# mcveanlab/Corticall

Hardware: AMD Instinct MI355X
Metric: k-mers traversed/sec (whole node) + contigs/sec, k=47 3-color LdBG (higher is better)
Workload: dtype u64

## Files before the change

### corticall_amd/csrc/capi.cpp

```cpp
#include <string.h>

#include <memory>

#include "build.h"
#include "cursor.h"
#include "engine_host.h"
#include "linkbuild.h"
#include "select.h"
#include "shard.h"
#include "thread.h"
#include "unitigs.h"

using namespace ldbg;

namespace ldbg {
int64_t sort_ctx_file(const std::string& in_path, const std::string& out_path, int device);
int64_t subset_ctx_file(const std::string& in_path, const int64_t* indices, int64_t n, const std::string& out_path);
int64_t join_ctx_files(const std::vector<std::string>& paths, const std::string& out_path, int device);
std::vector<uint8_t> join_ctx_image(const std::vector<std::string>& paths, int device, bool find_view);
void profile_reset_all();
bool profile_get(const char* family, double* ms, int64_t* n);
}

struct ldbg_graph {
    Graph g;
    ldbg_graph(const std::string& p, const void* img, int64_t n, int dev) : g(p, img, n, dev) {}
    ldbg_graph(const std::string& p, const void* hdr, int64_t hdr_bytes, const void* d_recs, int64_t n_recs, int dev) : g(p, hdr, hdr_bytes, d_recs, n_recs, dev) {}
};
struct ldbg_links {
    Links l;
    ldbg_links(const std::string& p, const Graph& g) : l(p, g) {}
    ldbg_links(const BuiltLinks& b, const Graph& g) : l(b, g) {}
};
struct ldbg_engine {
    Engine e;
    std::unique_ptr<CursorHost> cursor;
    std::unique_ptr<CursorBatchHost> cursor_batch;
    explicit ldbg_engine(const ldbg_engine_config& c) : e(c) {}
};
struct ldbg_dfs_result { std::unique_ptr<DfsBatch> b; };
struct ldbg_cursor_result { std::unique_ptr<CursorBatchResult> r; };
struct ldbg_unitigs { Unitigs u; ldbg_unitigs(const Graph& g, const int* c, int n) : u(g, c, n) {} };
struct ldbg_selection {
    Selection s;
    ldbg_selection(const Graph& g, const ldbg_record_filter& f, const Graph* q) : s(g, f, q) {}
    ldbg_selection(const Graph& g, int child_colour, const Graph& dirty) : s(g, child_colour, dirty) {}
};
struct ldbg_threading {
    Threading t;
    ldbg_threading(const Graph* g, const Graph* rois, const char* bases, const int64_t* offsets, int64_t n, int flags, bool dev, rt::stream_t s)
        : t(g, rois, bases, offsets, n, flags, dev, s) {}
};
struct ldbg_image { ShardImage img; ldbg_image(const Graph& shard, int64_t cap, int64_t global) : img(shard, cap, global) {} };

namespace {
thread_local std::string g_err;
template <class F>
ldbg_status guard(F f) {
    try { f(); return LDBG_OK; }
    catch (const StatusError& e) { g_err = e.what(); return (ldbg_status)e.status; }
    catch (const std::bad_alloc&) { g_err = "out of host memory"; return LDBG_ERR_HIP; }
    catch (const std::exception& e) { g_err = e.what(); return LDBG_ERR_ARG; }
}
ldbg_engine_config unwrap(const ldbg_engine_config& c, std::vector<const ldbg_links*>& keep) {
    ldbg_engine_config u = c;
    u.graph = c.graph ? (const ldbg_graph*)&c.graph->g : nullptr;
    u.rois = c.rois ? (const ldbg_graph*)&c.rois->g : nullptr;
    keep.clear();
    for (int i = 0; i < c.nlinks; i++) keep.push_back(c.links[i] ? (const ldbg_links*)&c.links[i]->l : nullptr);
    u.links = keep.data();
    return u;
}
}

extern "C" {

const char* ldbg_last_error(void) { return g_err.c_str(); }
#ifndef LDBG_SRCID
#define LDBG_SRCID "unstamped"
#endif
const char* ldbg_version(void) { return "ldbg 0.2 (gfx950, src " LDBG_SRCID ")"; }
ldbg_status ldbg_device_count(int* count) { *count = rt::device_count(); return LDBG_OK; }

ldbg_status ldbg_kmer_encode(const char* ascii, int k, uint64_t* words_out) {
    return guard([&] {
        if (k <= 0 || k > 128) throw StatusError(LDBG_ERR_ARG, "bad k");
        if (!ascii_to_words_ci(ascii, k, words_out, (k + 31) / 32))
            throw StatusError(LDBG_ERR_ARG, "Nucleotide is not a valid character nucleotide");
    });
}
ldbg_status ldbg_kmer_decode(const uint64_t* words, int k, char* ascii_out) {
    return guard([&] {
        if (k <= 0 || k > 128) throw StatusError(LDBG_ERR_ARG, "bad k");
        words_to_ascii(words, k, (k + 31) / 32, ascii_out);
        ascii_out[k] = 0;
    });
}

ldbg_status ldbg_sort_ctx(const char* in_path, const char* out_path, int device, int64_t* num_records) {
    return guard([&] { const int64_t n = sort_ctx_file(in_path, out_path, device); if (num_records) *num_records = n; });
}

ldbg_status ldbg_ctx_write_records(const char* in_path, const int64_t* indices, int64_t n, const char* out_path) {
    return guard([&] { subset_ctx_file(in_path, indices, n, out_path); });
}

ldbg_status ldbg_join_ctx(const char* const* in_paths, int n_paths, const char* out_path, int device, int64_t* num_records) {
    return guard([&] {
        std::vector<std::string> paths;
        for (int i = 0; i < n_paths; i++) paths.push_back(in_paths[i]);
        const int64_t n = join_ctx_files(paths, out_path, device);
        if (num_records) *num_records = n;
    });
}

ldbg_status ldbg_graph_open(const char* path, int device, ldbg_graph** out) {
    return guard([&] { *out = nullptr; *out = new ldbg_graph(path, nullptr, 0, device); });
}
ldbg_status ldbg_graph_open_memory(const void* image, int64_t nbytes, int device, ldbg_graph** out) {
    return guard([&] { *out = nullptr; *out = new ldbg_graph("<memory>", image, nbytes, device); });
}
ldbg_status ldbg_graph_open_device(const void* header, int64_t header_bytes, const void* d_records, int64_t n_records, int device, ldbg_graph** out) {
    return guard([&] { *out = nullptr; *out = new ldbg_graph("<device>", header, header_bytes, d_records, n_records, device); });
}
ldbg_status ldbg_graph_build(const ldbg_build_sample* samples, int n_samples, int k, int flags, int device, ldbg_graph** out) {
    return guard([&] {
        if (!out) throw StatusError(LDBG_ERR_ARG, "build: null output");
        *out = nullptr;
        const BuiltRecords b = build_records(samples, n_samples, k, flags, device);
        *out = new ldbg_graph("<build>", b.header.data(), (int64_t)b.header.size(), b.d_records.get(), b.N, device);
    });
}
ldbg_status ldbg_graph_build_ctx(const ldbg_build_sample* samples, int n_samples, int k, int flags, int device, const char* out_path, int64_t* num_records) {
    return guard([&] {
        if (!out_path) throw StatusError(LDBG_ERR_ARG, "build: null output path");
        const BuiltRecords b = build_records(samples, n_samples, k, flags, device);
        build_write_ctx(b, out_path);
        if (num_records) *num_records = b.N;
    });
}
ldbg_status ldbg_graph_open_collection(const char* const* paths, int n_paths, int find_view, int device, ldbg_graph** out) {
    return guard([&] {
        *out = nullptr;
        std::vector<std::string> ps;
        for (int i = 0; i < n_paths; i++) ps.push_back(paths[i]);
        const std::vector<uint8_t> img = join_ctx_image(ps, device, find_view != 0);
        *out = new ldbg_graph("<collection>", img.data(), (int64_t)img.size(), device);
    });
}
ldbg_status ldbg_graph_close(ldbg_graph* g) { return guard([&] { delete g; }); }
ldbg_status ldbg_graph_info(const ldbg_graph* g, int* k, int* W, int* C, int64_t* N, int* version) {
    return guard([&] {
        if (k) *k = g->g.hdr.k;
        if (W) *W = g->g.hdr.W;
        if (C) *C = g->g.hdr.C;
        if (N) *N = g->g.hdr.num_records;
        if (version) *version = g->g.hdr.version;
    });
}
ldbg_status ldbg_graph_device(const ldbg_graph* g, int* device) { *device = g->g.device; return LDBG_OK; }
ldbg_status ldbg_graph_set_shard(ldbg_graph* g, int is_shard) {
    return guard([&] { g->g.view.java_tiny = (!is_shard && g->g.view.N <= 2) ? 1 : 0; g->g.is_shard = is_shard != 0; });
}
ldbg_status ldbg_graph_sample_name(const ldbg_graph* g, int color, char* buf, int buflen) {
    return guard([&] {
        if (color < 0 || color >= g->g.hdr.C) throw StatusError(LDBG_ERR_ARG, "colour out of range");
        snprintf(buf, buflen, "%s", g->g.hdr.colors[color].sample_name.c_str());
    });
}
ldbg_status ldbg_graph_color_info(const ldbg_graph* g, int color, ldbg_color_info* out, char* name, int buflen) {
    return guard([&] {
        if (color < 0 || color >= g->g.hdr.C) throw StatusError(LDBG_ERR_ARG, "colour out of range");
        const CtxColor& c = g->g.hdr.colors[color];
        out->mean_read_length = c.mean_read_length;
        out->total_sequence = c.total_sequence;
        out->tip_clipping = c.tip_clipping;
        out->low_covg_supernodes_removed = c.low_covg_supernodes_removed;
        out->low_covg_kmers_removed = c.low_covg_kmers_removed;
        out->cleaned_against_graph = c.cleaned_against_graph;
        out->low_cov_supernodes_threshold = c.low_cov_supernodes_threshold;
        out->low_cov_kmer_threshold = c.low_cov_kmer_threshold;
        if (name) snprintf(name, buflen, "%s", c.cleaned_against_graph_name.c_str());
    });
}
ldbg_status ldbg_graph_color_for_sample_name(const ldbg_graph* g, const char* name, int* color) {
    return guard([&] { *color = g->g.color_for_sample_name(name); });
}

ldbg_status ldbg_graph_records_dev(const ldbg_graph* g, int64_t first, int64_t n, uint64_t* d_words, uint32_t* d_cov, uint8_t* d_edges, void* stream) {
    return guard([&] {
        if (first < 0 || n < 0 || first + n > g->g.hdr.num_records) throw StatusError(LDBG_ERR_ARG, "record range outside 0.." + std::to_string(g->g.hdr.num_records));
        rt::set_device(g->g.device);
        g->g.records_dev(first, n, d_words, d_cov, d_edges, stream ? (rt::stream_t)stream : g->g.stream);
    });
}
ldbg_status ldbg_graph_records(const ldbg_graph* g, int64_t first, int64_t n, uint64_t* words, uint32_t* cov, uint8_t* edges) {
    return guard([&] {
        if (first < 0 || n < 0 || first + n > g->g.hdr.num_records) throw StatusError(LDBG_ERR_ARG, "record range outside 0.." + std::to_string(g->g.hdr.num_records));
        if (n == 0) return;
        rt::set_device(g->g.device);
        const int W = g->g.hdr.W, C = g->g.hdr.C;
        rt::stream_t s = g->g.stream;
        uint64_t* dw = (uint64_t*)rt::dmalloc((size_t)n * W * 8);
        uint32_t* dc = cov ? (uint32_t*)rt::dmalloc((size_t)n * C * 4) : nullptr;
        uint8_t* de = edges ? (uint8_t*)rt::dmalloc((size_t)n * C) : nullptr;
        g->g.records_dev(first, n, dw, dc, de, s);
        if (words) rt::d2h(words, dw, (size_t)n * W * 8, s);
        if (cov) rt::d2h(cov, dc, (size_t)n * C * 4, s);
        if (edges) rt::d2h(edges, de, (size_t)n * C, s);
        rt::stream_sync(s);
        rt::dfree(dw); rt::dfree(dc); rt::dfree(de);
    });
}

ldbg_status ldbg_graph_find_dev(const ldbg_graph* g, const uint64_t* d_packed, int64_t n, int64_t* d_idx, uint32_t* d_cov, uint8_t* d_edges, void* stream) {
    return guard([&] {
        rt::set_device(g->g.device);
        g->g.find_dev(d_packed, n, d_idx, d_cov, d_edges, stream ? (rt::stream_t)stream : g->g.stream);
    });
}
ldbg_status ldbg_shard_owner_dev(int k, const uint64_t* d_packed, int64_t n, int world, uint64_t* d_canon, int32_t* d_owner, void* stream) {
    return guard([&] {
        shard_owner_dev(k, d_packed, n, world, d_canon, d_owner, (rt::stream_t)stream);
        rt::stream_sync((rt::stream_t)stream);
    });
}
ldbg_status ldbg_shard_owner(int k, const uint64_t* packed, int64_t n, int world, int device, int32_t* owner) {
    return guard([&] {
        if (n <= 0) return;
        if (rt::device_count() <= device) throw StatusError(LDBG_ERR_HIP, "no HIP device " + std::to_string(device) + " available (libldbg has no CPU fallback)");
        rt::set_device(device);
        const int W = (k + 31) / 32;
        rt::stream_t s = rt::stream_create();
        uint64_t* dq = (uint64_t*)rt::dmalloc((size_t)n * W * 8);
        int32_t* d_o = (int32_t*)rt::dmalloc((size_t)n * 4);
        rt::h2d(dq, packed, (size_t)n * W * 8, s);
        shard_owner_dev(k, dq, n, world, nullptr, d_o, s);
        rt::d2h(owner, d_o, (size_t)n * 4, s);
        rt::stream_sync(s);
        rt::dfree(dq); rt::dfree(d_o);
        rt::stream_destroy(s);
    });
}
ldbg_status ldbg_shard_nbr_queries(const ldbg_graph* g, int64_t first, int64_t n, uint64_t* d_words, uint8_t* d_flips, uint8_t* d_have) {
    return guard([&] { rt::set_device(g->g.device); shard_nbr_queries(g->g, first, n, d_words, d_flips, d_have); });
}
ldbg_status ldbg_shard_set_nbr(ldbg_graph* g, int64_t first, int64_t n, const int32_t* d_owner, const int64_t* d_lidx, const uint8_t* d_flips) {
    return guard([&] { rt::set_device(g->g.device); shard_set_nbr(g->g, first, n, d_owner, d_lidx, d_flips); });
}
ldbg_status ldbg_image_create(const ldbg_graph* shard, int64_t cap, int64_t global_records, ldbg_image** out) {
    return guard([&] {
        *out = nullptr;
        if (cap < 1 || cap > ldbg::max_records_per_device()) throw StatusError(LDBG_ERR_ARG, "image capacity out of range");
        *out = new ldbg_image(shard->g, cap, global_records);
    });
}
ldbg_status ldbg_image_destroy(ldbg_image* im) { return guard([&] { delete im; }); }
ldbg_status ldbg_image_graph(ldbg_image* im, ldbg_graph** g) { return guard([&] { *g = reinterpret_cast<ldbg_graph*>(&im->img.graph()); }); }
ldbg_status ldbg_image_row_bytes(const ldbg_image* im, int* bytes) { return guard([&] { *bytes = im->img.row_bytes(); }); }
ldbg_status ldbg_image_clear(ldbg_image* im) { return guard([&] { rt::set_device(im->img.graph().device); im->img.clear(); }); }
static rt::stream_t image_stream(const ldbg_image* im, void* stream) { return stream ? (rt::stream_t)stream : im->img.graph().stream; }
ldbg_status ldbg_image_serve(const ldbg_image* im, int my_rank, const uint64_t* d_keys, int64_t n, uint8_t* d_out, void* stream) {
    return guard([&] { rt::set_device(im->img.graph().device); im->img.serve(my_rank, (const unsigned long long*)d_keys, n, 1, d_out, image_stream(im, stream)); });
}
ldbg_status ldbg_image_serve_chain(const ldbg_image* im, int my_rank, const uint64_t* d_keys, int64_t n, int depth, uint8_t* d_out, void* stream) {
    return guard([&] { rt::set_device(im->img.graph().device); im->img.serve(my_rank, (const unsigned long long*)d_keys, n, depth, d_out, image_stream(im, stream)); });
}
ldbg_status ldbg_image_insert(ldbg_image* im, const ldbg_engine* e, const uint8_t* d_rows, int64_t n, void* stream) {
    return guard([&] { rt::set_device(im->img.graph().device); im->img.insert(e ? &e->e : nullptr, d_rows, n, image_stream(im, stream)); });
}
ldbg_status ldbg_image_lookup(const ldbg_image* im, const uint64_t* d_keys, int64_t n, int32_t* d_slots, void* stream) {
    return guard([&] { rt::set_device(im->img.graph().device); im->img.lookup((const unsigned long long*)d_keys, n, d_slots, image_stream(im, stream)); });
}
ldbg_status ldbg_image_bucket(ldbg_image* im, int world, uint32_t cap_per_owner, uint64_t* d_send, void* stream) {
    return guard([&] { rt::set_device(im->img.graph().device); im->img.bucket(world, cap_per_owner, (unsigned long long*)d_send, image_stream(im, stream)); });
}
ldbg_status ldbg_image_request(ldbg_image* im, const uint64_t* d_keys, int64_t n, void* stream) {
    return guard([&] { rt::set_device(im->img.graph().device); im->img.request((const unsigned long long*)d_keys, n, image_stream(im, stream)); });
}
ldbg_status ldbg_image_reset_requests(ldbg_image* im, void* stream) {
    return guard([&] { rt::set_device(im->img.graph().device); im->img.reset_requests(image_stream(im, stream)); });
}
ldbg_status ldbg_image_counters(const ldbg_image* im, int64_t* n_rows, int64_t* n_req, int* overflow) {
    return guard([&] { rt::set_device(im->img.graph().device); im->img.counters(n_rows, n_req, overflow); });
}
ldbg_status ldbg_engine_sharded_walk_begin(ldbg_engine* e, ldbg_image* im, const char* seeds, int64_t n, const int32_t* d_seed_slot, void* stream) {
    return guard([&] { e->e.sharded_walk_begin(im->img, seeds, n, d_seed_slot, (rt::stream_t)stream); });
}
ldbg_status ldbg_engine_sharded_walk_round(ldbg_engine* e, int64_t* d_stats) { return guard([&] { e->e.sharded_walk_round(d_stats); }); }
ldbg_status ldbg_engine_sharded_walk_finish(ldbg_engine* e, int64_t* total_bytes, int64_t* traversed) {
    return guard([&] {
        try { e->e.sharded_walk_finish(total_bytes, traversed); }
        catch (const StatusError& se) {
            if (se.status == LDBG_ERR_CAPACITY && std::string(se.what()) == "LINKSTORE_FULL") e->e.link_store_capacity *= 4;
            throw;
        }
    });
}

ldbg_status ldbg_graph_find(const ldbg_graph* g, const uint64_t* packed, int64_t n, int64_t* idx_out, uint32_t* cov_out, uint8_t* edges_out) {
    return guard([&] {
        if (n <= 0) return;
        rt::set_device(g->g.device);
        const int W = g->g.hdr.W, C = g->g.hdr.C;
        rt::stream_t s = g->g.stream;
        uint64_t* dq = (uint64_t*)rt::dmalloc((size_t)n * W * 8);
        int64_t* di = (int64_t*)rt::dmalloc((size_t)n * 8);
        uint32_t* dc = cov_out ? (uint32_t*)rt::dmalloc((size_t)n * C * 4) : nullptr;
        uint8_t* de = edges_out ? (uint8_t*)rt::dmalloc((size_t)n * C) : nullptr;
        rt::h2d(dq, packed, (size_t)n * W * 8, s);
        g->g.find_dev(dq, n, di, dc, de, s);
        rt::d2h(idx_out, di, (size_t)n * 8, s);
        if (cov_out) rt::d2h(cov_out, dc, (size_t)n * C * 4, s);
        if (edges_out) rt::d2h(edges_out, de, (size_t)n * C, s);
        rt::stream_sync(s);
        rt::dfree(dq); rt::dfree(di); rt::dfree(dc); rt::dfree(de);
    });
}
ldbg_status ldbg_graph_find_ascii(const ldbg_graph* g, const char* kmers, int64_t n, int64_t* idx_out, uint32_t* cov_out, uint8_t* edges_out) {
    return guard([&] {
        rt::set_device(g->g.device);
        const int W = g->g.hdr.W, k = g->g.hdr.k, C = g->g.hdr.C;
        if (n <= 0) return;
        std::vector<uint64_t> packed((size_t)n * W);
        std::vector<uint8_t> valid((size_t)n);
        ascii_batch_to_words(kmers, n, k, W, packed.data(), valid.data());
        rt::stream_t s = g->g.stream;
        DevBlocks tmp;
        uint64_t* dq = tmp.get<uint64_t>((size_t)n * W);
        uint8_t* dv = tmp.get<uint8_t>((size_t)n);
        int64_t* di = tmp.get<int64_t>((size_t)n);
        uint32_t* dc = cov_out ? tmp.get<uint32_t>((size_t)n * C) : nullptr;
        uint8_t* de = edges_out ? tmp.get<uint8_t>((size_t)n * C) : nullptr;
        rt::h2d(dq, packed.data(), (size_t)n * W * 8, s);
        rt::h2d(dv, valid.data(), (size_t)n, s);
        g->g.find_dev(dq, n, di, dc, de, s, dv);
        rt::d2h(idx_out, di, (size_t)n * 8, s);
        if (cov_out) rt::d2h(cov_out, dc, (size_t)n * C * 4, s);
        if (edges_out) rt::d2h(edges_out, de, (size_t)n * C, s);
        rt::stream_sync(s);
    });
}

ldbg_status ldbg_graph_unitigs(const ldbg_graph* g, const int* colors, int n_colors, ldbg_unitigs** out) {
    return guard([&] {
        *out = nullptr;
        if (!colors && n_colors > 0) throw StatusError(LDBG_ERR_ARG, "unitigs: null colours");
        *out = new ldbg_unitigs(g->g, colors, n_colors);
    });
}
ldbg_status ldbg_unitigs_info(const ldbg_unitigs* u, int64_t* count, int64_t* total_bases, int64_t* longest, double* build_ms) {
    return guard([&] {
        if (count) *count = u->u.count;
        if (total_bases) *total_bases = u->u.total_bases;
        if (longest) *longest = u->u.longest;
        if (build_ms) *build_ms = u->u.build_ms;
    });
}
ldbg_status ldbg_unitigs_get(const ldbg_unitigs* u, int64_t first, int64_t n, int64_t* offsets, char* bases, int64_t capacity) {
    return guard([&] { u->u.get(first, n, offsets, bases, capacity, false, u->u.graph.stream); });
}
ldbg_status ldbg_unitigs_get_dev(const ldbg_unitigs* u, int64_t first, int64_t n, int64_t* d_offsets, char* d_bases, int64_t capacity, void* stream) {
    return guard([&] { u->u.get(first, n, d_offsets, d_bases, capacity, true, stream ? (rt::stream_t)stream : u->u.graph.stream); });
}
ldbg_status ldbg_unitigs_coverage(const ldbg_unitigs* u, int64_t first, int64_t n, uint32_t* cov) { return guard([&] { u->u.coverage(first, n, cov); }); }
ldbg_status ldbg_unitigs_of_records(const ldbg_unitigs* u, const int64_t* records, int64_t n, int64_t* unitig, int64_t* position, int8_t* orientation) {
    return guard([&] { u->u.of_records(records, n, unitig, position, orientation); });
}
ldbg_status ldbg_unitigs_write_fasta(const ldbg_unitigs* u, const char* path) { return guard([&] { u->u.write_fasta(path); }); }
ldbg_status ldbg_unitigs_write_gfa1(const ldbg_unitigs* u, const char* path, int sample_color, int flags) {
    return guard([&] { u->u.write_gfa1(path, sample_color, flags); });
}
ldbg_status ldbg_unitigs_free(ldbg_unitigs* u) { return guard([&] { delete u; }); }

ldbg_status ldbg_graph_select(const ldbg_graph* g, const ldbg_record_filter* filter, ldbg_selection** out) {
    return guard([&] {
        *out = nullptr;
        if (!filter) throw StatusError(LDBG_ERR_ARG, "select: null filter");
        *out = new ldbg_selection(g->g, *filter, nullptr);
    });
}
ldbg_status ldbg_graph_select_lookup(const ldbg_graph* g, const ldbg_record_filter* filter, const ldbg_graph* q, ldbg_selection** out) {
    return guard([&] {
        *out = nullptr;
        if (!filter || !q) throw StatusError(LDBG_ERR_ARG, "select: null filter or query graph");
        *out = new ldbg_selection(g->g, *filter, &q->g);
    });
}
ldbg_status ldbg_selection_count(const ldbg_selection* sel, int64_t* n) { return guard([&] { *n = sel->s.count; }); }
ldbg_status ldbg_selection_indices(const ldbg_selection* sel, int64_t first, int64_t n, int64_t* idx) {
    return guard([&] { sel->s.indices(first, n, idx, false, sel->s.graph.stream); });
}
ldbg_status ldbg_selection_indices_dev(const ldbg_selection* sel, int64_t first, int64_t n, int64_t* d_idx, void* stream) {
    return guard([&] { sel->s.indices(first, n, d_idx, true, stream ? (rt::stream_t)stream : sel->s.graph.stream); });
}
ldbg_status ldbg_selection_write_ctx(const ldbg_selection* sel, const int* colours, int n_colours, const char* header_path, const char* out_path) {
    return guard([&] { sel->s.write_ctx(colours, n_colours, header_path, out_path); });
}
ldbg_status ldbg_selection_open_graph(const ldbg_selection* sel, const int* colours, int n_colours, const char* header_path, ldbg_graph** out) {
    return guard([&] {
        *out = nullptr;
        const std::vector<uint8_t> hdr = sel->s.header(colours, n_colours, header_path);
        const DevRecords d = sel->s.pack(colours, n_colours);
        *out = new ldbg_graph("<selection>", hdr.data(), (int64_t)hdr.size(), d.get(), sel->s.count, sel->s.graph.device);
    });
}
ldbg_status ldbg_selection_free(ldbg_selection* sel) { return guard([&] { delete sel; }); }

ldbg_status ldbg_graph_recover(const ldbg_graph* g, int child_colour, const ldbg_graph* dirty, ldbg_selection** out, int64_t* n_recovered) {
    return guard([&] {
        if (!out) throw StatusError(LDBG_ERR_ARG, "recover: null output");
        *out = nullptr;
        if (!g || !dirty) throw StatusError(LDBG_ERR_ARG, "recover: null graph");
        *out = new ldbg_selection(g->g, child_colour, dirty->g);
        if (n_recovered) *n_recovered = (*out)->s.n_recovered;
    });
}
ldbg_status ldbg_selection_recovered_coverage(const ldbg_selection* sel, int64_t first, int64_t n, int32_t* cov) {
    return guard([&] { sel->s.recovered_coverage(first, n, cov); });
}
ldbg_status ldbg_selection_write_recovered(const ldbg_selection* sel, const char* out_path) {
    return guard([&] {
        if (!out_path) throw StatusError(LDBG_ERR_ARG, "recover: null output path");
        sel->s.write_recovered(out_path);
    });
}
ldbg_status ldbg_selection_open_recovered(const ldbg_selection* sel, ldbg_graph** out) {
    return guard([&] {
        *out = nullptr;
        const std::vector<uint8_t> hdr = sel->s.recovered_header();
        const DevRecords d = sel->s.pack_recovered();
        *out = new ldbg_graph("<recovered>", hdr.data(), (int64_t)hdr.size(), d.get(), sel->s.count, sel->s.graph.device);
    });
}

ldbg_status ldbg_links_open(const char* path, const ldbg_graph* g, ldbg_links** out) {
    return guard([&] { *out = nullptr; *out = new ldbg_links(path, g->g); });
}
ldbg_status ldbg_links_build_ctp(const ldbg_graph* g, const char* sample_name, const char* bases, const int64_t* offsets, int64_t n_reads, int flags,
                                 const char* out_path, int64_t* num_kmers_with_links, int64_t* num_links) {
    return guard([&] {
        if (!g) throw StatusError(LDBG_ERR_ARG, "links build: null graph");
        if (!out_path) throw StatusError(LDBG_ERR_ARG, "links build: null output path");
        const BuiltLinks b = build_links(g->g, sample_name, bases, offsets, n_reads, flags);
        built_links_write(b, out_path);
        if (num_kmers_with_links) *num_kmers_with_links = (int64_t)b.records.size();
        if (num_links) *num_links = b.num_links;
    });
}
ldbg_status ldbg_links_build(const ldbg_graph* g, const char* sample_name, const char* bases, const int64_t* offsets, int64_t n_reads, int flags, ldbg_links** out) {
    return guard([&] {
        if (!out) throw StatusError(LDBG_ERR_ARG, "links build: null output");
        *out = nullptr;
        if (!g) throw StatusError(LDBG_ERR_ARG, "links build: null graph");
        const BuiltLinks b = build_links(g->g, sample_name, bases, offsets, n_reads, flags);
        *out = new ldbg_links(b, g->g);
    });
}
ldbg_status ldbg_graph_thread(const ldbg_graph* g, const ldbg_graph* rois, const char* bases, const int64_t* offsets, int64_t n_seqs, int flags, ldbg_threading** out) {
    return guard([&] {
        if (!out) throw StatusError(LDBG_ERR_ARG, "thread: null output");
        *out = nullptr;
        *out = new ldbg_threading(g ? &g->g : nullptr, rois ? &rois->g : nullptr, bases, offsets, n_seqs, flags, false, nullptr);
    });
}
ldbg_status ldbg_graph_thread_dev(const ldbg_graph* g, const ldbg_graph* rois, const void* d_bases, const void* d_offsets, int64_t n_seqs, int flags, void* stream,
                                  ldbg_threading** out) {
    return guard([&] {
        if (!out) throw StatusError(LDBG_ERR_ARG, "thread: null output");
        *out = nullptr;
        *out = new ldbg_threading(g ? &g->g : nullptr, rois ? &rois->g : nullptr, (const char*)d_bases, (const int64_t*)d_offsets, n_seqs, flags, true, (rt::stream_t)stream);
    });
}
ldbg_status ldbg_threading_info(const ldbg_threading* t, int64_t* n_seqs, int64_t* n_windows, int64_t* n_regions, double* device_ms) {
    return guard([&] {
        if (!t) throw StatusError(LDBG_ERR_ARG, "thread: null threading");
        if (n_seqs) *n_seqs = t->t.n_seqs;
        if (n_windows) *n_windows = t->t.n_windows;
        if (n_regions) *n_regions = t->t.n_regions;
        if (device_ms) *device_ms = t->t.device_ms;
    });
}
ldbg_status ldbg_threading_windows(const ldbg_threading* t, int64_t first, int64_t n, int64_t* rec, uint8_t* info, int32_t* copy_index) {
    return guard([&] {
        if (!t) throw StatusError(LDBG_ERR_ARG, "thread: null threading");
        t->t.windows(first, n, rec, info, copy_index, false, nullptr);
    });
}
ldbg_status ldbg_threading_windows_dev(const ldbg_threading* t, int64_t first, int64_t n, void* d_rec, void* d_info, void* d_copy_index, void* stream) {
    return guard([&] {
        if (!t) throw StatusError(LDBG_ERR_ARG, "thread: null threading");
        t->t.windows(first, n, (int64_t*)d_rec, (uint8_t*)d_info, (int32_t*)d_copy_index, true, (rt::stream_t)stream);
    });
}
ldbg_status ldbg_threading_coverage(const ldbg_threading* t, int colour, int64_t first, int64_t n, int32_t* cov) {
    return guard([&] {
        if (!t) throw StatusError(LDBG_ERR_ARG, "thread: null threading");
        t->t.coverage(colour, first, n, cov);
    });
}
ldbg_status ldbg_threading_summary(const ldbg_threading* t, int64_t first_seq, int64_t n, int64_t* win_start, int32_t* first_hit, int32_t* last_hit, int32_t* n_hits,
                                   int32_t* n_distinct, uint8_t* ends) {
    return guard([&] {
        if (!t) throw StatusError(LDBG_ERR_ARG, "thread: null threading");
        t->t.summary(first_seq, n, win_start, first_hit, last_hit, n_hits, n_distinct, ends);
    });
}
ldbg_status ldbg_threading_regions(const ldbg_threading* t, int64_t* region_offsets, int32_t* start, int32_t* stop, int64_t capacity) {
    return guard([&] {
        if (!t) throw StatusError(LDBG_ERR_ARG, "thread: null threading");
        t->t.regions(region_offsets, start, stop, capacity);
    });
}
ldbg_status ldbg_threading_free(ldbg_threading* t) { return guard([&] { delete t; }); }

ldbg_status ldbg_links_close(ldbg_links* l) { return guard([&] { delete l; }); }
ldbg_status ldbg_links_index(const char* in_path, const char* out_path, const char* source, int64_t* num_records) {
    return guard([&] { const int64_t n = links_index_file(in_path, out_path, source ? source : ""); if (num_records) *num_records = n; });
}
ldbg_status ldbg_links_source(const ldbg_links* l, char* buf, int buflen) { return guard([&] { snprintf(buf, buflen, "%s", l->l.source().c_str()); }); }
ldbg_status ldbg_links_info(const ldbg_links* l, int* version, int* num_colors, int* k, int64_t* nkg, int64_t* nkl, int64_t* nl) {
    return guard([&] {
        if (version) *version = l->l.version;
        if (num_colors) *num_colors = l->l.num_colors;
        if (k) *k = l->l.k;
        if (nkg) *nkg = l->l.num_kmers_in_graph;
        if (nkl) *nkl = l->l.num_kmers_with_links;
        if (nl) *nl = l->l.num_links;
    });
}
ldbg_status ldbg_links_sample_name(const ldbg_links* l, int color, char* buf, int buflen) {
    return guard([&] {
        if (color < 0 || color >= (int)l->l.sample_names.size()) throw StatusError(LDBG_ERR_ARG, "colour out of range");
        snprintf(buf, buflen, "%s", l->l.sample_names[color].c_str());
    });
}
ldbg_status ldbg_links_get(const ldbg_links* l, const char* kmer, int* found, char* buf, int64_t buflen) {
    return guard([&] {
        const HostLinksRecord* r = l->l.get(std::string(kmer, l->l.k));
        *found = r ? 1 : 0;
        std::string s;
        if (r) {
            s = r->kmer + " " + std::to_string(r->juncs.size()) + "\n";
            for (auto& j : r->juncs) {
                s += j.is_fw ? "F " : "R ";
                s += std::to_string(j.num_junctions) + " ";
                for (size_t c = 0; c < j.cov.size(); c++) { if (c) s += ","; s += std::to_string(j.cov[c]); }
                s += " " + j.junctions + "\n";
            }
        }
        if ((int64_t)s.size() + 1 > buflen) throw StatusError(LDBG_ERR_CAPACITY, "buffer too small: need " + std::to_string(s.size() + 1));
        memcpy(buf, s.c_str(), s.size() + 1);
    });
}

void ldbg_engine_config_default(ldbg_engine_config* c) {
    memset(c, 0, sizeof(*c));
    c->direction = LDBG_DIR_BOTH;
    c->combination_operator = LDBG_OP_OR;
    c->stopping_rule = LDBG_STOP_CONTIG;
    c->max_branch_length = 75000;
    c->connect_all_neighbors = 0;
    c->strict_java_flip = 1;
}
ldbg_status ldbg_engine_create(const ldbg_engine_config* cfg, ldbg_engine** out) {
    return guard([&] {
        *out = nullptr;
        if (cfg->n_traversal > LDBG_MAX_COLORS || cfg->n_joining > LDBG_MAX_COLORS || cfg->n_recruitment > LDBG_MAX_COLORS || cfg->n_secondary > LDBG_MAX_COLORS)
            throw StatusError(LDBG_ERR_ARG, "too many colours");
        std::vector<const ldbg_links*> keep;
        ldbg_engine_config u = unwrap(*cfg, keep);
        *out = new ldbg_engine(u);
    });
}
ldbg_status ldbg_engine_destroy(ldbg_engine* e) { return guard([&] { delete e; }); }

static ldbg_status walk_batch_run_any(ldbg_engine* e, const char* seeds, int64_t n, int64_t* total_bytes, int64_t* traversed, bool on_device) {
    return guard([&] {
        for (int attempt = 0;; attempt++) {
            try { e->e.walk_batch_run(seeds, n, total_bytes, traversed, on_device); return; }
            catch (const StatusError& se) {
                if (se.status == LDBG_ERR_CAPACITY && std::string(se.what()) == "LINKSTORE_FULL" && attempt < 8) { e->e.link_store_capacity *= 4; continue; }
                throw;
            }
        }
    });
}
ldbg_status ldbg_engine_walk_batch_run(ldbg_engine* e, const char* seeds, int64_t n, int64_t* total_bytes, int64_t* traversed) {
    return walk_batch_run_any(e, seeds, n, total_bytes, traversed, false);
}
ldbg_status ldbg_engine_walk_batch_run_device(ldbg_engine* e, const void* d_seeds, int64_t n, int64_t* total_bytes, int64_t* traversed) {
    if (n > 0 && !d_seeds) return guard([&] { throw StatusError(LDBG_ERR_ARG, "ldbg_engine_walk_batch_run_device: null seeds"); });
    return walk_batch_run_any(e, (const char*)d_seeds, n, total_bytes, traversed, true);
}
ldbg_status ldbg_host_alloc(int64_t bytes, void** out) {
    return guard([&] { *out = nullptr; if (bytes < 0) throw StatusError(LDBG_ERR_ARG, "ldbg_host_alloc: negative size"); *out = rt::hmalloc_pinned((size_t)bytes); });
}
ldbg_status ldbg_host_free(void* p) { return guard([&] { rt::hfree_pinned(p); }); }
ldbg_status ldbg_engine_walk_batch_fetch(ldbg_engine* e, char* arena, int64_t cap, int64_t* offsets, int64_t* walk_len) {
    return guard([&] { e->e.walk_batch_fetch(arena, cap, offsets, walk_len); });
}
ldbg_status ldbg_engine_walk_batch(ldbg_engine* e, const char* seeds, int64_t n, char* arena, int64_t cap, int64_t* offsets, int64_t* walk_len, int64_t* traversed) {
    int64_t total = 0;
    ldbg_status st = ldbg_engine_walk_batch_run(e, seeds, n, &total, traversed);
    if (st != LDBG_OK) return st;
    return ldbg_engine_walk_batch_fetch(e, arena, cap, offsets, walk_len);
}
ldbg_status ldbg_engine_walk_vertices(ldbg_engine* e, int64_t walk, int64_t capacity, int64_t* len, uint64_t* words, int64_t* rec, int32_t* copy, int32_t* index) {
    return guard([&] { e->e.walk_vertices(walk, capacity, len, words, rec, copy, index); });
}

ldbg_status ldbg_engine_walk_roi_hits(ldbg_engine* e, int64_t* offsets, uint32_t* hits, int64_t capacity, uint8_t* has_null) {
    return guard([&] { e->e.walk_roi_hits(offsets, hits, capacity, has_null); });
}

ldbg_status ldbg_engine_dfs_batch(ldbg_engine* e, const char* sources, int64_t n, const char* sinks, const int64_t* sink_offsets, ldbg_dfs_result** out) {
    return guard([&] {
        *out = nullptr;
        for (int attempt = 0;; attempt++) {
            try {
                std::unique_ptr<DfsBatch> b(e->e.dfs_batch(sources, n, sinks, sink_offsets));
                *out = new ldbg_dfs_result{std::move(b)};
                return;
            } catch (const StatusError& se) {
                const std::string what = se.what();
                if (se.status == LDBG_ERR_CAPACITY && what == "LINKSTORE_FULL" && attempt < 8) { e->e.link_store_capacity *= 4; continue; }
                if (se.status == LDBG_ERR_CAPACITY && what == "LOG_FULL" && e->e.dfs_log_blocks < (1 << 20)) { e->e.dfs_log_blocks *= 8; continue; }
                if (se.status == LDBG_ERR_CAPACITY && what == "DEPTH_OVERFLOW" && e->e.dfs_max_depth < 4096) { e->e.dfs_max_depth *= 4; continue; }
                if (se.status == LDBG_ERR_CAPACITY && what == "DEPTH_OVERFLOW")
                    throw StatusError(LDBG_ERR_UNSUPPORTED, "dfs recursion deeper than 4096 branches (the reference overflows its thread stack here)");
                throw;
            }
        }
    });
}
ldbg_status ldbg_engine_sharded_dfs_batch(ldbg_engine* e, ldbg_image* im, const char* sources, int64_t n, const char* sinks, const int64_t* sink_offsets,
                                          const int32_t* d_seed_slot, const int32_t* d_sink_slot, int (*round_done)(void*), void* user,
                                          int64_t* d_stats, void* stream, ldbg_dfs_result** out) {
    return guard([&] {
        *out = nullptr;
        if (&im->img.graph() != e->e.graph) throw StatusError(LDBG_ERR_ARG, "the engine was not created on this image's graph");
        ShardedRun sr{&im->img, d_seed_slot, d_sink_slot, round_done, user, d_stats, (rt::stream_t)stream};
        try {
            std::unique_ptr<DfsBatch> b(e->e.dfs_batch(sources, n, sinks, sink_offsets, &sr));
            b->materialize();
            *out = new ldbg_dfs_result{std::move(b)};
        } catch (const StatusError& se) {
            const std::string what = se.what();
            if (se.status == LDBG_ERR_CAPACITY && what == "LINKSTORE_FULL") e->e.link_store_capacity *= 4;
            if (se.status == LDBG_ERR_CAPACITY && what == "LOG_FULL" && e->e.dfs_log_blocks < (1 << 20)) e->e.dfs_log_blocks *= 8;
            if (se.status == LDBG_ERR_CAPACITY && what == "DEPTH_OVERFLOW" && e->e.dfs_max_depth < 4096) e->e.dfs_max_depth *= 4;
            throw;
        }
    });
}
static const DfsGraphHost& dfs_at(const ldbg_dfs_result* r, int64_t i) {
    if (!r || !r->b) throw StatusError(LDBG_ERR_ARG, "no dfs result");
    if (i < 0 || i >= (int64_t)r->b->results.size()) throw StatusError(LDBG_ERR_ARG, "dfs result index out of range");
    return r->b->results[(size_t)i];
}
ldbg_status ldbg_dfs_result_sizes(const ldbg_dfs_result* r, int64_t i, int* is_null, int64_t* n_vertices, int64_t* n_edges) {
    return guard([&] {
        const DfsGraphHost& g = dfs_at(r, i);
        if (is_null) *is_null = g.is_null ? 1 : 0;
        if (n_vertices) *n_vertices = g.n_vertices();
        if (n_edges) *n_edges = g.n_edges();
    });
}
ldbg_status ldbg_dfs_result_get(const ldbg_dfs_result* r, int64_t i, uint64_t* kmer_words, int64_t* rec, int32_t* copy_index, int32_t* index,
                                int32_t* edge_src, int32_t* edge_dst, int32_t* edge_color) {
    return guard([&] {
        dfs_at(r, i);
        if (kmer_words) r->b->materialize();
        const DfsGraphHost& g = dfs_at(r, i);
        if (g.packed) { r->b->read_packed(i, rec, copy_index, index, edge_src, edge_dst, edge_color); return; }
        if (kmer_words && !g.words.empty()) memcpy(kmer_words, g.words.data(), g.words.size() * 8);
        for (size_t v = 0; v < g.verts.size(); v++) {
            if (rec) rec[v] = g.verts[v].rec;
            if (copy_index) copy_index[v] = g.verts[v].copy;
            if (index) index[v] = g.verts[v].index;
        }
        for (size_t x = 0; x < g.edges.size(); x++) {
            if (edge_src) edge_src[x] = g.edges[x].src;
            if (edge_dst) edge_dst[x] = g.edges[x].dst;
            if (edge_color) edge_color[x] = g.edges[x].color;
        }
    });
}
ldbg_status ldbg_dfs_result_walk(const ldbg_dfs_result* r, int64_t i, const char* seed, int color, char* contig, int64_t capacity, int64_t* len) {
    return guard([&] {
        dfs_at(r, i);
        const std::string c = r->b->walk_contig(i, seed, color);
        if (len) *len = (int64_t)c.size();
        if ((int64_t)c.size() + 1 > capacity) throw StatusError(LDBG_ERR_CAPACITY, "contig buffer too small: need " + std::to_string(c.size() + 1));
        memcpy(contig, c.c_str(), c.size() + 1);
    });
}
ldbg_status ldbg_dfs_result_merge(ldbg_dfs_result* r, const int64_t* which, int64_t m, ldbg_dfs_result** out) {
    return guard([&] {
        *out = nullptr;
        std::unique_ptr<DfsBatch> b(dfs_merge(*r->b, which, m));
        *out = new ldbg_dfs_result{std::move(b)};
    });
}
ldbg_status ldbg_dfs_result_free(ldbg_dfs_result* r) { delete r; return LDBG_OK; }
ldbg_status ldbg_engine_neighbours_batch(ldbg_engine* e, const char* kmers, int64_t n, int forward, int64_t* offsets, uint64_t* kmer_words, int64_t* rec, int64_t capacity) {
    return guard([&] { e->e.neighbours_batch(kmers, n, forward != 0, offsets, kmer_words, rec, capacity); });
}
ldbg_status ldbg_engine_dfs_kmers_traversed(const ldbg_engine* e, int64_t* n) { return guard([&] { *n = e->e.dfs_traversed(); }); }

static CursorHost& cursor_of(ldbg_engine* e) {
    if (!e->cursor) e->cursor.reset(new CursorHost(e->e));
    return *e->cursor;
}
ldbg_status ldbg_engine_assemble(ldbg_engine* e, const char* seed, int64_t capacity, int64_t* len, uint64_t* kmer_words, int64_t* rec) {
    return guard([&] { cursor_of(e).assemble(seed, capacity, len, kmer_words, rec); });
}
ldbg_status ldbg_engine_seek(ldbg_engine* e, const char* kmer) { return guard([&] { cursor_of(e).seek(kmer); }); }
ldbg_status ldbg_engine_has_next(ldbg_engine* e, int* yes) { return guard([&] { *yes = cursor_of(e).has(true) ? 1 : 0; }); }
ldbg_status ldbg_engine_has_previous(ldbg_engine* e, int* yes) { return guard([&] { *yes = cursor_of(e).has(false) ? 1 : 0; }); }
ldbg_status ldbg_engine_next(ldbg_engine* e, char* kmer_out, int64_t* rec_out) { return guard([&] { cursor_of(e).step(true, kmer_out, rec_out); }); }
ldbg_status ldbg_engine_previous(ldbg_engine* e, char* kmer_out, int64_t* rec_out) { return guard([&] { cursor_of(e).step(false, kmer_out, rec_out); }); }

static ldbg_status cursor_batch_any(ldbg_engine* e, const char* seeds, int64_t n, bool on_device, int direction, int64_t max_steps, const ldbg_cursor_stop* stop,
                                    ldbg_cursor_result** out) {
    return guard([&] {
        if (!e || !out) throw StatusError(LDBG_ERR_ARG, "cursor batch: null engine or result pointer");
        *out = nullptr;
        if (!e->cursor_batch) e->cursor_batch.reset(new CursorBatchHost(e->e));
        std::unique_ptr<CursorBatchResult> r(e->cursor_batch->run(seeds, n, on_device, direction, max_steps, stop));
        *out = new ldbg_cursor_result{std::move(r)};
    });
}
ldbg_status ldbg_engine_cursor_batch(ldbg_engine* e, const char* seeds, int64_t n, int direction, int64_t max_steps, const ldbg_cursor_stop* stop,
                                     ldbg_cursor_result** out) {
    return cursor_batch_any(e, seeds, n, false, direction, max_steps, stop, out);
}
ldbg_status ldbg_engine_cursor_batch_device(ldbg_engine* e, const void* d_seeds, int64_t n, int direction, int64_t max_steps, const ldbg_cursor_stop* stop,
                                            ldbg_cursor_result** out) {
    return cursor_batch_any(e, (const char*)d_seeds, n, true, direction, max_steps, stop, out);
}
static const CursorBatchResult& cursor_result_of(const ldbg_cursor_result* r) {
    if (!r || !r->r) throw StatusError(LDBG_ERR_ARG, "no cursor result");
    return *r->r;
}
ldbg_status ldbg_cursor_result_sizes(const ldbg_cursor_result* r, int64_t* n_seeds, int64_t* n_vertices, int* kmer_words) {
    return guard([&] {
        const CursorBatchResult& c = cursor_result_of(r);
        if (n_seeds) *n_seeds = c.n;
        if (n_vertices) *n_vertices = c.total;
        if (kmer_words) *kmer_words = c.W;
    });
}
ldbg_status ldbg_cursor_result_get(const ldbg_cursor_result* r, int64_t* offsets, uint64_t* kmer_words, int64_t* rec, int32_t* n_reverse, int32_t* n_forward,
                                   int64_t* seed_rec, uint8_t* end_reverse, uint8_t* end_forward, uint8_t* status) {
    return guard([&] { cursor_result_of(r).get(offsets, kmer_words, rec, n_reverse, n_forward, seed_rec, end_reverse, end_forward, status, false, nullptr); });
}
ldbg_status ldbg_cursor_result_get_dev(const ldbg_cursor_result* r, void* d_offsets, void* d_kmer_words, void* d_rec, void* d_n_reverse, void* d_n_forward,
                                       void* d_seed_rec, void* d_end_reverse, void* d_end_forward, void* d_status, void* stream) {
    return guard([&] {
        cursor_result_of(r).get(d_offsets, d_kmer_words, d_rec, d_n_reverse, d_n_forward, d_seed_rec, d_end_reverse, d_end_forward, d_status, true, (rt::stream_t)stream);
    });
}
ldbg_status ldbg_cursor_result_free(ldbg_cursor_result* r) { delete r; return LDBG_OK; }

#ifdef LDBG_HOSTSIM
void ldbg_debug_ls(uint64_t* out) {
    auto& d = ldbg::ls_debug();
    out[0] = d.adds; out[1] = d.newkeys; out[2] = d.choices; out[3] = d.scan; out[4] = d.maxn; out[5] = d.steps; out[6] = d.sum_n;
    out[7] = d.runs_a; out[8] = d.runs_b; out[9] = d.run_vertices; out[10] = d.retries; out[11] = d.repeats;
    d = ldbg::LsDebug();
}
#endif
#ifdef LDBG_HOSTSIM
extern "C" void ldbg_hostsim_set_lanes(int n) { int v = 1; while (v * 2 <= n && v < 64) v *= 2; ::ldbg::sim::lanes_setting() = v; }
#endif
ldbg_status ldbg_profile_reset(void) { profile_reset_all(); return LDBG_OK; }
ldbg_status ldbg_profile_get(const char* family, double* total_ms, int64_t* launches) {
    profile_get(family, total_ms, launches);
    return LDBG_OK;
}

}
```

### corticall_amd/csrc/engine_host.h

```cpp
#pragma once
#include <memory>
#include <string>
#include <vector>

#include "engine.h"

namespace ldbg {

struct WalkChunk {
    int64_t first = 0, n = 0;
    void* d_path = nullptr;
    size_t path_cap = 0, contigs_cap = 0;
    void* d_contigs = nullptr;
    void* d_seed_words = nullptr;
    void* d_term = nullptr;
    void* d_contig_off = nullptr;
    void* d_walk_len = nullptr;
    int64_t total_bytes = 0;
    int64_t total_entries = 0;
    bool host_ready = false;
    std::vector<int64_t> strand_off;
    std::vector<int64_t> contig_off;
    std::vector<int64_t> walk_len;
    std::vector<uint32_t> status;
    void* d_strand_c = nullptr;
    void* d_strand_off = nullptr;
    int max_blocks = 0;
    RunIndexView runs{};
    bool dense_pending = false;
};

struct DfsVertex { int64_t rec; int64_t slot; int32_t copy, index; uint8_t flip; };
struct DfsEdge { int src, dst, color; };
struct DfsGraphHost {
    bool is_null = true;
    bool packed = false;
    uint32_t n_rev = 0, n_fwd = 0, p_seg = 0;
    uint64_t p_off = 0;
    int64_t n_vertices() const { return packed ? (int64_t)n_rev + n_fwd - ((n_rev && n_fwd) ? 1 : 0) : (int64_t)verts.size(); }
    int64_t n_edges() const { return packed ? (int64_t)(n_rev ? n_rev - 1 : 0) + (n_fwd ? n_fwd - 1 : 0) : (int64_t)edges.size(); }
    int64_t slot_base = 0;
    std::vector<DfsVertex> verts;
    std::vector<DfsEdge> edges;
    std::vector<uint64_t> words;
    std::vector<uint32_t> cov;
    std::vector<std::vector<uint64_t>> null_kmers;
};
struct DfsBatch {
    int k = 0, W = 0, C = 0;
    int64_t traversed = 0;
    std::vector<DfsGraphHost> results;
    const Graph* graph = nullptr;
    std::vector<std::vector<uint64_t>> packed_store;
    int color = 0;
    void read_packed(int64_t i, int64_t* rec, int32_t* copy_index, int32_t* index, int32_t* edge_src, int32_t* edge_dst, int32_t* edge_color) const;
    std::vector<std::vector<uint64_t>> key_segments;
    int64_t n_gather = 0;
    bool materialized = false;
    void materialize();
    std::string walk_contig(int64_t i, const char* seed, int color);
};

DfsBatch* dfs_merge(DfsBatch& b, const int64_t* which, int64_t m);

struct WalkArgs;
struct WalkRun;
struct DfsRun;
struct DfsKeys;
class ShardImage;
struct ShardedRun {
    ShardImage* img;
    const int32_t* d_seed_slot;
    const int32_t* d_sink_slot;
    int (*round_done)(void* user);
    void* user;
    int64_t* d_stats;
    rt::stream_t stream;
};
uint64_t vt_series(uint64_t init, uint64_t vmax);
uint32_t vt_initial_entries();

class Engine {
public:
    explicit Engine(const ldbg_engine_config& cfg);
    ~Engine();
    const Graph* graph = nullptr;
    const Graph* rois = nullptr;
    std::vector<const Links*> my_links;
    ldbg_engine_config cfg{};
    EngineView view{};

    void walk_batch_run(const char* seeds, int64_t n, int64_t* total_contig_bytes, int64_t* kmers_traversed, bool seeds_on_device = false);
    void walk_batch_fetch(char* arena, int64_t cap, int64_t* offsets, int64_t* walk_len);
    void walk_vertices(int64_t walk, int64_t capacity, int64_t* len, uint64_t* words, int64_t* rec, int32_t* copy, int32_t* index);
    void clear_batch();
    void enter();
    rt::stream_t estream() const { return stream_; }
    void quiesce() noexcept;
    void walk_roi_hits(int64_t* offsets, uint32_t* hits, int64_t capacity, uint8_t* has_null);
    void sharded_walk_begin(ShardImage& img, const char* seeds, int64_t n, const int32_t* d_seed_slot, rt::stream_t round_stream);
    void sharded_walk_round(int64_t* d_stats);
    void sharded_walk_finish(int64_t* total_contig_bytes, int64_t* kmers_traversed);
    void sharded_abort();
    DfsBatch* dfs_batch(const char* sources, int64_t n, const char* sinks, const int64_t* sink_offsets, const ShardedRun* sharded = nullptr);
    void neighbours_batch(const char* kmers, int64_t n, bool forward, int64_t* offsets, uint64_t* kmer_words, int64_t* rec, int64_t capacity);
    int dfs_max_depth = 64;
    int dfs_log_blocks = 64;
    int64_t dfs_traversed() const { return dfs_traversed_; }
    int64_t dfs_retried_ = 0;
    int64_t retried_strands() const { return retried_strands_; }

    int64_t batch_n = 0, batch_bytes = 0, batch_traversed = 0;
    std::vector<WalkChunk> chunks;
    uint32_t link_store_capacity = 64;

private:
    rt::stream_t stream_ = nullptr, own_stream_ = nullptr;
    void* d_vpool_ = nullptr; void* d_ls_ = nullptr; void* d_snap_ = nullptr;
    void* d_pool_ = nullptr; void* d_block_table_ = nullptr;
    int64_t n_slots_ = 0, bt_strands_ = 0;
    uint64_t n_blocks_ = 0, vpool_entries_ = 0, vpool_dirty_ = 0;
    uint32_t ecap_ = 0;
    int max_blocks_ = 0;
    void* d_frames_ = nullptr; size_t d_frames_bytes_ = 0;
    void* d_roi_bits_ = nullptr;
    void* d_roi_of_ = nullptr;
    int64_t dfs_traversed_ = 0;
    std::unique_ptr<MergedLinks> merged_;
    std::unique_ptr<class RunIndex> runs_;
    int64_t retried_strands_ = 0;
    std::vector<uint8_t> sink_valid_;
    std::vector<uint8_t> seed_valid_;
    void* d_batch_words_ = nullptr; void* d_batch_valid_ = nullptr; void* d_batch_ascii_ = nullptr;
    void seeds_to_device(const char* seeds, int64_t n, bool seeds_on_device);
    void drop_batch_seeds();
    unsigned long long* h_small_ = nullptr;
    void ensure_host(WalkChunk& c);
    void build_roi_bits();
    void dfs_prepare(DfsRun& r, const std::vector<uint64_t>& seed_words, const std::vector<uint64_t>& sink_words, const int64_t* sink_offsets,
                     int64_t first, int64_t n, const ShardedRun* sharded);
    void dfs_launch_resident(DfsRun& r);
    void dfs_launch_sharded(DfsRun& r);
    bool dfs_check_status(DfsRun& r, DfsBatch& out);
    void dfs_fetch_logs(DfsRun& r);
    DfsKeys dfs_assemble(DfsRun& r, DfsBatch& out);
    void dfs_secondary_colours(DfsRun& r, DfsBatch& out, DfsKeys& keys);
    void launch_compact_paths(const int64_t* d_strand_off, int64_t n_strands, uint64_t* d_dense, int max_blocks);
    void launch_path_lengths(const uint32_t* d_strand_c, int64_t n_strands, int max_blocks, uint32_t* d_len);
    void launch_expand_paths(const uint32_t* d_strand_c, const int64_t* d_strand_off, int64_t n_strands, uint64_t* d_dense, int max_blocks, const RunIndexView& runs,
                             unsigned* d_overflow);
    void ensure_run_index();
    void ensure_scratch(int64_t n_strands, uint32_t ecap, int max_blocks, uint64_t table_floor = 0, bool small = false);
    uint64_t scratch_scale_ = 1, scratch_scale_built_ = 1; bool scratch_full_ = true; int64_t pool_growths_ = 0;
    uint64_t table_floor_ = 0;
    void* h_stage_[2] = {nullptr, nullptr};
    void download(char* dst, const void* d_src, size_t bytes);
    uint64_t* h_log_ = nullptr; size_t h_log_cap_ = 0;
    void release_scratch();
    struct Spare { void* p; size_t bytes; };
    std::vector<Spare> spares_;
    void* result_alloc(size_t bytes, size_t* cap);
    void result_free(void* p, size_t cap);
    void drop_spares();
    void zero_dirty_tables(rt::stream_t s);
    bool run_chunk(int64_t first, int64_t n, WalkChunk& out, int64_t* traversed);
    void ensure_dense(WalkChunk& c);
    void materialize_pending();
    static constexpr int64_t kFetchStride = 7919;
    static constexpr uint32_t kWalkImgYield = 32u, kDfsImgYield = 128u;
    void fill_strand_args(WalkArgs& a, int64_t ns, int max_blocks, uint32_t vcap_max, unsigned long long* d_ctr, ShardImage* img, const int32_t* d_seed_slot,
                          int64_t stride, uint32_t img_yield);
    void walk_prepare(int64_t first, int64_t n, WalkRun& r, ShardImage* img, const int32_t* d_seed_slot);
    void walk_launch(WalkRun& r);
    bool walk_finish(WalkRun& r, int64_t* traversed);
    WalkRun* sharded_run_ = nullptr;
    ShardImage* sharded_img_ = nullptr;
    rt::stream_t sharded_stream_ = nullptr;
    int64_t sharded_rounds_ = 0;
};

}
```

### corticall_amd/csrc/rt.h

```cpp
#pragma once
#include <stdint.h>
#include <stdlib.h>
#include <string.h>

#include <algorithm>
#include <map>
#include <mutex>
#include <string>
#include <type_traits>
#include <unordered_map>
#include <utility>
#include <vector>

#include "../../include/ldbg.h"
#include "ctx_host.h"

#ifndef LDBG_HOSTSIM
#include <hip/hip_runtime.h>
#define LDBG_KERNEL __global__
#define LDBG_WAVE_KERNEL __global__ __launch_bounds__(64)
#define LDBG_WAVE_KERNEL_N(n) __global__ __launch_bounds__(n)
#define LDBG_DEV __device__ __forceinline__
#define LDBG_HOSTDEV __host__ __device__ __forceinline__
#if defined(__HIP_DEVICE_COMPILE__)
#define LDBG_GLOBAL(T, p) ((__attribute__((address_space(1))) T*)(p))
#define LDBG_LDS(T, p) ((__attribute__((address_space(3))) T*)(p))
#else
#define LDBG_GLOBAL(T, p) ((T*)(p))
#define LDBG_LDS(T, p) ((T*)(p))
#endif

namespace ldbg {
namespace rt {

inline void check(hipError_t e, const char* what) {
    if (e != hipSuccess) throw StatusError(LDBG_ERR_HIP, std::string(what) + ": " + hipGetErrorString(e));
}
inline int device_count() {
    int n = 0;
    hipError_t e = hipGetDeviceCount(&n);
    if (e != hipSuccess) { (void)hipGetLastError(); return 0; }
    return n;
}
inline void set_device(int d) { check(hipSetDevice(d), "hipSetDevice"); }
inline int cu_count(int d) {
    int n = 0;
    check(hipDeviceGetAttribute(&n, hipDeviceAttributeMultiprocessorCount, d), "hipDeviceGetAttribute");
    return n > 0 ? n : 256;
}
struct BlockCache {
    std::mutex m;
    std::unordered_map<void*, std::pair<int, size_t>> live;
    std::map<std::pair<int, size_t>, std::vector<void*>> free_;
    size_t held = 0;
    static size_t size_class(size_t n) {
        size_t c = 4096;
        while (c < n) { if (c + c / 2 >= n) return c + c / 2; c *= 2; }
        return c;
    }
    void release_all() {
        std::lock_guard<std::mutex> g(m);
        for (auto& kv : free_) for (void* p : kv.second) (void)hipFree(p);
        free_.clear(); held = 0;
    }
};
inline BlockCache& block_cache() { static BlockCache c; return c; }
inline void* dmalloc(size_t n) {
    void* p = nullptr;
    hipError_t e = hipMalloc(&p, n ? n : 1);
    if (e != hipSuccess) { (void)hipGetLastError(); block_cache().release_all(); e = hipMalloc(&p, n ? n : 1); }
    check(e, "hipMalloc");
    return p;
}
inline void dfree(void* p) {
    if (!p) return;
    { BlockCache& c = block_cache(); std::lock_guard<std::mutex> g(c.m); c.live.erase(p); }
    (void)hipFree(p);
}
inline void* tmalloc(size_t n) {
    BlockCache& c = block_cache();
    const size_t cls = BlockCache::size_class(n);
    if (cls > ((size_t)64 << 20)) return dmalloc(n);
    int dev = 0;
    check(hipGetDevice(&dev), "hipGetDevice");
    {
        std::lock_guard<std::mutex> g(c.m);
        auto it = c.free_.find({dev, cls});
        if (it != c.free_.end() && !it->second.empty()) {
            void* p = it->second.back();
            it->second.pop_back();
            c.held -= cls;
            c.live[p] = {dev, cls};
            return p;
        }
    }
    void* p = dmalloc(cls);
    std::lock_guard<std::mutex> g(c.m);
    c.live[p] = {dev, cls};
    return p;
}
inline void tfree(void* p) {
    if (!p) return;
    BlockCache& c = block_cache();
    {
        std::lock_guard<std::mutex> g(c.m);
        auto it = c.live.find(p);
        if (it != c.live.end() && c.held + it->second.second <= ((size_t)1 << 30)) {
            c.free_[it->second].push_back(p);
            c.held += it->second.second;
            c.live.erase(it);
            return;
        }
        if (it != c.live.end()) c.live.erase(it);
    }
    (void)hipFree(p);
}
inline void* hmalloc_pinned(size_t n) { void* p = nullptr; check(hipHostMalloc(&p, n ? n : 1, hipHostMallocDefault), "hipHostMalloc"); return p; }
inline void hfree_pinned(void* p) { if (p) (void)hipHostFree(p); }
inline bool host_is_pinned(const void* p) {
    hipPointerAttribute_t a;
    if (hipPointerGetAttributes(&a, p) != hipSuccess) { (void)hipGetLastError(); return false; }
    return a.type == hipMemoryTypeHost;
}
typedef hipStream_t stream_t;
inline stream_t stream_create() { hipStream_t s; check(hipStreamCreateWithFlags(&s, hipStreamNonBlocking), "hipStreamCreate"); return s; }
inline void stream_destroy(stream_t s) { if (s) (void)hipStreamDestroy(s); }
inline void stream_sync(stream_t s) { check(hipStreamSynchronize(s), "hipStreamSynchronize"); }
inline void h2d(void* d, const void* h, size_t n, stream_t s) { if (n) check(hipMemcpyAsync(d, h, n, hipMemcpyHostToDevice, s), "hipMemcpyAsync H2D"); }
inline void d2h(void* h, const void* d, size_t n, stream_t s) { if (n) check(hipMemcpyAsync(h, d, n, hipMemcpyDeviceToHost, s), "hipMemcpyAsync D2H"); }
inline void d2d(void* d, const void* s_, size_t n, stream_t s) { if (n) check(hipMemcpyAsync(d, s_, n, hipMemcpyDeviceToDevice, s), "hipMemcpyAsync D2D"); }
inline void dmemset(void* d, int v, size_t n, stream_t s) { if (n) check(hipMemsetAsync(d, v, n, s), "hipMemsetAsync"); }
inline void mem_info(size_t* free_b, size_t* total_b) { check(hipMemGetInfo(free_b, total_b), "hipMemGetInfo"); }
inline void launch_check(const char* name) { check(hipGetLastError(), name); }
template <class K>
inline int blocks_per_cu(K kernel, int block) {
    static std::mutex m;
    static std::map<std::pair<const void*, std::pair<int, int>>, int> known;
    int dev = 0;
    check(hipGetDevice(&dev), "hipGetDevice");
    const std::pair<const void*, std::pair<int, int>> key{(const void*)kernel, {block, dev}};
    std::lock_guard<std::mutex> g(m);
    auto it = known.find(key);
    if (it != known.end()) return it->second;
    int n = 0;
    check(hipOccupancyMaxActiveBlocksPerMultiprocessor(&n, kernel, block, 0), "hipOccupancyMaxActiveBlocksPerMultiprocessor");
    if (n < 1) throw StatusError(LDBG_ERR_HIP, "hipOccupancyMaxActiveBlocksPerMultiprocessor: the kernel does not fit a compute unit");
    known[key] = n;
    return n;
}

struct Event {
    hipEvent_t e = nullptr;
    Event() { check(hipEventCreate(&e), "hipEventCreate"); }
    ~Event() { if (e) (void)hipEventDestroy(e); }
    Event(Event&& o) noexcept : e(o.e) { o.e = nullptr; }
    Event& operator=(Event&& o) noexcept { if (this != &o) { if (e) (void)hipEventDestroy(e); e = o.e; o.e = nullptr; } return *this; }
    Event(const Event&) = delete;
    Event& operator=(const Event&) = delete;
    void record(stream_t s) { check(hipEventRecord(e, s), "hipEventRecord"); }
    void wait() { check(hipEventSynchronize(e), "hipEventSynchronize"); }
    static float elapsed_ms(Event& a, Event& b) {
        check(hipEventSynchronize(b.e), "hipEventSynchronize");
        float ms = 0;
        check(hipEventElapsedTime(&ms, a.e, b.e), "hipEventElapsedTime");
        return ms;
    }
};

}
}

#define LDBG_LAUNCH(kernel, grid, block, stream, ...)                               \
    do {                                                                            \
        hipLaunchKernelGGL(kernel, dim3((unsigned)(grid)), dim3((unsigned)(block)), 0, stream, __VA_ARGS__); \
        ::ldbg::rt::launch_check(#kernel);                                          \
    } while (0)

namespace ldbg {
LDBG_DEV int64_t global_tid() { return (int64_t)blockIdx.x * blockDim.x + threadIdx.x; }
LDBG_DEV int64_t global_nthreads() { return (int64_t)gridDim.x * blockDim.x; }
LDBG_DEV unsigned long long atomic_add_u64(unsigned long long* p, unsigned long long v) { return atomicAdd(p, v); }
LDBG_DEV unsigned atomic_add_u32(unsigned* p, unsigned v) { return atomicAdd(p, v); }
LDBG_DEV unsigned atomic_min_u32(unsigned* p, unsigned v) { return atomicMin(p, v); }
LDBG_DEV unsigned atomic_max_u32(unsigned* p, unsigned v) { return atomicMax(p, v); }
LDBG_DEV unsigned atomic_or_u32(unsigned* p, unsigned v) { return atomicOr(p, v); }
LDBG_DEV unsigned long long atomic_min_u64(unsigned long long* p, unsigned long long v) { return atomicMin(p, v); }
LDBG_DEV unsigned long long atomic_cas_u64(unsigned long long* p, unsigned long long cmp, unsigned long long v) { return atomicCAS(p, cmp, v); }
LDBG_DEV unsigned long long atomic_exch_u64(unsigned long long* p, unsigned long long v) { return atomicExch(p, v); }
LDBG_DEV int wave_size() { return blockDim.x < 64u ? (int)blockDim.x : 64; }
LDBG_DEV int wave_lane() { return (int)(threadIdx.x & 63u); }
LDBG_DEV unsigned long long wave_ballot(bool p) { return __ballot(p ? 1 : 0); }
LDBG_DEV uint32_t wave_bcast_u32(uint32_t v, int src) { return (uint32_t)__builtin_amdgcn_readlane((int)v, __builtin_amdgcn_readfirstlane(src)); }
LDBG_DEV uint64_t wave_bcast_u64(uint64_t v, int src) {
    uint32_t lo = wave_bcast_u32((uint32_t)v, src), hi = wave_bcast_u32((uint32_t)(v >> 32), src);
    return ((uint64_t)hi << 32) | lo;
}
LDBG_DEV uint32_t wave_shfl_u32(uint32_t v, int src) { return (uint32_t)__shfl((int)v, src & 63, 64); }
LDBG_DEV uint64_t wave_shfl_u64(uint64_t v, int src) { return ((uint64_t)wave_shfl_u32((uint32_t)(v >> 32), src) << 32) | wave_shfl_u32((uint32_t)v, src); }
LDBG_DEV void wave_fence() { __threadfence_block(); }
LDBG_DEV void device_fence() { __threadfence(); }
LDBG_DEV uint64_t wave_shfl_xor_u64(uint64_t v, int m) {
    uint32_t lo = (uint32_t)__shfl_xor((int)(uint32_t)v, m, 64), hi = (uint32_t)__shfl_xor((int)(uint32_t)(v >> 32), m, 64);
    return ((uint64_t)hi << 32) | lo;
}
LDBG_DEV uint64_t wave_min_u64(uint64_t v) { for (int m = wave_size() >> 1; m > 0; m >>= 1) { uint64_t o = wave_shfl_xor_u64(v, m); v = o < v ? o : v; } return v; }
LDBG_DEV uint64_t wave_max_u64(uint64_t v) { for (int m = wave_size() >> 1; m > 0; m >>= 1) { uint64_t o = wave_shfl_xor_u64(v, m); v = o > v ? o : v; } return v; }
LDBG_DEV int wave_count_below(unsigned long long ballot) { return __builtin_popcountll(ballot & ((1ull << wave_lane()) - 1ull)); }
LDBG_DEV uint32_t wave_incl_scan_u32(uint32_t v) {
    const int lane = wave_lane();
    for (int d = 1; d < wave_size(); d <<= 1) { const uint32_t o = (uint32_t)__shfl_up((int)v, d, 64); if (lane >= d) v += o; }
    return v;
}
}

#else
#define LDBG_KERNEL static
#define LDBG_WAVE_KERNEL static
#define LDBG_WAVE_KERNEL_N(n) static
#define LDBG_DEV inline
#define LDBG_HOSTDEV inline
#define LDBG_GLOBAL(T, p) ((T*)(p))
#define LDBG_LDS(T, p) ((T*)(p))
#ifndef __forceinline__
#define __forceinline__
#endif

namespace ldbg {
namespace rt {
inline int device_count() { return 1; }
inline void set_device(int) {}
inline int cu_count(int) { return 256; }
inline bool poison() { static const bool on = getenv("LDBG_HOSTSIM_POISON") != nullptr; return on; }
inline void* dmalloc(size_t n) {
    if (!poison()) return calloc(n ? n : 1, 1);
    void* p = malloc(n ? n : 1);
    if (p) memset(p, 0xAB, n ? n : 1);
    return p;
}
inline void dfree(void* p) { free(p); }
inline void* tmalloc(size_t n) { return dmalloc(n); }
inline void tfree(void* p) { free(p); }
inline void* hmalloc_pinned(size_t n) { return malloc(n ? n : 1); }
inline void hfree_pinned(void* p) { free(p); }
inline bool host_is_pinned(const void*) { return getenv("LDBG_HOSTSIM_PAGEABLE") == nullptr; }
typedef void* stream_t;
inline stream_t stream_create() { return nullptr; }
inline void stream_destroy(stream_t) {}
inline void stream_sync(stream_t) {}
inline void h2d(void* d, const void* h, size_t n, stream_t) { if (n) memcpy(d, h, n); }
inline void d2h(void* h, const void* d, size_t n, stream_t) { if (n) memcpy(h, d, n); }
inline void d2d(void* d, const void* s, size_t n, stream_t) { if (n) memmove(d, s, n); }
inline void dmemset(void* d, int v, size_t n, stream_t) { if (n) memset(d, v, n); }
template <class K> inline int blocks_per_cu(K, int) { return 8; }
inline void mem_info(size_t* free_b, size_t* total_b) {
    size_t mb = 2048;
    if (const char* ev = getenv("LDBG_HOSTSIM_MEM_MB")) mb = (size_t)atoll(ev);
    *free_b = mb << 20; *total_b = mb << 20;
}
struct Event {
    void record(stream_t) {}
    void wait() {}
    static float elapsed_ms(Event&, Event&) { return 0.0f; }
};
}
}
#include <execinfo.h>
#include <ucontext.h>
#include <stdio.h>
#include <functional>
#include <vector>
namespace ldbg {
namespace sim {
struct Wave {
    int lanes = 1, cur = 0, live = 0, arrived = 0;
    unsigned long long gen = 0;
    bool active = false;
    ucontext_t sched;
    ucontext_t ctx[64];
    std::vector<char> stacks[64];
    uint8_t done[64];
    int kind[64];
    void* site[64];
    uint64_t x[2][64];
    uint64_t y[2][64];
    int64_t tid0 = 0, nthreads = 1;
    std::function<void()>* body = nullptr;
};
inline Wave& wave() { static thread_local Wave w; return w; }
inline int& lanes_setting() { static int n = [] { const char* e = getenv("LDBG_HOSTSIM_LANES"); int v = e ? atoi(e) : 1; return v < 1 ? 1 : (v > 64 ? 64 : v); }(); return n; }
inline int lanes_env() { return lanes_setting(); }
inline void yield() { Wave& w = wave(); swapcontext(&w.ctx[w.cur], &w.sched); }
inline int collective(int kind, uint64_t a, uint64_t b = 0) {
    Wave& w = wave();
    const int buf = (int)(w.gen & 1ull);
    const unsigned long long my_gen = w.gen;
    w.x[buf][w.cur] = a; w.y[buf][w.cur] = b; w.kind[w.cur] = kind; w.site[w.cur] = __builtin_return_address(0);
    w.arrived++;
    if (w.arrived == w.live) {
        for (int l = 0; l < w.lanes; l++)
            if (!w.done[l] && w.kind[l] != kind) {
                fprintf(stderr, "[hostsim] wavefront divergence: lane %d is at primitive %d (%p), lane %d at %d (%p); the arriving lane's stack:\n", w.cur, kind, w.site[w.cur], l, w.kind[l], w.site[l]);
                void* bt[32];
                backtrace_symbols_fd(bt, backtrace(bt, 32), 2);
                abort();
            }
        w.arrived = 0; w.gen++;
    } else {
        while (w.gen == my_gen) yield();
    }
    return buf;
}
inline void trampoline() {
    Wave& w = wave();
    (*w.body)();
    w.done[w.cur] = 1;
    w.live--;
    if (w.live > 0 && w.arrived == w.live) {
        const int kd = [&] { for (int l = 0; l < w.lanes; l++) if (!w.done[l]) return w.kind[l]; return 0; }();
        for (int l = 0; l < w.lanes; l++)
            if (!w.done[l] && w.kind[l] != kd) { fprintf(stderr, "[hostsim] wavefront divergence at a lane's exit\n"); abort(); }
        w.arrived = 0; w.gen++;
    }
    swapcontext(&w.ctx[w.cur], &w.sched);
}
void run_wave(int lanes, int64_t tid0, int64_t nthreads, std::function<void()>& body);
}
struct SimIdx { int64_t tid, nthreads; };
inline SimIdx& sim_idx() { static thread_local SimIdx s{0, 1}; return s; }
inline int64_t global_tid() { return sim_idx().tid; }
inline int64_t global_nthreads() { return sim_idx().nthreads; }
inline void sim::run_wave(int lanes, int64_t tid0, int64_t nthreads, std::function<void()>& body) {
    Wave& w = wave();
    w.lanes = lanes; w.live = lanes; w.arrived = 0; w.gen = 0; w.active = true; w.body = &body; w.tid0 = tid0; w.nthreads = nthreads;
    for (int l = 0; l < lanes; l++) {
        if (w.stacks[l].empty()) w.stacks[l].resize((size_t)1 << 20);
        w.done[l] = 0; w.kind[l] = 0;
        getcontext(&w.ctx[l]);
        w.ctx[l].uc_stack.ss_sp = w.stacks[l].data();
        w.ctx[l].uc_stack.ss_size = w.stacks[l].size();
        w.ctx[l].uc_link = &w.sched;
        makecontext(&w.ctx[l], (void (*)())sim::trampoline, 0);
    }
    while (w.live > 0) {
        for (int l = 0; l < lanes; l++) {
            if (w.done[l]) continue;
            w.cur = l;
            sim_idx().tid = tid0 + l; sim_idx().nthreads = nthreads;
            swapcontext(&w.sched, &w.ctx[l]);
        }
    }
    w.active = false; w.lanes = 1; w.cur = 0;
}
inline unsigned long long atomic_add_u64(unsigned long long* p, unsigned long long v) { unsigned long long o = *p; *p += v; return o; }
inline unsigned atomic_add_u32(unsigned* p, unsigned v) { unsigned o = *p; *p += v; return o; }
inline unsigned atomic_min_u32(unsigned* p, unsigned v) { unsigned o = *p; if (v < o) *p = v; return o; }
inline unsigned atomic_max_u32(unsigned* p, unsigned v) { unsigned o = *p; if (v > o) *p = v; return o; }
inline unsigned atomic_or_u32(unsigned* p, unsigned v) { unsigned o = *p; *p |= v; return o; }
inline unsigned long long atomic_min_u64(unsigned long long* p, unsigned long long v) { unsigned long long o = *p; if (v < o) *p = v; return o; }
inline unsigned long long atomic_cas_u64(unsigned long long* p, unsigned long long cmp, unsigned long long v) { unsigned long long o = *p; if (o == cmp) *p = v; return o; }
inline unsigned long long atomic_exch_u64(unsigned long long* p, unsigned long long v) { unsigned long long o = *p; *p = v; return o; }
inline int wave_size() { return sim::wave().active ? sim::wave().lanes : 1; }
inline int wave_lane() { return sim::wave().active ? sim::wave().cur : 0; }
inline unsigned long long wave_ballot(bool p) {
    sim::Wave& w = sim::wave();
    if (!w.active) return p ? 1ull : 0ull;
    const int b = sim::collective(1, p ? 1ull : 0ull);
    unsigned long long m = 0;
    for (int l = 0; l < w.lanes; l++) if (!w.done[l] && w.x[b][l]) m |= 1ull << l;
    return m;
}
inline uint64_t wave_shfl_u64(uint64_t v, int src) {
    sim::Wave& w = sim::wave();
    if (!w.active) return v;
    const int b = sim::collective(2, v);
    return w.x[b][src & (w.lanes - 1)];
}
inline uint32_t wave_shfl_u32(uint32_t v, int src) { return (uint32_t)wave_shfl_u64(v, src); }
inline uint32_t wave_bcast_u32(uint32_t v, int src) { return (uint32_t)wave_shfl_u64(v, src); }
inline uint64_t wave_bcast_u64(uint64_t v, int src) { return wave_shfl_u64(v, src); }
inline uint64_t wave_shfl_xor_u64(uint64_t v, int m) { return wave_shfl_u64(v, wave_lane() ^ m); }
inline void wave_fence() { if (sim::wave().active) (void)sim::collective(3, 0ull); }
inline void device_fence() {}
inline uint64_t wave_min_u64(uint64_t v) { for (int m = wave_size() >> 1; m > 0; m >>= 1) { uint64_t o = wave_shfl_xor_u64(v, m); v = o < v ? o : v; } return v; }
inline uint64_t wave_max_u64(uint64_t v) { for (int m = wave_size() >> 1; m > 0; m >>= 1) { uint64_t o = wave_shfl_xor_u64(v, m); v = o > v ? o : v; } return v; }
inline int wave_count_below(unsigned long long ballot) { return __builtin_popcountll(ballot & ((1ull << wave_lane()) - 1ull)); }
inline uint32_t wave_incl_scan_u32(uint32_t v) {
    sim::Wave& w = sim::wave();
    if (!w.active) return v;
    const int b = sim::collective(4, v);
    uint32_t s = 0;
    for (int l = 0; l <= w.cur; l++) if (!w.done[l]) s += (uint32_t)w.x[b][l];
    return s;
}
}

#define LDBG_LAUNCH(kernel, grid, block, stream, ...)                      \
    do {                                                                   \
        int64_t nt__ = (int64_t)(grid) * (int64_t)(block);                 \
        if (nt__ > 4096) nt__ = 4096;                                      \
        const int lanes__ = ::ldbg::sim::lanes_env() > 1 && (int64_t)(block) <= 64 ? (int)std::min<int64_t>((int64_t)(block), (int64_t)::ldbg::sim::lanes_env()) : 1; \
        if (lanes__ > 1) {                                                 \
            nt__ = (nt__ / lanes__) * lanes__; if (nt__ < lanes__) nt__ = lanes__; \
            std::function<void()> body__ = [&]() { kernel(__VA_ARGS__); }; \
            for (int64_t t__ = 0; t__ < nt__; t__ += lanes__) ::ldbg::sim::run_wave(lanes__, t__, nt__, body__); \
            ::ldbg::sim_idx().tid = 0; ::ldbg::sim_idx().nthreads = 1;     \
            break;                                                         \
        }                                                                  \
        ::ldbg::sim_idx().nthreads = nt__;                                 \
        for (int64_t t__ = 0; t__ < nt__; t__++) {                         \
            ::ldbg::sim_idx().tid = t__;                                   \
            kernel(__VA_ARGS__);                                           \
        }                                                                  \
    } while (0)
#endif

#define LDBG_LAUNCH_W(W, KER, grid, block, stream, ...)                               \
    do {                                                                              \
        switch ((int)(W)) {                                                           \
            case 1: LDBG_LAUNCH(KER<1>, grid, block, stream, __VA_ARGS__); break;     \
            case 2: LDBG_LAUNCH(KER<2>, grid, block, stream, __VA_ARGS__); break;     \
            case 3: LDBG_LAUNCH(KER<3>, grid, block, stream, __VA_ARGS__); break;     \
            default: LDBG_LAUNCH(KER<4>, grid, block, stream, __VA_ARGS__); break;    \
        }                                                                             \
    } while (0)

namespace ldbg {
template <class F>
inline decltype(auto) with_words(int W, F&& f) {
    switch (W) {
        case 1: return f(std::integral_constant<int, 1>{});
        case 2: return f(std::integral_constant<int, 2>{});
        case 3: return f(std::integral_constant<int, 3>{});
        default: return f(std::integral_constant<int, 4>{});
    }
}
inline int grid_for(int64_t n, int block = 256, int max_blocks = 4096) {
    return (int)std::max<int64_t>(1, std::min<int64_t>((n + block - 1) / block, max_blocks));
}
inline uint32_t next_pow2(uint64_t v, uint64_t cap = ~0ull) { uint64_t p = 1; while (p < v) p <<= 1; return (uint32_t)std::min<uint64_t>(p, cap); }
}
```

### corticall_amd/csrc/walk.cpp

```cpp
#include <algorithm>
#include <chrono>
#include <numeric>
#include <thread>

#include "lscoop.h"
#include "runs.h"
#include "runstep.h"
#include "shard.h"
#include "strand.h"

namespace ldbg {

#define LDBG_STREAM_BLOCK 64
#define LDBG_STREAM_GRID 65536

LDBG_DEV void walk_finish(const WalkArgs& a, StrandState& st) {
    strand_finish(a, st);
    const bool good = !st.branch_null && st.status == ST_OK;
    a.strand_n[st.s] = good ? st.gV : 0u;
    a.strand_c[st.s] = good ? st.pw.n : 0u;
}

template <int W>
LDBG_DEV bool strand_step(const WalkArgs& a, StrandState& st, LinkStoreDev& ls, const StepPre& pre, RunState& rs) {
    const EngineView& e = a.e;
    const bool fwd = st.fwd;
    if (st.status != ST_OK) return true;
    st.iters++;
    Node& cv = st.cv;
    const uint32_t m = fwd ? cv.next_mask : cv.prev_mask;
    int adj = 0;
    Node av = cv;
    if (e.cursor_on && st.cu.has) {
        av = cursor_step<W, true>(e, st.cu, ls, st.vt, fwd, &pre, &rs.seen_marks);
        if (st.cu.status != ST_OK) { st.status = st.cu.status; return true; }
        if (st.cu.has) { node_sync(cv, st.cu.nxt); node_sync(av, st.cu.nxt); }
        const int cnt = node_count(av);
        av.copy = fwd ? cnt : -cnt;
        adj = 1;
    } else {
        for (unsigned b = 0; b < 4; b++) {
            if (!((m >> b) & 1u)) continue;
            Node x;
            node_child_located(e, st.vt, cv, fwd, b, x);
            if (node_count(x) > 0) continue;
            adj++;
            av = x;
        }
    }
    const int acopy = cv.copy < 0 ? -cv.copy : cv.copy;
    const uint64_t ecv = cv.idx >= 0 ? cv.vent : 0ull;
    const bool previously = acopy < vt_count_e(ecv);
    if (!previously && cv.idx >= 0) {
        if (acopy + 1 > 32767) { st.status = ST_COPY_OVERFLOW; return true; }
        node_store(st.vt, cv, vt_with_count(ecv, acopy + 1));
        node_sync(av, cv);
        if (e.cursor_on) { node_sync(st.cu.cur, cv); if (st.cu.has) node_sync(st.cu.nxt, cv); }
    }
    const bool reached = st.gV > (uint32_t)e.max_len;
    if (previously) { st.branch_null = true; return true; }
    if (adj != 1 || reached) return true;
    if (st.gV == 0) {
        if (!path_append(a, st.s, st.pw, pack_vertex(cv))) { st.status = ST_POOL_FULL; return true; }
        st.gV = 1;
    }
    if (!path_append(a, st.s, st.pw, pack_vertex(av))) { st.status = ST_POOL_FULL; return true; }
    st.gV++;
    st.quirk |= (cv.flip && !cv.fj) || (av.flip && !av.fj);
    if (av.idx < 0) {
        const Kmer<W> tk = child_kmer<W>(e, cv, fwd, av.base);
        uint64_t* out = a.term + st.s * W;
#pragma unroll
        for (int i = 0; i < W; i++) out[i] = tk.w[i];
    }
    cv = av;
    if (cv.npe) { st.status = ST_NULLPTR; return true; }
    return false;
}

LDBG_DEV bool lean_ok(const WalkArgs& a, const StrandState& st) {
    return lean_cursor_ok(a.e, st) && st.gV >= 2 && st.gV <= (uint32_t)a.e.max_len
        && (st.pw.n & (LDBG_PATH_BLOCK - 1)) != 0u;
}
LDBG_DEV bool lean_again(const WalkArgs& a, const StrandState& st, const RunState& rs) {
    return lean_cursor_again(a.e, st) && st.gV <= (uint32_t)a.e.max_len && (st.pw.n & (LDBG_PATH_BLOCK - 1)) != 0u
        && !(a.e.runs.uinfo && run_entry_a(a.e, st, rs));
}
template <int W>
LDBG_DEV void lean_step(const WalkArgs& a, StrandState& st, LinkStoreDev& ls, RunState& rs) {
#ifdef LDBG_LEAN_PROFILE
    const unsigned long long t0 = __builtin_readcyclecounter();
#endif
    const Node av = lean_cursor_advance<W>(a.e, st, ls, &rs.seen_marks);
#ifdef LDBG_LEAN_PROFILE
    if (a.st_gen && a.e.lean_rows) {
        const unsigned long long t3 = __builtin_readcyclecounter();
        a.st_prof[4 * st.s] += st.cu.nxt.p1 - t0; a.st_prof[4 * st.s + 1] += st.cu.nxt.p2 - st.cu.nxt.p1;
        a.st_prof[4 * st.s + 2] += t3 - st.cu.nxt.p2; a.st_prof[4 * st.s + 3] += 1;
    }
#endif
    LDBG_GLOBAL(uint64_t, st.pw.cur)[st.pw.n & (LDBG_PATH_BLOCK - 1)] = pack_vertex(av);
    st.pw.n++;
    st.gV++;
    st.cv = av;
}

template <int W, int BS, bool IMG>
LDBG_WAVE_KERNEL_N(BS) void k_walk(WalkArgs a) {
    const int64_t slot = global_tid();
    if (slot >= a.n_slots) return;
#ifdef LDBG_WALK_DIAG
    if (a.wg_times && threadIdx.x == 0) a.wg_times[2 * blockIdx.x] = __builtin_amdgcn_s_memrealtime();
#endif
    uint32_t kc_run = 0, kc_runv = 0, kc_lean = 0, kc_gen = 0, kc_add = 0, kc_choice = 0, wave_general = 0;
    LinkStoreDev ls;
    LsWave lw;
    lane_link_store<BS>(a, slot, ls, lw);
    WalkLane wl;
    StrandState& st = wl.st;
    st.vt.tab = nullptr; st.vt.mask = 0; st.vt.used = 0; st.status = ST_OK;
    RunState& rs = wl.rs;
    rs.seed_pos = LDBG_RUN_NONE; rs.seen_marks = 0; rs.choices = 0; rs.anchor_at = 0; rs.anchor_gv = 0; rs.anchor_marks = 0; rs.anchor_n = 0; rs.anchor_cap = 0;
    rs.period = 0; rs.anchor_sig = 0; rs.anchor_cv = 0; rs.anchor_t = 0;
    const bool runs_on = a.e.runs.uinfo != nullptr;
    bool active = false, exhausted = false;
    bool suspended = false, begun = true;
    StrandSave* save = (StrandSave*)a.save;
    if constexpr (IMG) active = lane_restore(save[slot], wl, ls, begun);
    uint32_t wave_iterations = 0;
    while (wave_ballot((active && !suspended) || (!active && !exhausted)) != 0ull) {
        if (IMG && a.yield_iters != 0u && wave_iterations >= a.yield_iters) break;
        wave_iterations++;
        if (!active && !exhausted) {
            int64_t skipped = -1;
            const int64_t s = strand_fetch(a, exhausted, &skipped);
            if (skipped >= 0) a.strand_c[skipped] = 0;
            if (s >= 0 && IMG) {
                st.s = s; st.fwd = (s & 1) != 0; active = true; begun = false;
            } else if (s >= 0) {
                active = strand_begin<W>(a, st, ls, s);
                rs.seed_pos = st.cv.idx >= 0 && ui_valid(st.cv.ui) ? ui_pos(st.cv.ui) : LDBG_RUN_NONE;
                rs.seen_marks = 0; rs.choices = 0; rs.anchor_at = 0; rs.period = 0;
                if (!active) walk_finish(a, st);
            }
        }
        if (IMG && active && !suspended) {
            if (!begun) {
                if (!seed_rows_ready<W>(a, st.s, st.fwd)) suspended = true;
                else {
                    begun = true;
                    active = strand_begin<W>(a, st, ls, st.s);
                    rs.seed_pos = LDBG_RUN_NONE; rs.seen_marks = 0; rs.choices = 0; rs.anchor_at = 0; rs.period = 0;
                    if (!active) walk_finish(a, st);
                }
            }
            if (active && begun && !suspended && st.status == ST_OK) {
                const bool ready = (a.e.cursor_on && st.cu.has) ? rows_ready(a.img, st.cu.nxt, st.fwd) : rows_ready(a.img, st.cv, st.fwd);
                if (!ready) suspended = true;
            }
        }
        const bool running = active && begun && !suspended;
#ifdef LDBG_WALK_DIAG
        unsigned long long tc0 = 0;
        if (a.wave_cat) tc0 = __builtin_amdgcn_s_memrealtime();
#endif
        wave_grow_tables(a, st, running);
#ifdef LDBG_WALK_DIAG
        unsigned long long tc1 = 0;
        if (a.wave_cat) tc1 = __builtin_amdgcn_s_memrealtime();
#endif
        bool stepped = false;
        auto run_phase = [&](bool on) {
            if (!(runs_on && on)) return;
            const bool ma = run_mode_a(a, st, rs);
            const bool mb = !ma && run_mode_b(a, st, rs);
            if (ma || mb) {
                stepped = true;
                const uint32_t it0 = st.iters;
                const bool ended = run_step<W>(a, st, ls, rs, ma);
                kc_run++; kc_runv += st.iters - it0;
                if (ended) { walk_finish(a, st); active = false; }
            }
        };
        run_phase(running);
#ifdef LDBG_WALK_DIAG
        unsigned long long tc2 = 0;
        if (a.wave_cat) tc2 = __builtin_amdgcn_s_memrealtime();
#endif
        const bool lean = running && active && (!IMG || !stepped) && lean_ok(a, st) && !(runs_on && run_entry_a(a.e, st, rs));
        if (lean) {
            int r = 0;
            const uint32_t used0 = st.vt.used;
#pragma unroll 1
            do { lean_step<W>(a, st, ls, rs); } while (++r < a.lean_run && lean_again(a, st, rs));
            kc_lean += (uint32_t)r;
            rs.seen_marks += st.vt.used - used0;
            st.cu.cur = st.cv;
        }
#ifdef LDBG_WALK_DIAG
        if (a.wave_cat && threadIdx.x == 0) {
            const unsigned long long tc3 = __builtin_amdgcn_s_memrealtime();
            unsigned long long* wc = a.wave_cat + 16 * blockIdx.x;
            wc[0] += 1; wc[1] += tc1 - tc0; wc[2] += tc2 - tc1; wc[3] += tc3 - tc2;
        }
#endif
        bool general = running && active;
        if (general && (lean || stepped)) {
            if constexpr (IMG) general = false;
            else general = !(runs_on && (run_mode_a(a, st, rs) || run_mode_b(a, st, rs))) && !(lean_ok(a, st) && !(runs_on && run_entry_a(a.e, st, rs)));
        }
        const unsigned long long general_lanes = wave_ballot(general);
        if (general_lanes == 0ull) continue;
        wave_general++;
#ifdef LDBG_WALK_DIAG
        unsigned long long tc4 = 0, tprep[4] = {0, 0, 0, 0};
        if (a.wave_cat) tc4 = __builtin_amdgcn_s_memrealtime();
        const unsigned long long t_general = a.st_gen ? __builtin_amdgcn_s_memrealtime() : 0ull;
#endif
        const bool cur_mode = general && st.status == ST_OK && a.e.cursor_on && st.cu.has;
        StepPre pre;
        const uint32_t used1 = st.vt.used;
#ifdef LDBG_WALK_DIAG
        coop_step_prepare<W>(a.e, st, ls, lw, cur_mode, pre, a.wave_cat ? tprep : nullptr);
        if (a.st_gen && general) {
            a.st_gen[2 * st.s] += __builtin_amdgcn_s_memrealtime() - t_general;
            a.st_gen[2 * st.s + 1] += 1;
        }
        unsigned long long tc5 = 0;
        if (a.wave_cat) tc5 = __builtin_amdgcn_s_memrealtime();
#else
        coop_step_prepare<W>(a.e, st, ls, lw, cur_mode, pre);
#endif
        kc_add += pre.n_added; kc_choice += pre.choice_done ? 1u : 0u;
        if (general) {
            kc_gen++;
            bool ended = strand_step<W>(a, st, ls, pre, rs);
            rs.seen_marks += st.vt.used - used1;
            if (!ended && a.snap && pre.choice_done && st.status == ST_OK) ended = periodic_check(a, st, ls, rs, a.snap + (size_t)slot * LDBG_SNAP_CAP);
            if (ended) { walk_finish(a, st); active = false; }
        }
#ifdef LDBG_WALK_DIAG
        if (a.wave_cat && threadIdx.x == 0) {
            unsigned long long* wc = a.wave_cat + 16 * blockIdx.x;
            const unsigned long long tc6 = __builtin_amdgcn_s_memrealtime();
            wc[4] += 1; wc[5] += tc6 - tc4; wc[6] += tprep[0] - tc4; wc[7] += tprep[1] - tprep[0]; wc[8] += tc5 - tprep[1]; wc[9] += tc6 - tc5;
            wc[10] += (unsigned long long)__builtin_popcountll(general_lanes); wc[11] += tprep[2] & 0xFFFFFFFFull; wc[12] += tprep[2] >> 32;
            wc[13] += tprep[3] & 0xFFFFull; wc[14] += (tprep[3] >> 16) & 0xFFFFull; wc[15] += tprep[3] >> 32;
        }
#endif
    }
    if constexpr (IMG) lane_save(a, save[slot], active, wl, ls, begun);
#ifdef LDBG_WALK_DIAG
    if (a.wg_times && threadIdx.x == 0) a.wg_times[2 * blockIdx.x + 1] = __builtin_amdgcn_s_memrealtime();
#endif
    if (a.kinds) {
        const uint32_t kc[6] = {kc_run, kc_runv, kc_lean, kc_gen, kc_add, kc_choice};
#pragma unroll
        for (int q = 0; q < 6; q++) {
            const uint32_t tot = wave_incl_scan_u32(kc[q]);
            if (wave_lane() == wave_size() - 1 && tot) atomic_add_u64(a.kinds + q, (unsigned long long)tot);
        }
        if (wave_lane() == 0) {
            atomic_add_u64(a.kinds + 6, (unsigned long long)wave_iterations);
            atomic_add_u64(a.kinds + 7, (unsigned long long)wave_general);
            unsigned long long* mx = a.kinds + 8;
            const unsigned long long mine = ((unsigned long long)wave_general << 32) | (unsigned long long)wave_iterations;
#ifndef LDBG_HOSTSIM
            atomicMax(mx, mine);
#else
            if (mine > *mx) *mx = mine;
#endif
        }
    }
}

LDBG_KERNEL void k_seed_words(const unsigned char* ascii, int64_t n, int k, int W, uint64_t* words, uint8_t* valid) {
    const int nw = (k + 31) / 32, lead = W - nw;
    for (int64_t q = global_tid(); q < n; q += global_nthreads()) {
        const unsigned char* c = ascii + q * k;
        uint64_t w[4] = {0ull, 0ull, 0ull, 0ull};
        bool bad = false;
        int i = 0;
        for (int wi = lead; wi < W; wi++) {
            const int cnt = wi == lead ? k - 32 * (nw - 1) : 32;
            uint64_t acc = 0;
            for (int j = 0; j < cnt; j++) {
                unsigned v = 0;
                switch (c[i++]) {
                    case 'A': v = 0; break;
                    case 'C': v = 1; break;
                    case 'G': v = 2; break;
                    case 'T': v = 3; break;
                    default: bad = true; break;
                }
                acc = (acc << 2) | (uint64_t)v;
            }
            w[wi] = acc;
        }
        for (int wi = 0; wi < W; wi++) words[q * W + wi] = bad ? 0ull : w[wi];
        valid[q] = bad ? 0 : 1;
    }
}
LDBG_KERNEL void k_retry_list(const uint32_t* status, int64_t ns, uint32_t* list, unsigned long long* count) {
    for (int64_t s = global_tid(); s < ns; s += global_nthreads())
        if (status[s] == ST_RETRY_PLAIN) list[atomic_add_u64(count, 1ull)] = (uint32_t)s;
}
struct AsmArgs {
    EngineView e;
    int64_t n;
    int op_and, k;
    const uint64_t* seeds;
    const uint64_t* pool; const uint32_t* block_table; int max_blocks;
    const uint32_t* strand_n; const uint32_t* status; const uint32_t* iters; const uint8_t* quirk;
    int64_t* walk_len;
    uint8_t* seed_ok;
    uint32_t* contig_len;
    unsigned long long* flags;
};
LDBG_DEV unsigned long long wave_sum_u64(unsigned long long v) { for (int m = wave_size() >> 1; m > 0; m >>= 1) v += wave_shfl_xor_u64(v, m); return v; }
LDBG_KERNEL void k_walk_lengths(AsmArgs a) {
    const int64_t WS = wave_size(), lane = wave_lane();
    const int64_t wave = global_tid() / WS, nwaves = (global_nthreads() + WS - 1) / WS;
    unsigned long long n_full = 0, n_err = 0, n_quirk = 0, n_iters = 0;
    for (int64_t base = wave * WS; base < a.n; base += nwaves * WS) {
        const int64_t i = base + lane;
        if (i >= a.n) continue;
        const uint32_t sr = a.status[2 * i], sf = a.status[2 * i + 1];
        uint32_t nr = a.strand_n[2 * i], nf = a.strand_n[2 * i + 1];
        bool null_r = sr == ST_BRANCH_NULL, null_f = sf == ST_BRANCH_NULL;
        bool err = (sr != ST_OK && !null_r) || (sf != ST_OK && !null_f);
        bool is_null = a.op_and ? (null_r || null_f) : (null_r && null_f);
        int64_t len = 0;
        uint8_t ok = 0;
        if (!err && !is_null && nr + nf > 0) {
            const int64_t ss = nr > 0 ? 2 * i : 2 * i + 1;
            uint64_t seed_entry = a.pool[(uint64_t)a.block_table[ss * a.max_blocks] * LDBG_PATH_BLOCK];
            int64_t idx = path_idx(seed_entry);
            if (idx >= 0 && (int32_t)graph_cov(a.e.g, idx, a.e.first_trav) > 0) {
                ok = 1;
                len = (int64_t)(nr > 0 ? nr - 1 : 0) + (int64_t)(nf > 0 ? nf - 1 : 0) + 1;
            }
        }
        a.walk_len[i] = len;
        a.seed_ok[i] = ok;
        a.contig_len[i] = len > 0 ? (uint32_t)(len + a.k - 1) : 0u;
        n_full += (sr == ST_POOL_FULL) + (sf == ST_POOL_FULL);
        n_err += (sr != ST_OK && !null_r && sr != ST_POOL_FULL) + (sf != ST_OK && !null_f && sf != ST_POOL_FULL);
        n_quirk += (a.quirk[2 * i] != 0) + (a.quirk[2 * i + 1] != 0);
        n_iters += (unsigned long long)a.iters[2 * i] + a.iters[2 * i + 1];
    }
    n_full = wave_sum_u64(n_full); n_err = wave_sum_u64(n_err); n_quirk = wave_sum_u64(n_quirk); n_iters = wave_sum_u64(n_iters);
    if (lane == 0) {
        if (n_full) atomic_add_u64(a.flags + 0, n_full);
        if (n_err) atomic_add_u64(a.flags + 1, n_err);
        if (n_quirk) atomic_add_u64(a.flags + 2, n_quirk);
        if (n_iters) atomic_add_u64(a.flags + 3, n_iters);
    }
}
#define OFF_SCAN_OWNERS 4096
LDBG_KERNEL void k_off_sums(int64_t n, int64_t chunk, const uint32_t* cnt, unsigned long long* sums) {
    for (int64_t t = global_tid(); t < OFF_SCAN_OWNERS; t += global_nthreads()) {
        const int64_t lo = std::min<int64_t>(t * chunk, n), hi = std::min<int64_t>(lo + chunk, n);
        unsigned long long s = 0;
        for (int64_t i = lo; i < hi; i++) s += cnt[i];
        sums[t] = s;
    }
}
LDBG_KERNEL void k_off_top(unsigned long long* sums, int64_t* total) {
    if (global_tid() / wave_size() != 0) return;
    const int WS = wave_size(), lane = wave_lane(), per = OFF_SCAN_OWNERS / WS;
    unsigned long long mine = 0;
    for (int j = 0; j < per; j++) mine += sums[lane * per + j];
    unsigned long long base = 0, all = 0;
    for (int l = 0; l < WS; l++) { const unsigned long long t = wave_bcast_u64(mine, l); if (l < lane) base += t; all += t; }
    for (int j = 0; j < per; j++) { const unsigned long long v = sums[lane * per + j]; sums[lane * per + j] = base; base += v; }
    if (lane == 0) *total = (int64_t)all;
}
LDBG_KERNEL void k_off_apply(int64_t n, int64_t chunk, const uint32_t* cnt, const unsigned long long* sums, const int64_t* total, int64_t* off) {
    for (int64_t t = global_tid(); t < OFF_SCAN_OWNERS; t += global_nthreads()) {
        const int64_t lo = std::min<int64_t>(t * chunk, n), hi = std::min<int64_t>(lo + chunk, n);
        unsigned long long run = sums[t];
        for (int64_t i = lo; i < hi; i++) { off[i] = (int64_t)run; run += cnt[i]; }
        if (t == 0) off[n] = *total;
    }
}
static void launch_offsets(const uint32_t* d_cnt, int64_t n, int64_t* d_off, unsigned long long* d_tmp, int64_t* d_total, rt::stream_t s) {
    const int64_t chunk = (n + OFF_SCAN_OWNERS - 1) / OFF_SCAN_OWNERS;
    LDBG_LAUNCH(k_off_sums, OFF_SCAN_OWNERS / 256, 256, s, n, chunk, d_cnt, d_tmp);
    LDBG_LAUNCH(k_off_top, 1, 64, s, d_tmp, d_total);
    LDBG_LAUNCH(k_off_apply, OFF_SCAN_OWNERS / 256, 256, s, n, chunk, d_cnt, (const unsigned long long*)d_tmp, (const int64_t*)d_total, d_off);
}


LDBG_KERNEL void k_compact_paths(const uint64_t* pool, const uint32_t* block_table, int max_blocks, const int64_t* strand_off,
                                 int64_t n_strands, uint64_t* dense) {
    const int64_t wave = global_tid() >> 6, lane = global_tid() & 63, nwaves = (global_nthreads() + 63) >> 6;
    for (int64_t s = wave; s < n_strands; s += nwaves) {
        const int64_t o = strand_off[s], n = strand_off[s + 1] - o;
        for (int64_t j = lane; j < n; j += 64)
            dense[o + j] = pool[(uint64_t)block_table[s * max_blocks + j / LDBG_PATH_BLOCK] * LDBG_PATH_BLOCK + (j & (LDBG_PATH_BLOCK - 1))];
    }
}

struct ExpandArgs {
    const uint64_t* pool; const uint32_t* block_table; int max_blocks;
    const uint32_t* strand_c;
    const int64_t* strand_off;
    int64_t n_strands;
    RunIndexView runs;
    uint64_t* dense;
    unsigned* overflow;
};
LDBG_DEV uint64_t expand_stored(const ExpandArgs& a, int64_t s, uint32_t j) {
    return a.pool[(uint64_t)a.block_table[s * a.max_blocks + j / LDBG_PATH_BLOCK] * LDBG_PATH_BLOCK + (j & (LDBG_PATH_BLOCK - 1))];
}
LDBG_KERNEL void k_expand_paths(ExpandArgs a) {
    const int64_t wave = global_tid() / wave_size(), nwaves = (global_nthreads() + wave_size() - 1) / wave_size();
    const uint32_t lane = (uint32_t)wave_lane(), WS = (uint32_t)wave_size();
    for (int64_t s = wave; s < a.n_strands; s += nwaves) {
        const uint32_t nc = a.strand_c[s];
        uint64_t* out = a.dense + a.strand_off[s];
        const bool fwd = (s & 1) != 0;
        uint32_t base_v = 0;
        for (uint32_t j0 = 0; j0 < nc; j0 += WS) {
            const uint32_t j = j0 + lane;
            uint64_t e = 0, prev = 0;
            if (j < nc) {
                e = expand_stored(a, s, j);
                if (j & (LDBG_PATH_BLOCK - 1)) prev = expand_stored(a, s, j - 1);
            }
            const uint32_t cnt = j < nc ? pd_expanded(prev, e) : 0u;
            const uint32_t incl = wave_incl_scan_u32(cnt);
            const uint32_t at = base_v + incl - cnt;
            const bool head = cnt > 0u && pd_is_head(e);
            if (cnt == 1u && !head) out[at] = e;
            unsigned long long hb = wave_ballot(head);
            while (hb) {
                const int L = __builtin_ctzll(hb);
                hb &= hb - 1;
                const uint64_t he = wave_bcast_u64(e, L);
                const uint32_t hat = wave_bcast_u32(at, L);
                const uint32_t hj = j0 + (uint32_t)L;
                const uint64_t payload = expand_stored(a, s, hj + 1);
                const uint32_t len = wave_bcast_u32(cnt, L);
                if (LDBG_PD_KIND(he) == LDBG_PD_RUN) {
                    const uint32_t acopy = (uint32_t)(he >> 20) & 0xFFFFu;
                    const bool asc = (he >> 36) & 1ull, inv = (he >> 37) & 1ull;
                    const uint32_t first = (uint32_t)payload;
                    const int copy = fwd ? (int)acopy : -(int)acopy;
                    for (uint32_t i = lane; i < len; i += WS) {
                        const uint32_t pos = asc ? first + i : first - i;
                        const uint32_t u = a.runs.uo[pos];
                        const unsigned bb = a.runs.ubase[pos];
                        const unsigned b0 = !inv ? (bb & 3u) : 3u - ((bb >> 2) & 3u), b1 = !inv ? ((bb >> 2) & 3u) : 3u - (bb & 3u);
                        out[hat + i] = path_pack((int64_t)(u & 0x7FFFFFFFu), ((u >> 31) != 0u) != inv, fwd ? b1 : b0, copy);
                    }
                } else {
                    wave_fence();
                    const uint32_t first = (uint32_t)payload, period = (uint32_t)(payload >> 32);
                    for (uint32_t i = lane; i < len; i += WS) {
                        const uint32_t o = i % period;
                        const uint64_t s1 = LDBG_GLOBAL(const uint64_t, out)[first + o], s2 = LDBG_GLOBAL(const uint64_t, out)[first + period + o];
                        const int c = path_copy(s2) + (int)(i / period + 1u) * (path_copy(s2) - path_copy(s1));
                        if (c > 32767 || c < -32767) *a.overflow = 1u;
                        out[hat + i] = (s2 & ~(0xFFFFFFull << 36)) | (((uint64_t)(uint32_t)c & 0xFFFFFFull) << 36);
                    }
                }
            }
            base_v += wave_bcast_u32(incl, (int)WS - 1);
        }
    }
}

struct ContigArgs {
    GraphView g;
    int64_t n;
    const uint64_t* seeds;
    const uint64_t* dense;
    const int64_t* strand_off;
    const int64_t* walk_len;
    const int64_t* contig_off;
    const uint8_t* quirk;
    const uint64_t* term;
    char* out;
};
template <int W>
LDBG_DEV Kmer<W> walk_vertex_kmer(const ContigArgs& a, int64_t i, int64_t v, int64_t ro, int64_t nr, int64_t fo) {
    const int64_t nrev = nr > 0 ? nr - 1 : 0;
    uint64_t e;
    const uint64_t* term;
    if (v < nrev) { e = a.dense[ro + (nr - 1 - v)]; term = a.term + (2 * i) * W; }
    else if (v == nrev) { e = nr > 0 ? a.dense[ro] : a.dense[fo]; term = a.seeds + i * W; }
    else { e = a.dense[fo + (v - nrev)]; term = a.term + (2 * i + 1) * W; }
    Kmer<W> km;
    const int64_t ri = path_idx(e);
    if (ri >= 0) { km = graph_key<W>(a.g, ri); if (path_flip(e)) km = kmer_revcomp<W>(km, a.g.k); }
    else { for (int w = 0; w < W; w++) km.w[w] = term[w]; }
    return km;
}
template <int W>
LDBG_KERNEL void k_contigs(ContigArgs a) {
    const int k = a.g.k;
    const int64_t wave = global_tid() >> 6, lane = global_tid() & 63, nwaves = (global_nthreads() + 63) >> 6;
    for (int64_t i = wave; i < a.n; i += nwaves) {
        if (a.walk_len[i] == 0) continue;
        const int64_t L = a.contig_off[i + 1] - a.contig_off[i];
        const int64_t ro = a.strand_off[2 * i], nr = a.strand_off[2 * i + 1] - ro;
        const int64_t fo = a.strand_off[2 * i + 1];
        const int64_t nrev = nr > 0 ? nr - 1 : 0;
        char* o = a.out + a.contig_off[i];
        if (a.quirk[2 * i] | a.quirk[2 * i + 1]) {
            for (int64_t p = lane; p < L; p += 64) {
                const int64_t v = p < k ? 0 : p - k + 1;
                const Kmer<W> km = walk_vertex_kmer<W>(a, i, v, ro, nr, fo);
                o[p] = "ACGT"[kmer_base<W>(km, k, p < k ? (int)p : k - 1)];
            }
            continue;
        }
        Kmer<W> sk;
#pragma unroll
        for (int w = 0; w < W; w++) sk.w[w] = a.seeds[i * W + w];
        for (int64_t p = lane; p < L; p += 64) {
            unsigned b;
            if (p < nrev) b = path_base(a.dense[ro + (nr - 1 - p)]);
            else if (p < nrev + k) b = kmer_base<W>(sk, k, (int)(p - nrev));
            else b = path_base(a.dense[fo + (p - nrev - k + 1)]);
            o[p] = "ACGT"[b];
        }
    }
}

struct ContigRleArgs {
    GraphView g;
    RunIndexView runs;
    int64_t n;
    const uint64_t* seeds;
    const uint64_t* pool; const uint32_t* block_table; int max_blocks;
    const uint32_t* strand_c; const uint32_t* strand_n;
    const int64_t* walk_len; const int64_t* contig_off;
    char* out;
};
LDBG_DEV uint64_t rle_stored(const ContigRleArgs& a, int64_t s, uint32_t j) {
    return a.pool[(uint64_t)a.block_table[s * a.max_blocks + j / LDBG_PATH_BLOCK] * LDBG_PATH_BLOCK + (j & (LDBG_PATH_BLOCK - 1))];
}
template <int W>
LDBG_KERNEL void k_contigs_rle(ContigRleArgs a) {
    const int k = a.g.k;
    const int64_t wave = global_tid() / wave_size(), nwaves = (global_nthreads() + wave_size() - 1) / wave_size();
    const uint32_t lane = (uint32_t)wave_lane(), WS = (uint32_t)wave_size();
    for (int64_t i = wave; i < a.n; i += nwaves) {
        if (a.walk_len[i] == 0) continue;
        char* o = a.out + a.contig_off[i];
        const int64_t nr = a.strand_n[2 * i], nrev = nr > 0 ? nr - 1 : 0;
        Kmer<W> sk;
#pragma unroll
        for (int w = 0; w < W; w++) sk.w[w] = a.seeds[i * W + w];
        for (uint32_t p = lane; p < (uint32_t)k; p += WS) o[nrev + p] = "ACGT"[kmer_base<W>(sk, k, (int)p)];
        for (int dir = 0; dir < 2; dir++) {
            const int64_t s = 2 * i + dir;
            const bool fwd = dir == 1;
            const uint32_t nc = a.strand_c[s];
            auto place = [&](uint32_t v) -> int64_t { return fwd ? nrev + k - 1 + (int64_t)v : nrev - (int64_t)v; };
            uint32_t base_v = 0;
            uint64_t carry = 0;
            for (uint32_t j0 = 0; j0 < nc; j0 += WS) {
                const uint32_t j = j0 + lane;
                const uint64_t* blk = a.pool + (uint64_t)a.block_table[s * a.max_blocks + j0 / LDBG_PATH_BLOCK] * LDBG_PATH_BLOCK;
                const uint64_t e = j < nc ? LDBG_GLOBAL(const uint64_t, blk)[j & (LDBG_PATH_BLOCK - 1)] : 0ull;
                const uint64_t up = wave_shfl_u64(e, (int)lane - 1);
                const uint64_t prev = (j & (LDBG_PATH_BLOCK - 1)) == 0u ? 0ull : (lane == 0u ? carry : up);
                carry = wave_shfl_u64(e, (int)WS - 1);
                const uint32_t cnt = j < nc ? pd_expanded(prev, e) : 0u;
                const uint32_t incl = wave_incl_scan_u32(cnt);
                const uint32_t at = base_v + incl - cnt;
                const bool head = cnt > 0u && pd_is_head(e);
                if (cnt == 1u && !head && at >= 1u) o[place(at)] = "ACGT"[path_base(e)];
                const bool is_run = head && LDBG_PD_KIND(e) == LDBG_PD_RUN;
                unsigned long long hb = wave_ballot(is_run);
                const uint32_t GS = WS == 64u ? 16u : WS, g = lane / GS, sub = lane % GS;
                const uint8_t* ub = LDBG_GLOBAL(const uint8_t, a.runs.ubase);
                while (hb) {
                    uint32_t myL = 0;
                    bool gv = false;
                    for (uint32_t q = 0; q < WS / GS; q++) {
                        if (!hb) break;
                        const int L = __builtin_ctzll(hb);
                        hb &= hb - 1;
                        if (g == q) { myL = (uint32_t)L; gv = true; }
                    }
                    const uint64_t he = wave_shfl_u64(e, (int)myL);
                    const uint32_t hat = wave_shfl_u32(at, (int)myL), len_of = wave_shfl_u32(cnt, (int)myL);
                    const uint32_t len = gv ? len_of : 0u;
                    const uint64_t next_e = wave_shfl_u64(e, (int)myL + 1);
                    const uint64_t payload = !gv ? 0ull : (myL + 1u < WS ? next_e : rle_stored(a, s, j0 + myL + 1u));
                    const bool asc = (he >> 36) & 1ull, inv = (he >> 37) & 1ull;
                    const uint32_t first = (uint32_t)payload;
                    const unsigned shift = (fwd != inv) ? 2u : 0u, comp = inv ? 3u : 0u;
                    auto ascii = [&](unsigned bb) -> unsigned { return (0x54474341u >> (8u * (((bb >> shift) & 3u) ^ comp))) & 0xFFu; };
                    auto ascii4 = [&](uint32_t bb4) -> uint32_t {
                        const uint32_t f = ((bb4 >> shift) & 0x03030303u) ^ (comp * 0x01010101u);
#ifndef LDBG_HOSTSIM
                        return __builtin_amdgcn_perm(0u, 0x54474341u, f);
#else
                        uint32_t v = 0;
                        for (int bI = 0; bI < 4; bI++) v |= ((0x54474341u >> (8u * ((f >> (8 * bI)) & 3u))) & 0xFFu) << (8 * bI);
                        return v;
#endif
                    };
                    const uint8_t* in_lo = asc ? ub + first : ub + first - (len ? len - 1u : 0u);
                    char* out_lo = LDBG_GLOBAL(char, o) + (fwd ? place(hat) : place(hat + (len ? len - 1u : 0u)));
                    const bool same = asc == fwd;
                    const uint32_t nd = len / 8u;
                    uint32_t max_nd = wave_bcast_u32(nd, 0);
                    for (uint32_t q = 1; q < WS / GS; q++) { const uint32_t o2 = wave_bcast_u32(nd, (int)(q * GS)); max_nd = o2 > max_nd ? o2 : max_nd; }
                    for (uint32_t base = 0; base < max_nd; base += 4u * GS) {
                        uint64_t w[4];
#pragma unroll
                        for (int q = 0; q < 4; q++) {
                            const uint32_t ci = base + (uint32_t)q * GS + sub;
                            w[q] = 0;
                            if (ci < nd) __builtin_memcpy(&w[q], in_lo + (same ? 8u * ci : len - 8u - 8u * ci), 8);
                        }
#pragma unroll
                        for (int q = 0; q < 4; q++) {
                            const uint32_t ci = base + (uint32_t)q * GS + sub;
                            uint64_t v = (uint64_t)ascii4((uint32_t)w[q]) | ((uint64_t)ascii4((uint32_t)(w[q] >> 32)) << 32);
                            if (!same) v = __builtin_bswap64(v);
                            if (ci < nd) __builtin_memcpy(out_lo + 8u * ci, &v, 8);
                        }
                    }
                    for (uint32_t t = 8u * nd + sub; t < len; t += GS) {
                        const unsigned bb = in_lo[same ? t : len - 1u - t];
                        out_lo[t] = (char)ascii(bb);
                    }
                }
                hb = wave_ballot(head && !is_run);
                while (hb) {
                    const int L = __builtin_ctzll(hb);
                    hb &= hb - 1;
                    const uint32_t hat = wave_bcast_u32(at, L), len = wave_bcast_u32(cnt, L);
                    const uint64_t payload = (uint32_t)L + 1u < WS ? wave_bcast_u64(e, L + 1) : rle_stored(a, s, j0 + (uint32_t)L + 1);
                    wave_fence();
                    const uint32_t first = (uint32_t)payload, period = (uint32_t)(payload >> 32);
                    const uint32_t nch = (len + 7u) / 8u;
                    for (uint32_t c = lane; c < nch; c += WS) {
                        const uint32_t t0 = 8u * c, m = len - t0 < 8u ? len - t0 : 8u;
                        uint32_t r = t0 % period;
                        uint64_t v = 0;
#pragma unroll
                        for (uint32_t b = 0; b < 8u; b++) {
                            if (b < m) {
                                const uint64_t ch = (uint8_t)LDBG_GLOBAL(const char, o)[place(first + period + r)];
                                v |= ch << (8u * (fwd ? b : m - 1u - b));
                            }
                            r++;
                            if (r == period) r = 0;
                        }
                        char* lo = LDBG_GLOBAL(char, o) + (fwd ? place(hat + t0) : place(hat + t0 + m - 1u));
                        if (m == 8u) __builtin_memcpy(lo, &v, 8);
                        else for (uint32_t b = 0; b < m; b++) lo[b] = (char)(v >> (8u * b));
                    }
                }
                base_v += wave_bcast_u32(incl, (int)WS - 1);
            }
        }
    }
}

template <int W>
LDBG_KERNEL void k_walk_vertices(GraphView g, const uint64_t* dense, int64_t ro, int64_t nr, int64_t fo, int64_t nf,
                                 const uint64_t* term_r, const uint64_t* term_f, int64_t len, uint64_t* words, int64_t* rec,
                                 int32_t* copy, int32_t* index) {
    const int64_t nrev = nr > 0 ? nr - 1 : 0;
    for (int64_t p = global_tid(); p < len; p += global_nthreads()) {
        uint64_t e;
        int idx_label;
        const uint64_t* term;
        if (p < nrev) { e = dense[ro + (nr - 1 - p)]; idx_label = -1; term = term_r; }
        else if (p == nrev) { e = nr > 0 ? dense[ro] : dense[fo]; idx_label = 0; term = nullptr; }
        else { e = dense[fo + (p - nrev)]; idx_label = 1; term = term_f; }
        int64_t ri = path_idx(e);
        Kmer<W> km;
        if (ri >= 0) {
            km = graph_key<W>(g, ri);
            if (path_flip(e)) km = kmer_revcomp<W>(km, g.k);
        } else {
            for (int w = 0; w < W; w++) km.w[w] = term ? term[w] : 0;
        }
        for (int w = 0; w < W; w++) words[p * W + w] = km.w[w];
        rec[p] = ri;
        copy[p] = path_copy(e);
        index[p] = idx_label;
    }
}

struct RoiHitArgs {
    const uint32_t* roi_of;
    int64_t n;
    const uint64_t* dense; const int64_t* strand_off; const int64_t* walk_len;
    unsigned long long* count;
    const int64_t* out_off;
    uint32_t* out;
    uint8_t* has_null;
    int fill;
};
LDBG_KERNEL void k_roi_hits(RoiHitArgs a) {
    const int64_t wave = global_tid() >> 6, lane = global_tid() & 63, nwaves = (global_nthreads() + 63) >> 6;
    for (int64_t i = wave; i < a.n; i += nwaves) {
        const int64_t ro = a.strand_off[2 * i], nr = a.strand_off[2 * i + 1] - ro;
        const int64_t fo = a.strand_off[2 * i + 1], nf = a.strand_off[2 * i + 2] - fo;
        const bool in_walk = a.walk_len[i] > 0;
        bool null_seen = false;
        for (int64_t p = lane; p < nr + nf; p += 64) {
            const bool fwd_part = p >= nr;
            const uint64_t e = a.dense[fwd_part ? fo + (p - nr) : ro + p];
            const int64_t idx = path_idx(e);
            if (idx < 0) { null_seen = true; continue; }
            if (fwd_part && p == nr && nr > 0) continue;
            if (!in_walk) continue;
            const uint32_t r = a.roi_of[idx];
            if (r == 0xFFFFFFFFu) continue;
            const unsigned long long slot = atomic_add_u64(&a.count[i], 1ull);
            if (a.fill) a.out[a.out_off[i] + (int64_t)slot] = r;
        }
        if (!a.fill && null_seen) a.has_null[i] = 1;
    }
}
template <int W>
LDBG_KERNEL void k_roi_of(GraphView g, GraphView rois, uint32_t* roi_of) {
    for (int64_t i = global_tid(); i < rois.N; i += global_nthreads()) {
        GraphView exact = g;
        exact.java_tiny = 0;
        const int64_t idx = graph_find_canonical<W>(exact, graph_key<W>(rois, i));
        if (idx >= 0) roi_of[idx] = (uint32_t)i;
    }
}

Engine::Engine(const ldbg_engine_config& c) : cfg(c) {
    if (c.n_traversal <= 0) throw StatusError(LDBG_ERR_CORTEXJDK, "Traversal color(s) must be specified.");
    if (!c.graph) throw StatusError(LDBG_ERR_CORTEXJDK, "Must provide graph to traverse.");
    graph = (const Graph*)c.graph;
    rois = (const Graph*)c.rois;
    stream_ = graph->stream;
    const int nc = graph->hdr.C;
    auto fail = [&](const char* what, int col) {
        throw StatusError(LDBG_ERR_CORTEXJDK, std::string(what) + " colors must be between 0 and " + std::to_string(nc) + " (provided " + std::to_string(col) + ")");
    };
    for (int i = 0; i < c.n_traversal; i++) if (c.traversal_colors[i] >= nc || c.traversal_colors[i] < 0) fail("Traversal", c.traversal_colors[i]);
    for (int i = 0; i < c.n_joining; i++) if (c.joining_colors[i] < 0 || c.joining_colors[i] >= nc) fail("Joining", c.joining_colors[i]);
    for (int i = 0; i < c.n_recruitment; i++) if (c.recruitment_colors[i] < 0 || c.recruitment_colors[i] >= nc) fail("Recruitment", c.recruitment_colors[i]);
    for (int i = 0; i < c.n_secondary; i++) if (c.secondary_colors[i] < 0 || c.secondary_colors[i] >= nc) fail("Secondary", c.secondary_colors[i]);
    if (c.stopping_rule < 0 || c.stopping_rule >= LDBG_STOP_COUNT) throw StatusError(LDBG_ERR_CORTEXJDK, "Must provide stopping rule for graph traversal");

    rt::set_device(graph->device);
    view.g = graph->view;
    view.trav_mask = view.recruit_mask = view.join_mask = 0;
    for (int i = 0; i < c.n_traversal; i++) view.trav_mask |= 1u << c.traversal_colors[i];
    for (int i = 0; i < c.n_recruitment; i++) view.recruit_mask |= 1u << c.recruitment_colors[i];
    for (int i = 0; i < c.n_joining; i++) view.join_mask |= 1u << c.joining_colors[i];
    view.trav_sel4 = view.recruit_sel4 = 0;
    for (int col = 0; col < 4; col++) {
        if ((view.trav_mask >> col) & 1u) view.trav_sel4 |= 0xFFu << (8 * col);
        if ((view.recruit_mask >> col) & 1u) view.recruit_sel4 |= 0xFFu << (8 * col);
    }
    view.first_trav = c.traversal_colors[0];
    view.stopper = c.stopping_rule;
    view.max_len = c.max_branch_length;
    view.connect_all = c.connect_all_neighbors;
    view.strict_flip = c.strict_java_flip;
    view.lean_rows = (view.g.k & 1) && row_is_packed(view.g) ? 1 : 0;
    for (int i = 0; i < c.nlinks; i++) {
        const Links* l = (const Links*)c.links[i];
        if (!l) continue;
        bool mine = false;
        for (int t = 0; t < c.n_traversal; t++)
            if (!l->sample_names.empty() && l->sample_names[0] == graph->hdr.colors[c.traversal_colors[t]].sample_name) mine = true;
        if (mine) my_links.push_back(l);
    }
    merged_.reset(new MergedLinks(my_links, *graph));
    view.links = merged_->view;
    view.link_flag_mask = merged_->flag_mask;
    view.cursor_on = c.nlinks > 0 ? 1 : 0;
    if (!graph->is_image) {
        rt::set_device(graph->device);
        rt::stream_sync(graph->stream);
        own_stream_ = rt::stream_create();
        if (own_stream_) stream_ = own_stream_;
    }
}
void Engine::enter() {
    rt::set_device(graph->device);
    if (stream_ != graph->stream) rt::stream_sync(graph->stream);
}

Engine::~Engine() { if (own_stream_) { try { rt::set_device(graph->device); } catch (...) {} }
                    sharded_abort(); clear_batch(); drop_batch_seeds(); drop_spares(); rt::hfree_pinned(h_small_); rt::hfree_pinned(h_log_); rt::hfree_pinned(h_stage_[0]); rt::hfree_pinned(h_stage_[1]); release_scratch(); rt::dfree(d_frames_); rt::dfree(d_roi_bits_); rt::dfree(d_roi_of_);
                    if (own_stream_) { quiesce(); rt::stream_destroy(own_stream_); } }

void Engine::walk_roi_hits(int64_t* offsets, uint32_t* hits, int64_t capacity, uint8_t* has_null) {
    if (!rois) throw StatusError(LDBG_ERR_ARG, "walk_roi_hits: the engine has no ROI graph");
    enter();
    rt::stream_t s = stream_;
    const int W = graph->hdr.W;
    if (!d_roi_of_) {
        if (rois->hdr.k != graph->hdr.k) throw StatusError(LDBG_ERR_ARG, "the ROI graph must have the k-mer size of the traversed graph");
        const size_t nrec = (size_t)std::max<int64_t>(1, graph->view.N);
        d_roi_of_ = rt::dmalloc(nrec * 4);
        rt::dmemset(d_roi_of_, 0xFF, nrec * 4, s);
        if (rois->view.N > 0) {
            LDBG_LAUNCH_W(W, k_roi_of, grid_for(rois->view.N), 256, s, graph->view, rois->view, (uint32_t*)d_roi_of_);
        }
    }
    std::vector<std::vector<unsigned long long>> counts(chunks.size());
    int64_t total = 0;
    offsets[0] = 0;
    for (size_t ci = 0; ci < chunks.size(); ci++) {
        WalkChunk& c = chunks[ci];
        RoiHitArgs a;
        ensure_dense(c);
        a.roi_of = (const uint32_t*)d_roi_of_; a.n = c.n; a.dense = (const uint64_t*)c.d_path;
        const int64_t* d_soff = (const int64_t*)c.d_strand_off;
        const int64_t* d_wl = (const int64_t*)c.d_walk_len;
        unsigned long long* d_cnt = (unsigned long long*)rt::dmalloc((size_t)std::max<int64_t>(1, c.n) * 8);
        uint8_t* d_null = (uint8_t*)rt::dmalloc((size_t)std::max<int64_t>(1, c.n));
        rt::dmemset(d_cnt, 0, (size_t)std::max<int64_t>(1, c.n) * 8, s);
        rt::dmemset(d_null, 0, (size_t)std::max<int64_t>(1, c.n), s);
        a.strand_off = d_soff; a.walk_len = d_wl; a.count = d_cnt; a.out_off = nullptr; a.out = nullptr; a.has_null = d_null; a.fill = 0;
        const int grid = grid_for(c.n * 64);
        LDBG_LAUNCH(k_roi_hits, grid, 256, s, a);
        counts[ci].resize((size_t)c.n);
        rt::d2h(counts[ci].data(), d_cnt, (size_t)c.n * 8, s);
        rt::d2h(has_null + c.first, d_null, (size_t)c.n, s);
        rt::stream_sync(s);
        std::vector<int64_t> off((size_t)c.n + 1, 0);
        for (int64_t i = 0; i < c.n; i++) { off[i + 1] = off[i] + (int64_t)counts[ci][i]; offsets[c.first + i + 1] = total + off[i + 1]; }
        const int64_t chunk_total = off[c.n];
        if (total + chunk_total <= capacity && chunk_total > 0) {
            int64_t* d_off = (int64_t*)rt::dmalloc((size_t)(c.n + 1) * 8);
            uint32_t* d_out = (uint32_t*)rt::dmalloc((size_t)chunk_total * 4);
            rt::h2d(d_off, off.data(), (size_t)(c.n + 1) * 8, s);
            rt::dmemset(d_cnt, 0, (size_t)c.n * 8, s);
            a.out_off = d_off; a.out = d_out; a.fill = 1;
            LDBG_LAUNCH(k_roi_hits, grid, 256, s, a);
            rt::d2h(hits + total, d_out, (size_t)chunk_total * 4, s);
            rt::stream_sync(s);
            rt::dfree(d_off); rt::dfree(d_out);
        }
        total += chunk_total;
        rt::dfree(d_cnt); rt::dfree(d_null);
    }
    if (total > capacity) throw StatusError(LDBG_ERR_CAPACITY, "hit buffer too small: need " + std::to_string(total));
}

void Engine::ensure_run_index() {
    if (runs_ || getenv("LDBG_NO_RUNS") || !(view.g.k & 1) || graph->is_image) return;
    runs_.reset(new RunIndex(view, graph->device, stream_));
    profile_add("run_index", runs_->build_ms);
    if (getenv("LDBG_HOST_TIMES"))
        fprintf(stderr, "[ldbg] run index: %lld chains hold %lld of %lld records, built in %.1f ms\n", (long long)runs_->n_chains,
                (long long)runs_->n_in_chains, (long long)view.g.N, runs_->build_ms);
}

void Engine::ensure_dense(WalkChunk& c) {
    if (!c.dense_pending) return;
    enter();
    rt::stream_t s = stream_;
    const int64_t ns = 2 * c.n;
    c.d_path = result_alloc((size_t)std::max<int64_t>(1, c.total_entries) * 8, &c.path_cap);
    unsigned* d_ovf = (unsigned*)rt::dmalloc(4);
    rt::dmemset(d_ovf, 0, 4, s);
    ExpandArgs xa;
    xa.pool = (const uint64_t*)d_pool_; xa.block_table = (const uint32_t*)d_block_table_; xa.max_blocks = c.max_blocks;
    xa.strand_c = (const uint32_t*)c.d_strand_c; xa.strand_off = (const int64_t*)c.d_strand_off; xa.n_strands = ns;
    xa.runs = c.runs; xa.dense = (uint64_t*)c.d_path; xa.overflow = d_ovf;
    LDBG_LAUNCH(k_expand_paths, grid_for(ns * 64, LDBG_STREAM_BLOCK, LDBG_STREAM_GRID), LDBG_STREAM_BLOCK, s, xa);
    unsigned ovf = 0;
    rt::d2h(&ovf, d_ovf, 4, s);
    rt::stream_sync(s);
    rt::dfree(d_ovf);
    c.dense_pending = false;
    if (ovf) throw StatusError(LDBG_ERR_UNSUPPORTED, "a vertex was visited more than 32767 times in one walk");
}
void Engine::materialize_pending() { for (auto& c : chunks) ensure_dense(c); }

LDBG_KERNEL void k_path_lengths(const uint64_t* pool, const uint32_t* block_table, int max_blocks, const uint32_t* strand_c, int64_t n_strands, uint32_t* len) {
    const int64_t wave = global_tid() / wave_size(), nwaves = (global_nthreads() + wave_size() - 1) / wave_size();
    const uint32_t lane = (uint32_t)wave_lane(), WS = (uint32_t)wave_size();
    for (int64_t s = wave; s < n_strands; s += nwaves) {
        const uint32_t nc = strand_c[s];
        uint32_t total = 0;
        for (uint32_t j0 = 0; j0 < nc; j0 += WS) {
            const uint32_t j = j0 + lane;
            uint32_t cnt = 0;
            if (j < nc) {
                const uint64_t* blk = pool + (uint64_t)block_table[s * max_blocks + j / LDBG_PATH_BLOCK] * LDBG_PATH_BLOCK;
                const uint32_t o = j & (LDBG_PATH_BLOCK - 1);
                cnt = pd_expanded(o ? blk[o - 1] : 0ull, blk[o]);
            }
            total += wave_bcast_u32(wave_incl_scan_u32(cnt), (int)WS - 1);
        }
        if (lane == 0) len[s] = total;
    }
}
void Engine::launch_path_lengths(const uint32_t* d_strand_c, int64_t n_strands, int max_blocks, uint32_t* d_len) {
    LDBG_LAUNCH(k_path_lengths, grid_for(n_strands * 64, LDBG_STREAM_BLOCK, LDBG_STREAM_GRID), LDBG_STREAM_BLOCK, stream_, (const uint64_t*)d_pool_, (const uint32_t*)d_block_table_, max_blocks,
                d_strand_c, n_strands, d_len);
}
void Engine::launch_expand_paths(const uint32_t* d_strand_c, const int64_t* d_strand_off, int64_t n_strands, uint64_t* d_dense, int max_blocks, const RunIndexView& runs,
                                 unsigned* d_overflow) {
    ExpandArgs xa;
    xa.pool = (const uint64_t*)d_pool_; xa.block_table = (const uint32_t*)d_block_table_; xa.max_blocks = max_blocks;
    xa.strand_c = d_strand_c; xa.strand_off = d_strand_off; xa.n_strands = n_strands;
    xa.runs = runs; xa.dense = d_dense; xa.overflow = d_overflow;
    LDBG_LAUNCH(k_expand_paths, grid_for(n_strands * 64, LDBG_STREAM_BLOCK, LDBG_STREAM_GRID), LDBG_STREAM_BLOCK, stream_, xa);
}

void Engine::launch_compact_paths(const int64_t* d_strand_off, int64_t n_strands, uint64_t* d_dense, int max_blocks) {
    LDBG_LAUNCH(k_compact_paths, grid_for(n_strands * 64), 256, stream_, (const uint64_t*)d_pool_, (const uint32_t*)d_block_table_, max_blocks,
                d_strand_off, n_strands, d_dense);
}

void Engine::release_scratch() {
    drop_spares();
    rt::dfree(d_vpool_); rt::dfree(d_ls_); rt::dfree(d_snap_); rt::dfree(d_pool_); rt::dfree(d_block_table_);
    d_vpool_ = d_ls_ = d_snap_ = d_pool_ = d_block_table_ = nullptr;
    n_slots_ = 0; n_blocks_ = 0; bt_strands_ = 0; vpool_entries_ = 0; vpool_dirty_ = 0;
}

LDBG_KERNEL void k_zero16(uint64_t* p, uint64_t n_pairs) {
    for (uint64_t i = (uint64_t)global_tid(); i < n_pairs; i += (uint64_t)global_nthreads()) {
#ifndef LDBG_HOSTSIM
        struct alignas(16) U2 { uint64_t a, b; };
        ((U2*)p)[i] = U2{0ull, 0ull};
#else
        p[2 * i] = 0; p[2 * i + 1] = 0;
#endif
    }
}
void Engine::zero_dirty_tables(rt::stream_t s) {
    if (vpool_dirty_ == 0) { vpool_dirty_ = vpool_entries_; return; }
    const uint64_t n = std::min<uint64_t>((vpool_dirty_ + 1) & ~1ull, vpool_entries_ & ~1ull);
    if (n > 0) LDBG_LAUNCH(k_zero16, 256 * 16, 256, s, (uint64_t*)d_vpool_, n / 2);
    if (n < std::min<uint64_t>(vpool_dirty_, vpool_entries_)) rt::dmemset((uint64_t*)d_vpool_ + n, 0, (size_t)(std::min<uint64_t>(vpool_dirty_, vpool_entries_) - n) * 8, s);
    vpool_dirty_ = vpool_entries_;
}

void* Engine::result_alloc(size_t bytes, size_t* cap) {
    int best = -1;
    for (int i = 0; i < (int)spares_.size(); i++)
        if (spares_[i].bytes >= bytes && (best < 0 || spares_[i].bytes < spares_[best].bytes)) best = i;
    if (best >= 0) {
        Spare sp = spares_[best];
        spares_.erase(spares_.begin() + best);
        *cap = sp.bytes;
        return sp.p;
    }
    void* p = nullptr;
    try { p = rt::dmalloc(bytes); }
    catch (const StatusError&) { drop_spares(); p = rt::dmalloc(bytes); }
    *cap = bytes;
    return p;
}
void Engine::result_free(void* p, size_t cap) {
    if (!p) return;
    if (spares_.size() >= 8 || cap == 0) { rt::dfree(p); return; }
    spares_.push_back({p, cap});
}
void Engine::drop_spares() {
    for (auto& sp : spares_) rt::dfree(sp.p);
    spares_.clear();
}

void Engine::quiesce() noexcept {
    try {
        rt::stream_sync(stream_);
        if (sharded_run_ && sharded_stream_ && sharded_stream_ != stream_) rt::stream_sync(sharded_stream_);
    } catch (...) {}
}
void Engine::clear_batch() {
    if (!chunks.empty()) quiesce();
    for (auto& c : chunks) {
        result_free(c.d_path, c.path_cap); result_free(c.d_contigs, c.contigs_cap); rt::tfree(c.d_seed_words); rt::tfree(c.d_term);
        rt::tfree(c.d_strand_c); rt::tfree(c.d_strand_off); rt::tfree(c.d_contig_off); rt::tfree(c.d_walk_len);
    }
    chunks.clear();
    batch_n = batch_bytes = batch_traversed = 0;
}

uint64_t vt_series(uint64_t init, uint64_t vmax) {
    uint64_t c = std::min(init, vmax), sum = 0;
    while (true) { sum += c; if (c >= vmax) break; c = std::min(c * 4, vmax); }
    return sum;
}
uint32_t vt_initial_entries() {
    uint32_t v = LDBG_VT_INITIAL;
    if (const char* ev = getenv("LDBG_VT_INITIAL")) v = std::max<uint32_t>(64u, next_pow2((uint64_t)atoll(ev)));
    return v;
}

void Engine::ensure_scratch(int64_t ns, uint32_t ecap, int max_blocks, uint64_t table_floor, bool small) {
    rt::stream_t s = stream_;
    const uint64_t small_v = (uint64_t)ns * 1024ull * scratch_scale_, small_b = (uint64_t)ns * 2ull * scratch_scale_;
    const bool reusable = d_vpool_ && ecap_ == ecap && max_blocks_ == max_blocks && bt_strands_ >= ns && table_floor_ >= table_floor;
    if (reusable && (scratch_full_ || (small && scratch_scale_ == scratch_scale_built_))) return;
    release_scratch();
    size_t free_b = 0, total_b = 0;
    rt::mem_info(&free_b, &total_b);
    const int64_t slots = ((ns + 63) / 64) * 64;
    const uint64_t vcap_max = next_pow2(2ull * (uint64_t)(cfg.max_branch_length + 12));
    uint64_t want_v = std::max<uint64_t>((uint64_t)ns * vt_series(vt_initial_entries(), vcap_max), table_floor) + LDBG_VT_INITIAL;
    uint64_t want_blocks = (uint64_t)ns * (uint64_t)max_blocks;
    scratch_full_ = !small || (small_v >= want_v && small_b >= want_blocks);
    if (small) { want_v = std::min<uint64_t>(want_v, std::max<uint64_t>(small_v, table_floor) + LDBG_VT_INITIAL); want_blocks = std::min<uint64_t>(want_blocks, std::max<uint64_t>(small_b, 2)); }
    scratch_scale_built_ = scratch_scale_;
    vpool_entries_ = std::max<uint64_t>(LDBG_VT_INITIAL * 2, std::min<uint64_t>(want_v, (uint64_t)(free_b * 0.40) / 8));
    table_floor_ = table_floor;
    n_blocks_ = std::max<uint64_t>(2, std::min<uint64_t>(want_blocks, (uint64_t)(free_b * 0.35) / (LDBG_PATH_BLOCK * 8)));
    d_vpool_ = rt::dmalloc((size_t)vpool_entries_ * 8);
    d_ls_ = rt::dmalloc((size_t)slots * ecap * sizeof(LsElem));
    d_snap_ = rt::dmalloc((size_t)slots * LDBG_SNAP_CAP * sizeof(LsSnap));
    d_pool_ = rt::dmalloc((size_t)n_blocks_ * LDBG_PATH_BLOCK * 8);
    d_block_table_ = rt::dmalloc((size_t)ns * max_blocks * 4);
    rt::dmemset(d_vpool_, 0, (size_t)vpool_entries_ * 8, s);
    vpool_dirty_ = 0;
    n_slots_ = slots; ecap_ = ecap; max_blocks_ = max_blocks; bt_strands_ = ns;
}

struct HostLaps {
    bool on = getenv("LDBG_HOST_TIMES") != nullptr;
    std::chrono::steady_clock::time_point t = std::chrono::steady_clock::now();
    void lap(const char* what) {
        if (!on) return;
        auto n = std::chrono::steady_clock::now();
        fprintf(stderr, "[ldbg] host %-28s %8.3f ms\n", what, std::chrono::duration<double, std::milli>(n - t).count());
        t = n;
    }
};

void Engine::seeds_to_device(const char* seeds, int64_t n, bool seeds_on_device) {
    rt::stream_t s = stream_;
    const int k = graph->hdr.k, W = graph->hdr.W;
    drop_batch_seeds();
    d_batch_words_ = rt::tmalloc((size_t)std::max<int64_t>(1, n) * W * 8);
    d_batch_valid_ = rt::tmalloc((size_t)std::max<int64_t>(1, n));
    if (n <= 0) return;
    if (!seeds_on_device) {
        d_batch_ascii_ = rt::tmalloc((size_t)n * k);
        rt::h2d(d_batch_ascii_, seeds, (size_t)n * k, s);
    }
    LDBG_LAUNCH(k_seed_words, grid_for(n, 256, 1024), 256, s, (const unsigned char*)(seeds_on_device ? (const void*)seeds : d_batch_ascii_), n, k, W,
                (uint64_t*)d_batch_words_, (uint8_t*)d_batch_valid_);
}
void Engine::drop_batch_seeds() {
    if (d_batch_words_ || d_batch_valid_ || d_batch_ascii_) quiesce();
    rt::tfree(d_batch_words_); rt::tfree(d_batch_valid_); rt::tfree(d_batch_ascii_);
    d_batch_words_ = d_batch_valid_ = d_batch_ascii_ = nullptr;
}

void Engine::walk_batch_run(const char* seeds, int64_t n, int64_t* total_bytes, int64_t* traversed, bool seeds_on_device) {
    if (cfg.stopping_rule != LDBG_STOP_CONTIG || cfg.connect_all_neighbors)
        throw StatusError(LDBG_ERR_UNSUPPORTED, "walk_batch runs ContigStopper without connectAllNeighbors; use dfs_batch for other rules");
    if (cfg.n_secondary > 0) throw StatusError(LDBG_ERR_UNSUPPORTED, "secondary colours are not supported by walk_batch");
    enter();
    HostLaps laps;
    clear_batch();
    laps.lap("clear_batch");
    seeds_to_device(seeds, n, seeds_on_device);
    laps.lap("seed words (device)");
    batch_n = n;
    int64_t trav = 0;
    std::vector<std::pair<int64_t, int64_t>> todo{{0, n}};
    while (!todo.empty()) {
        auto [first, cnt] = todo.back();
        todo.pop_back();
        if (cnt <= 0) continue;
        WalkChunk c;
        int64_t t = 0;
        if (run_chunk(first, cnt, c, &t)) { trav += t; chunks.push_back(std::move(c)); }
        else if (!scratch_full_ && scratch_scale_ < (1ull << 24)) {
            scratch_scale_ *= 4;
            pool_growths_++;
            todo.push_back({first, cnt});
        } else {
            if (cnt == 1) throw StatusError(LDBG_ERR_HIP, "path pool too small for a single walk: not enough device memory");
            todo.push_back({first + cnt / 2, cnt - cnt / 2});
            todo.push_back({first, cnt / 2});
        }
    }
    std::sort(chunks.begin(), chunks.end(), [](const WalkChunk& a, const WalkChunk& b) { return a.first < b.first; });
    batch_traversed = trav;
    batch_bytes = 0;
    for (auto& c : chunks) batch_bytes += c.total_bytes;
    if (total_bytes) *total_bytes = batch_bytes;
    if (traversed) *traversed = trav;
}

struct WalkRun {
    WalkArgs a;
    int W = 0, k = 0, block = 64, grid = 1, max_blocks = 0;
    int64_t first = 0, n = 0, ns = 0;
    int64_t refills = 0;
    uint32_t vcap_max = 0;
    bool want_times = false;
    double walk_ms = 0;
    rt::Event ev0, ev1;
    bool timed = false;
    uint32_t *d_strand_n = nullptr, *d_strand_c = nullptr, *d_retry = nullptr, *d_status = nullptr, *d_iters = nullptr;
    uint8_t *d_quirk = nullptr, *d_seed_valid = nullptr;
    unsigned long long* d_ctr = nullptr;
    void* d_save = nullptr;
    WalkChunk out;
    void free_tmp() {
        rt::tfree(d_strand_n); rt::tfree(d_strand_c); rt::tfree(d_retry); rt::tfree(d_seed_valid); rt::tfree(d_status); rt::tfree(d_iters); rt::tfree(d_ctr); rt::tfree(d_quirk);
        rt::dfree(d_save);
        d_strand_n = d_strand_c = d_retry = d_status = d_iters = nullptr; d_quirk = d_seed_valid = nullptr; d_ctr = nullptr; d_save = nullptr;
    }
    void discard() {
        free_tmp();
        rt::tfree(out.d_seed_words); rt::tfree(out.d_term);
        out.d_seed_words = out.d_term = nullptr;
    }
};

static void launch_k_walk(const WalkRun& r, const WalkArgs& a, rt::stream_t s) {
    with_words(r.W, [&](auto w_) {
        constexpr int WW = decltype(w_)::value;
        if (a.img_on) LDBG_LAUNCH((k_walk<WW, 64, true>), r.grid, 64, s, a);
        else if (r.block == 16) LDBG_LAUNCH((k_walk<WW, 16, false>), r.grid, 16, s, a);
        else if (r.block == 64) LDBG_LAUNCH((k_walk<WW, 64, false>), r.grid, 64, s, a);
        else LDBG_LAUNCH((k_walk<WW, 32, false>), r.grid, 32, s, a);
    });
}

void Engine::fill_strand_args(WalkArgs& a, int64_t ns, int max_blocks, uint32_t vcap_max, unsigned long long* d_ctr, ShardImage* img,
                              const int32_t* d_seed_slot, int64_t stride, uint32_t img_yield) {
    a.e = view;
    a.n_strands = ns;
    a.n_slots = std::min<int64_t>(n_slots_, ((ns + 63) / 64) * 64);
    {
        auto gcd = [](int64_t x, int64_t y) { while (y) { int64_t t = x % y; x = y; y = t; } return x; };
        while (gcd(stride, ns) != 1) stride++;
        a.fetch_stride = stride % ns ? stride % ns : 1;
    }
    a.run_rev = cfg.direction == LDBG_DIR_BOTH || cfg.direction == LDBG_DIR_REVERSE;
    a.run_fwd = cfg.direction == LDBG_DIR_BOTH || cfg.direction == LDBG_DIR_FORWARD;
    a.next_strand = d_ctr; a.next_block = d_ctr + 1; a.vnext = d_ctr + 2; a.unfinished = d_ctr + 4;
    a.pool = (uint64_t*)d_pool_; a.n_blocks = n_blocks_;
    a.block_table = (uint32_t*)d_block_table_; a.max_blocks = max_blocks;
    a.vpool = (uint64_t*)d_vpool_; a.vpool_entries = vpool_entries_; a.vcap_max = vcap_max; a.vcap_init = vt_initial_entries();
    a.ls = (LsElem*)d_ls_; a.ecap = ecap_;
    a.retry = nullptr;
    a.img_on = img ? 1 : 0;
    a.seed_slot = d_seed_slot;
    if (img) a.img = img->view((uint64_t*)view.links.rec_of);
    a.yield_iters = img ? img_yield : 0u;
    if (const char* ev = getenv("LDBG_IMG_YIELD")) a.yield_iters = img ? (uint32_t)std::max(0, atoi(ev)) : 0u;
}

void Engine::walk_prepare(int64_t first, int64_t n, WalkRun& r, ShardImage* img, const int32_t* d_seed_slot) {
    rt::stream_t s = stream_;
    WalkArgs& a = r.a;
    const int W = r.W = graph->hdr.W;
    const int64_t ns = r.ns = 2 * n;
    r.k = graph->hdr.k; r.first = first; r.n = n;
    r.out.first = first; r.out.n = n;
    r.vcap_max = std::max<uint32_t>(64u, next_pow2(2ull * (uint64_t)(cfg.max_branch_length + 12)));
    r.max_blocks = (int)(((int64_t)cfg.max_branch_length + 2 + LDBG_PATH_BLOCK - 1) / LDBG_PATH_BLOCK);
    HostLaps laps;
    const bool lean_pools = !img && (view.g.k & 1) && !getenv("LDBG_NO_RUNS") && !getenv("LDBG_VT_INITIAL") && !getenv("LDBG_FULL_POOLS");
    ensure_scratch(ns, link_store_capacity, r.max_blocks, 0, lean_pools);
    zero_dirty_tables(s);
    laps.lap("scratch + zero (issued)");

    r.out.d_seed_words = rt::tmalloc((size_t)n * W * 8);
    rt::d2d(r.out.d_seed_words, (const uint64_t*)d_batch_words_ + first * W, (size_t)n * W * 8, s);
    r.d_seed_valid = (uint8_t*)rt::tmalloc((size_t)n);
    rt::d2d(r.d_seed_valid, (const uint8_t*)d_batch_valid_ + first, (size_t)n, s);
    r.out.d_term = rt::tmalloc((size_t)ns * W * 8);
    r.d_strand_n = (uint32_t*)rt::tmalloc((size_t)ns * 4);
    r.d_strand_c = (uint32_t*)rt::tmalloc((size_t)ns * 4);
    r.d_status = (uint32_t*)rt::tmalloc((size_t)ns * 4);
    r.d_iters = (uint32_t*)rt::tmalloc((size_t)ns * 4);
    r.d_quirk = (uint8_t*)rt::tmalloc((size_t)ns);
    r.d_ctr = (unsigned long long*)rt::tmalloc(256);
    rt::dmemset(r.d_ctr, 0, 256, s);
    rt::dmemset(r.out.d_term, 0, (size_t)ns * W * 8, s);

    laps.lap("small allocations");
    int64_t stride = kFetchStride;
    if (const char* ev = getenv("LDBG_FETCH_STRIDE")) stride = std::max<int64_t>(1, atoll(ev));
    fill_strand_args(a, ns, r.max_blocks, r.vcap_max, r.d_ctr, img, d_seed_slot, stride, kWalkImgYield);
    if (!img) ensure_run_index();
    if (runs_ && !img) a.e.runs = runs_->view;
    a.save = nullptr;
    a.kinds = r.d_ctr + 8;
    if (img) {
        r.d_save = rt::dmalloc((size_t)std::max<int64_t>(64, n_slots_) * sizeof(StrandSave));
        rt::dmemset(r.d_save, 0, (size_t)std::max<int64_t>(64, n_slots_) * sizeof(StrandSave), s);
        a.save = r.d_save;
    }
    a.seeds = (const uint64_t*)r.out.d_seed_words;
    a.seed_valid = r.d_seed_valid;
    if (const char* ev = getenv("LDBG_MAX_SLOTS")) a.n_slots = std::max<int64_t>(64, std::min<int64_t>(a.n_slots, (atoll(ev) / 64) * 64));
    a.lean_run = 4;
    a.grow_at = 2;
    if (const char* ev = getenv("LDBG_VT_GROW_AT")) a.grow_at = (int)std::max<long long>(2, std::min<long long>(8, atoll(ev)));
    if (const char* ev = getenv("LDBG_LEAN_RUN")) a.lean_run = (int)std::max<long long>(1, atoll(ev));
    a.strand_n = r.d_strand_n; a.strand_c = r.d_strand_c; a.status = r.d_status; a.iters = r.d_iters; a.quirk = r.d_quirk;
    a.term = (uint64_t*)r.out.d_term;
    if (!getenv("LDBG_VT_INITIAL")) {
        if (runs_ && !img) {
            a.vcap_init = std::min<uint32_t>(512u, r.vcap_max);
        } else {
            const uint64_t per = vpool_entries_ / 2 / (uint64_t)std::max<int64_t>(1, ns);
            while ((uint64_t)a.vcap_init * 4 <= per && (uint64_t)a.vcap_init * 4 <= r.vcap_max) a.vcap_init *= 4;
        }
    }
    a.snap = getenv("LDBG_NO_REPEAT") ? nullptr : (LsSnap*)d_snap_;

    a.wg_times = nullptr; a.st_times = nullptr; a.st_gen = nullptr; a.wave_cat = nullptr;
#ifdef LDBG_WALK_DIAG
    a.ls_diag = nullptr;
    r.want_times = getenv("LDBG_WG_TIMES") != nullptr && !img;
#else
    r.want_times = false;
#endif
    int& block = r.block;
    block = 64;
    if (const char* ev = getenv("LDBG_WALK_BLOCK")) block = atoi(ev) == 16 ? 16 : (atoi(ev) == 32 ? 32 : 64);
    int wg_per_cu = 4;
    if (!img) wg_per_cu = with_words(W, [&](auto w_) {
        constexpr int WW = decltype(w_)::value;
        return block == 16 ? rt::blocks_per_cu(k_walk<WW, 16, false>, 16) : (block == 64 ? rt::blocks_per_cu(k_walk<WW, 64, false>, 64) : rt::blocks_per_cu(k_walk<WW, 32, false>, 32));
    });
    if (const char* ev = getenv("LDBG_WG_PER_CU")) wg_per_cu = std::max(1, std::min(wg_per_cu, atoi(ev)));
    a.n_slots = std::min<int64_t>(a.n_slots, (int64_t)wg_per_cu * rt::cu_count(graph->device) * block);
    a.n_slots = (a.n_slots / block) * block;
    if (a.n_slots < block) a.n_slots = block;
    const int grid = r.grid = (int)((a.n_slots + block - 1) / block);
    r.refills = std::max<int64_t>(0, (a.run_rev && a.run_fwd ? ns : ns / 2) - a.n_slots);
    if (r.want_times) {
        a.wg_times = (unsigned long long*)rt::dmalloc((size_t)grid * 16); rt::dmemset(a.wg_times, 0, (size_t)grid * 16, s);
        a.st_times = (unsigned long long*)rt::dmalloc((size_t)ns * 16); rt::dmemset(a.st_times, 0, (size_t)ns * 16, s);
        a.st_gen = (unsigned long long*)rt::dmalloc((size_t)ns * 16); rt::dmemset(a.st_gen, 0, (size_t)ns * 16, s);
        a.wave_cat = (unsigned long long*)rt::dmalloc((size_t)grid * 128); rt::dmemset(a.wave_cat, 0, (size_t)grid * 128, s);
#ifdef LDBG_LEAN_PROFILE
        a.st_prof = (unsigned long long*)rt::dmalloc((size_t)ns * 32); rt::dmemset(a.st_prof, 0, (size_t)ns * 32, s);
#endif
#ifdef LDBG_WALK_DIAG
        a.ls_diag = (unsigned long long*)rt::dmalloc((size_t)grid * 16); rt::dmemset(a.ls_diag, 0, (size_t)grid * 16, s);
#endif
    }
}

void Engine::walk_launch(WalkRun& r) {
    rt::stream_t s = stream_;
    r.ev0.record(s);
    launch_k_walk(r, r.a, s);
    r.ev1.record(s);
    r.timed = true;
}

static void walk_report_times(WalkRun& r, const std::vector<uint32_t>& iters, const unsigned long long* ctr, rt::stream_t s) {
    const WalkArgs& a = r.a;
    const int grid = r.grid;
    const int64_t ns = r.ns;
    std::vector<unsigned long long> t((size_t)grid * 2);
    rt::d2h(t.data(), a.wg_times, (size_t)grid * 16, s);
    rt::stream_sync(s);
    unsigned long long t0 = ~0ull;
    for (int i = 0; i < grid; i++) t0 = std::min(t0, t[2 * i]);
    std::vector<double> st(grid), en(grid);
    for (int i = 0; i < grid; i++) { st[i] = (t[2 * i] - t0) / 1e5; en[i] = (t[2 * i + 1] - t0) / 1e5; }
    std::vector<double> ss = st, ee = en;
    std::sort(ss.begin(), ss.end()); std::sort(ee.begin(), ee.end());
    fprintf(stderr, "[ldbg] k_walk workgroups=%d start ms p0/p50/p90/p100 = %.2f %.2f %.2f %.2f ; end ms p0/p50/p90/p100 = %.2f %.2f %.2f %.2f\n",
            grid, ss[0], ss[grid / 2], ss[grid * 9 / 10], ss[grid - 1], ee[0], ee[grid / 2], ee[grid * 9 / 10], ee[grid - 1]);
    rt::dfree(a.wg_times);
    {
        std::vector<unsigned long long> wc((size_t)grid * 16);
        rt::d2h(wc.data(), a.wave_cat, (size_t)grid * 128, s);
        rt::stream_sync(s);
        rt::dfree(a.wave_cat);
        unsigned long long sum[16] = {0};
        int slowest = 0;
        for (int i = 0; i < grid; i++) { for (int q = 0; q < 16; q++) sum[q] += wc[16 * i + q]; if (en[i] > en[slowest]) slowest = i; }
        auto line = [&](const char* who, const unsigned long long* w, double div) {
            fprintf(stderr, "[ldbg] %s: %.0f loop iterations; table regrowth %.2f ms, run steps %.2f ms, lean runs %.2f ms; %.0f with a general part, %.2f ms (%.1f us each)\n", who,
                    w[0] / div, w[1] / 1e5 / div, w[2] / 1e5 / div, w[3] / 1e5 / div, w[4] / div, w[5] / 1e5 / div, w[4] ? w[5] / 100.0 / w[4] : 0.0);
            const double g = w[4] ? (double)w[4] : 1.0;
            fprintf(stderr, "[ldbg] %s: general part per iteration: prefetch %.2f us, adds %.2f us, choices %.2f us, step %.2f us; lanes %.1f, add owners %.2f, choice owners %.2f\n", who,
                    w[6] / 100.0 / g, w[7] / 100.0 / g, w[8] / 100.0 / g, w[9] / 100.0 / g, w[10] / g, w[11] / g, w[12] / g);
            fprintf(stderr, "[ldbg] %s: add owners in 16-lane groups %.2f per iteration, of which a store of <= 8 elements %.2f; elements per add owner (store + records) %.1f\n", who,
                    w[13] / g, w[14] / g, w[11] ? (double)w[15] / (double)w[11] : 0.0);
        };
        line("average wavefront", sum, (double)grid);
        line("slowest wavefront", &wc[16 * (size_t)slowest], 1.0);
#ifdef LDBG_WALK_DIAG
        std::vector<unsigned long long> lc((size_t)grid * 2);
        rt::d2h(lc.data(), a.ls_diag, (size_t)grid * 16, s);
        rt::stream_sync(s);
        rt::dfree(a.ls_diag);
        unsigned long long all = 0, tail = 0;
        for (int i = 0; i < grid; i++) { all += lc[2 * i]; tail += lc[2 * i + 1]; }
        fprintf(stderr, "[ldbg] link-store element reads and writes: %llu, of which in the HBM tail (element %u and up) %llu = %.4f %%; slowest wavefront %llu of %llu\n",
                all, (unsigned)LDBG_LS_FAST, tail, all ? 100.0 * (double)tail / (double)all : 0.0, lc[2 * (size_t)slowest + 1], lc[2 * (size_t)slowest]);
#endif
    }
    std::vector<unsigned long long> tt((size_t)ns * 2);
    rt::d2h(tt.data(), a.st_times, (size_t)ns * 16, s);
    rt::stream_sync(s);
    std::vector<int64_t> order(ns);
    for (int64_t i = 0; i < ns; i++) order[i] = i;
    std::sort(order.begin(), order.end(), [&](int64_t x, int64_t y) { return tt[2 * x + 1] - tt[2 * x] > tt[2 * y + 1] - tt[2 * y]; });
    std::vector<unsigned long long> gen((size_t)ns * 2);
    rt::d2h(gen.data(), a.st_gen, (size_t)ns * 16, s);
    rt::stream_sync(s);
    rt::dfree(a.st_gen);
#ifdef LDBG_LEAN_PROFILE
    {
        std::vector<unsigned long long> pr((size_t)ns * 4);
        rt::d2h(pr.data(), a.st_prof, (size_t)ns * 32, s);
        rt::stream_sync(s);
        rt::dfree(a.st_prof);
        for (int j = 0; j < 6 && j < ns; j++) {
            int64_t i = order[j];
            double n = (double)std::max<unsigned long long>(1, pr[4 * i + 3]);
            fprintf(stderr, "[ldbg] strand %lld lean steps %.0f: cycles per step issue %.0f, wait %.0f, rest %.0f\n", (long long)i, n, pr[4 * i] / n, pr[4 * i + 1] / n, pr[4 * i + 2] / n);
        }
    }
#endif
    for (int j = 0; j < 3 && j < ns; j++) {
        int64_t i = order[j];
        fprintf(stderr, "[ldbg] strand %lld: %llu of its %u steps went through the general step, %.1f ms there (%.2f us each, the step itself not included)\n",
                (long long)i, gen[2 * i + 1], iters[i], gen[2 * i] / 1e5, gen[2 * i + 1] ? gen[2 * i] / 100.0 / gen[2 * i + 1] : 0.0);
    }
    for (int j = 0; j < 12 && j < ns; j++) {
        int64_t i = order[j];
        double ms = (tt[2 * i + 1] - tt[2 * i]) / 1e5;
        fprintf(stderr, "[ldbg] slow strand %lld (seed %lld %s): %.1f ms, %u iterations, %.2f us/iter, lane %lld of its wave, status %u\n", (long long)i, (long long)(r.first + i / 2),
                (i & 1) ? "fwd" : "rev", ms, iters[i], iters[i] ? ms * 1e3 / iters[i] : 0.0, (long long)(i & 63), r.out.status[i]);
    }
    {
        std::vector<double> us;
        uint32_t max_it = 0;
        for (int64_t i = 0; i < ns; i++) max_it = std::max(max_it, iters[i]);
        for (int64_t i = 0; i < ns; i++) if (iters[i] == max_it && max_it > 0) us.push_back((tt[2 * i + 1] - tt[2 * i]) / 100.0 / max_it);
        std::sort(us.begin(), us.end());
        if (!us.empty())
            fprintf(stderr, "[ldbg] %zu strands of %u iterations: us/iter p0/p10/p50/p90/p100 = %.2f %.2f %.2f %.2f %.2f\n", us.size(), max_it,
                    us[0], us[us.size() / 10], us[us.size() / 2], us[us.size() * 9 / 10], us.back());
    }
    double tot_ms = 0; for (int64_t i = 0; i < ns; i++) tot_ms += (tt[2 * i + 1] - tt[2 * i]) / 1e5;
    fprintf(stderr, "[ldbg] sum of strand durations %.1f s over %lld strands; %llu wavefront loop iterations in %d wavefronts\n", tot_ms / 1e3, (long long)ns,
            ctr[14], grid);
    rt::dfree(a.st_times);
}

bool Engine::walk_finish(WalkRun& r, int64_t* traversed) {
    rt::stream_t s = stream_;
    const WalkArgs& a = r.a;
    WalkChunk& out = r.out;
    const int64_t n = r.n, ns = r.ns;
    HostLaps laps;

    if (!h_small_) h_small_ = (unsigned long long*)rt::hmalloc_pinned(64 * 8);
    unsigned long long* const ctr = h_small_;
    if (runs_ && !a.img_on) {
        r.d_retry = (uint32_t*)rt::tmalloc((size_t)ns * 4);
        LDBG_LAUNCH(k_retry_list, grid_for(ns, 256, 1024), 256, s, (const uint32_t*)r.d_status, ns, r.d_retry, r.d_ctr + 28);
        rt::d2h(ctr, r.d_ctr, 256, s);
        rt::stream_sync(s);
        if (r.timed) { r.walk_ms += rt::Event::elapsed_ms(r.ev0, r.ev1); r.timed = false; }
        const int64_t n_again = (int64_t)ctr[28];
        if (n_again > 0) {
            rt::dmemset(r.d_ctr, 0, 8, s);
            WalkArgs b = a;
            b.e.runs = RunIndexView{nullptr, nullptr, nullptr};
            b.retry = r.d_retry;
            b.n_strands = n_again;
            retried_strands_ += n_again;
            r.refills += std::max<int64_t>(0, n_again - b.n_slots);
            launch_k_walk(r, b, s);
        }
    }

    int64_t* d_walk_len = (int64_t*)rt::tmalloc((size_t)n * 8);
    uint8_t* d_seed_ok = (uint8_t*)rt::tmalloc((size_t)n);
    uint32_t* d_contig_len = (uint32_t*)rt::tmalloc((size_t)n * 4);
    int64_t* d_strand_off = (int64_t*)rt::tmalloc((size_t)(ns + 1) * 8);
    int64_t* d_contig_off = (int64_t*)rt::tmalloc((size_t)(n + 1) * 8);
    unsigned long long* d_scan = (unsigned long long*)rt::tmalloc((size_t)(2 * OFF_SCAN_OWNERS + 2) * 8);
    auto free_results = [&] {
        rt::tfree(d_walk_len); rt::tfree(d_seed_ok); rt::tfree(d_contig_len); rt::tfree(d_strand_off); rt::tfree(d_contig_off); rt::tfree(d_scan);
        d_walk_len = nullptr; d_seed_ok = nullptr; d_contig_len = nullptr; d_strand_off = nullptr; d_contig_off = nullptr; d_scan = nullptr;
    };
    AsmArgs aa;
    aa.e = view; aa.n = n; aa.op_and = cfg.combination_operator == LDBG_OP_AND; aa.k = r.k;
    aa.seeds = a.seeds; aa.pool = a.pool; aa.block_table = a.block_table; aa.max_blocks = r.max_blocks;
    aa.strand_n = r.d_strand_n; aa.status = r.d_status; aa.iters = r.d_iters; aa.quirk = r.d_quirk;
    aa.walk_len = d_walk_len; aa.seed_ok = d_seed_ok; aa.contig_len = d_contig_len; aa.flags = r.d_ctr + 24;
    LDBG_LAUNCH(k_walk_lengths, grid_for(n, 256, 2048), 256, s, aa);
    int64_t* d_totals = (int64_t*)(d_scan + 2 * OFF_SCAN_OWNERS);
    launch_offsets(r.d_strand_n, ns, d_strand_off, d_scan, d_totals, s);
    launch_offsets(d_contig_len, n, d_contig_off, d_scan + OFF_SCAN_OWNERS, d_totals + 1, s);
    rt::d2h(ctr, r.d_ctr, 256, s);
    rt::d2h(ctr + 32, d_totals, 16, s);
    rt::stream_sync(s);
    if (r.timed) { r.walk_ms += rt::Event::elapsed_ms(r.ev0, r.ev1); r.timed = false; }
    {
        static const char* const kind_names[8] = {"walk_steps_run", "walk_run_vertices", "walk_steps_lean", "walk_steps_general", "walk_link_adds", "walk_choices",
                                                  "walk_wave_iterations", "walk_wave_general"};
        for (int q = 0; q < 8; q++) profile_add(kind_names[q], (double)ctr[8 + q]);
        profile_add("walk_busiest_general", (double)(ctr[16] >> 32));
        profile_add("walk_busiest_iterations", (double)(ctr[16] & 0xFFFFFFFFull));
        profile_add("walk_wavefronts", (double)r.grid);
        profile_add("walk_refills", (double)r.refills);
    }
    const bool pool_full = ctr[24] != 0, any_error = ctr[25] != 0, any_quirk = ctr[26] != 0;
    if (r.want_times || any_error) {
        std::vector<uint32_t> iters;
        out.status.resize(ns);
        rt::d2h(out.status.data(), r.d_status, (size_t)ns * 4, s);
        if (r.want_times) { iters.resize(ns); rt::d2h(iters.data(), r.d_iters, (size_t)ns * 4, s); }
        rt::stream_sync(s);
        if (r.want_times) walk_report_times(r, iters, ctr, s);
    }
    vpool_dirty_ = ctr[2];
    profile_add("walk", r.walk_ms);
    laps.lap("launch .. results on host");

    if (pool_full) {
        r.discard(); free_results();
        return false;
    }
    if (any_error) {
        for (int64_t i = 0; i < ns; i++) {
            const uint32_t st = out.status[i];
            if (st != ST_NULLPTR && st != ST_LINKSTORE_FULL && st != ST_COPY_OVERFLOW) continue;
            r.discard(); free_results();
            if (st == ST_NULLPTR)
                throw StatusError(LDBG_ERR_NULLPOINTER, "getNextVertices: record missing while recruitment colours are set (seed " + std::to_string(r.first + i / 2) + ")");
            if (st == ST_LINKSTORE_FULL) throw StatusError(LDBG_ERR_CAPACITY, "LINKSTORE_FULL");
            throw StatusError(LDBG_ERR_UNSUPPORTED, "a vertex was visited more than 32767 times in one walk");
        }
    }
    *traversed += (int64_t)ctr[27];
    out.total_entries = (int64_t)ctr[32];
    out.total_bytes = (int64_t)ctr[33];
    out.host_ready = false;

    const bool lazy = !any_quirk && r.first == 0 && n == batch_n && !getenv("LDBG_EAGER_PATHS");
    out.d_contigs = result_alloc((size_t)out.total_bytes, &out.contigs_cap);
    out.d_strand_off = d_strand_off; d_strand_off = nullptr;
    out.d_contig_off = d_contig_off;
    out.d_walk_len = d_walk_len;
    out.d_strand_c = r.d_strand_c; r.d_strand_c = nullptr;
    out.max_blocks = r.max_blocks;
    out.runs = a.e.runs;
    out.dense_pending = true;
    laps.lap("result buffers");
    rt::Event c0, c1;
    c0.record(s);
    if (lazy) {
        ContigRleArgs ra;
        ra.g = graph->view; ra.runs = a.e.runs; ra.n = n; ra.seeds = a.seeds;
        ra.pool = (const uint64_t*)d_pool_; ra.block_table = (const uint32_t*)d_block_table_; ra.max_blocks = r.max_blocks;
        ra.strand_c = (const uint32_t*)out.d_strand_c; ra.strand_n = r.d_strand_n; ra.walk_len = d_walk_len; ra.contig_off = d_contig_off;
        ra.out = (char*)out.d_contigs;
        int rb = LDBG_STREAM_BLOCK, rcap = LDBG_STREAM_GRID;
#ifndef LDBG_HOSTSIM
        if (const char* ev = getenv("LDBG_RLE_BLOCK")) rb = atoi(ev) >= 256 ? 256 : (atoi(ev) >= 128 ? 128 : 64);
        if (const char* ev = getenv("LDBG_RLE_GRID")) rcap = std::max(1, atoi(ev));
#endif
        LDBG_LAUNCH_W(r.W, k_contigs_rle, grid_for(n * 64, rb, rcap), rb, s, ra);
    } else {
        ensure_dense(out);
        ContigArgs ca;
        ca.g = graph->view; ca.n = n; ca.seeds = a.seeds; ca.dense = (const uint64_t*)out.d_path; ca.strand_off = (const int64_t*)out.d_strand_off;
        ca.walk_len = d_walk_len; ca.contig_off = d_contig_off; ca.quirk = r.d_quirk; ca.term = (const uint64_t*)out.d_term;
        ca.out = (char*)out.d_contigs;
        LDBG_LAUNCH_W(r.W, k_contigs, grid_for(n * 64), 256, s, ca);
    }
    c1.record(s);
    rt::stream_sync(s);
    profile_add("contig", rt::Event::elapsed_ms(c0, c1));
    laps.lap("paths + contigs");
    r.free_tmp();
    d_walk_len = nullptr; d_contig_off = nullptr;
    free_results();
    laps.lap("frees");
    return true;
}


void Engine::sharded_walk_begin(ShardImage& img, const char* seeds, int64_t n, const int32_t* d_seed_slot, rt::stream_t round_stream) {
    if (cfg.stopping_rule != LDBG_STOP_CONTIG || cfg.connect_all_neighbors || cfg.n_secondary > 0)
        throw StatusError(LDBG_ERR_UNSUPPORTED, "walks over a sharded table run ContigStopper without connectAllNeighbors / secondary colours");
    if (&img.graph() != graph) throw StatusError(LDBG_ERR_ARG, "the engine was not created on this image's graph");
    enter();
    sharded_abort();
    clear_batch();
    seeds_to_device(seeds, n, false);
    batch_n = n;
    sharded_run_ = new WalkRun;
    sharded_img_ = &img;
    sharded_stream_ = round_stream ? round_stream : stream_;
    try {
        walk_prepare(0, n, *sharded_run_, &img, d_seed_slot);
        rt::stream_sync(stream_);
    } catch (...) { sharded_abort(); throw; }
}
void Engine::sharded_abort() {
    if (sharded_run_) {
        quiesce();
        sharded_run_->discard();
        delete sharded_run_;
        sharded_run_ = nullptr;
    }
    sharded_img_ = nullptr;
}
void Engine::sharded_walk_round(int64_t* d_stats) {
    if (!sharded_run_) throw StatusError(LDBG_ERR_ARG, "sharded_walk_round without sharded_walk_begin");
    enter();
    WalkRun& r = *sharded_run_;
    rt::stream_t s = sharded_stream_;
    rt::dmemset(r.d_ctr + 4, 0, 8, s);
    sharded_img_->reset_requests(s);
    launch_k_walk(r, r.a, s);
    sharded_img_->round_stats(r.d_ctr, r.ns, d_stats, s);
    sharded_rounds_++;
}
void Engine::sharded_walk_finish(int64_t* total_bytes, int64_t* traversed) {
    if (!sharded_run_) throw StatusError(LDBG_ERR_ARG, "sharded_walk_finish without sharded_walk_begin");
    enter();
    WalkRun& r = *sharded_run_;
    rt::stream_sync(sharded_stream_);
    profile_add("walk_rounds", (double)sharded_rounds_);
    sharded_rounds_ = 0;
    int64_t trav = 0;
    bool ok = false;
    try { ok = walk_finish(r, &trav); } catch (...) { sharded_abort(); throw; }
    if (!ok) { sharded_abort(); throw StatusError(LDBG_ERR_CAPACITY, "path pool exhausted during a walk over a sharded table: use smaller batches"); }
    chunks.push_back(std::move(r.out));
    r.out = WalkChunk();
    sharded_abort();
    batch_traversed = trav;
    batch_bytes = chunks.back().total_bytes;
    if (total_bytes) *total_bytes = batch_bytes;
    if (traversed) *traversed = trav;
}

bool Engine::run_chunk(int64_t first, int64_t n, WalkChunk& out, int64_t* traversed) {
    WalkRun r;
    try {
        walk_prepare(first, n, r, nullptr, nullptr);
        walk_launch(r);
        const bool ok = walk_finish(r, traversed);
        if (ok) out = std::move(r.out);
        r.free_tmp();
        return ok;
    } catch (...) { quiesce(); r.free_tmp(); throw; }
}

#define LDBG_STAGE_BYTES ((size_t)32 << 20)
void Engine::download(char* dst, const void* d_src, size_t bytes) {
    rt::stream_t s = stream_;
    if (bytes == 0) return;
    if (bytes < ((size_t)4 << 20) || rt::host_is_pinned(dst)) { rt::d2h(dst, d_src, bytes, s); rt::stream_sync(s); return; }
    for (int b = 0; b < 2; b++) if (!h_stage_[b]) h_stage_[b] = rt::hmalloc_pinned(LDBG_STAGE_BYTES);
    const size_t nchunks = (bytes + LDBG_STAGE_BYTES - 1) / LDBG_STAGE_BYTES;
    rt::Event landed[2];
    auto scatter = [&](size_t c) {
        const size_t off = c * LDBG_STAGE_BYTES, len = std::min(LDBG_STAGE_BYTES, bytes - off);
        const char* src = (const char*)h_stage_[c & 1];
        const int T = 4;
        std::thread th[T - 1];
        auto part = [&](int t) { const size_t lo = len * (size_t)t / T, hi = len * (size_t)(t + 1) / T; memcpy(dst + off + lo, src + lo, hi - lo); };
        for (int t = 1; t < T; t++) th[t - 1] = std::thread(part, t);
        part(0);
        for (int t = 1; t < T; t++) th[t - 1].join();
    };
    for (size_t c = 0; c < nchunks; c++) {
        const size_t off = c * LDBG_STAGE_BYTES, len = std::min(LDBG_STAGE_BYTES, bytes - off);
        rt::d2h(h_stage_[c & 1], (const char*)d_src + off, len, s);
        landed[c & 1].record(s);
        if (c > 0) { landed[(c - 1) & 1].wait(); scatter(c - 1); }
    }
    landed[(nchunks - 1) & 1].wait();
    scatter(nchunks - 1);
}

void Engine::ensure_host(WalkChunk& c) {
    if (c.host_ready) return;
    rt::stream_t s = stream_;
    c.strand_off.resize((size_t)(2 * c.n + 1));
    c.contig_off.resize((size_t)(c.n + 1));
    c.walk_len.resize((size_t)c.n);
    rt::d2h(c.strand_off.data(), c.d_strand_off, (size_t)(2 * c.n + 1) * 8, s);
    rt::d2h(c.contig_off.data(), c.d_contig_off, (size_t)(c.n + 1) * 8, s);
    rt::d2h(c.walk_len.data(), c.d_walk_len, (size_t)c.n * 8, s);
    rt::stream_sync(s);
    c.host_ready = true;
}

void Engine::walk_batch_fetch(char* arena, int64_t cap, int64_t* offsets, int64_t* walk_len) {
    enter();
    if (offsets || walk_len) for (auto& c : chunks) ensure_host(c);
    if (offsets) {
        int64_t o = 0;
        offsets[0] = 0;
        for (auto& c : chunks)
            for (int64_t i = 0; i < c.n; i++) { o += c.contig_off[i + 1] - c.contig_off[i]; offsets[c.first + i + 1] = o; }
    }
    if (walk_len) for (auto& c : chunks) for (int64_t i = 0; i < c.n; i++) walk_len[c.first + i] = c.walk_len[i];
    if (cap < batch_bytes) throw StatusError(LDBG_ERR_CAPACITY, "contig arena too small: need " + std::to_string(batch_bytes) + " bytes");
    if (arena) {
        int64_t o = 0;
        for (auto& c : chunks) {
            download(arena + o, c.d_contigs, (size_t)c.total_bytes);
            o += c.total_bytes;
        }
    }
}

void Engine::walk_vertices(int64_t walk, int64_t capacity, int64_t* len, uint64_t* words, int64_t* rec, int32_t* copy, int32_t* index) {
    enter();
    if (walk < 0 || walk >= batch_n) throw StatusError(LDBG_ERR_ARG, "walk index out of range");
    const int W = graph->hdr.W;
    for (auto& c : chunks) {
        if (walk < c.first || walk >= c.first + c.n) continue;
        int64_t i = walk - c.first;
        ensure_host(c);
        int64_t L = c.walk_len[i];
        *len = L;
        if (L == 0) return;
        if (capacity < L) throw StatusError(LDBG_ERR_CAPACITY, "vertex buffers too small: need " + std::to_string(L));
        ensure_dense(c);
        rt::stream_t s = stream_;
        uint64_t* d_words = (uint64_t*)rt::dmalloc((size_t)L * W * 8);
        int64_t* d_rec = (int64_t*)rt::dmalloc((size_t)L * 8);
        int32_t* d_copy = (int32_t*)rt::dmalloc((size_t)L * 4);
        int32_t* d_index = (int32_t*)rt::dmalloc((size_t)L * 4);
        int64_t ro = c.strand_off[2 * i], nr = c.strand_off[2 * i + 1] - ro, fo = c.strand_off[2 * i + 1], nf = c.strand_off[2 * i + 2] - fo;
        const uint64_t* tr = (const uint64_t*)c.d_term + (2 * i) * W;
        const uint64_t* tf = (const uint64_t*)c.d_term + (2 * i + 1) * W;
        LDBG_LAUNCH_W(W, k_walk_vertices, grid_for(L, 256, 1024), 256, s, graph->view, (const uint64_t*)c.d_path, ro, nr, fo, nf, tr, tf, L, d_words, d_rec, d_copy, d_index);
        if (words) rt::d2h(words, d_words, (size_t)L * W * 8, s);
        if (rec) rt::d2h(rec, d_rec, (size_t)L * 8, s);
        if (copy) rt::d2h(copy, d_copy, (size_t)L * 4, s);
        if (index) rt::d2h(index, d_index, (size_t)L * 4, s);
        rt::stream_sync(s);
        rt::dfree(d_words); rt::dfree(d_rec); rt::dfree(d_copy); rt::dfree(d_index);
        return;
    }
}

}

#ifdef LDBG_HOSTSIM
extern "C" unsigned ldbg_hostsim_ls_peak(void) { const unsigned p = ::ldbg::ls_peak_elements(); ::ldbg::ls_peak_elements() = 0; return p; }
extern "C" unsigned ldbg_hostsim_ls_fast(void) { return (unsigned)LDBG_LS_FAST; }
extern "C" unsigned long long ldbg_hostsim_group_tail(void) { const unsigned long long n = ::ldbg::group_tail_accesses(); ::ldbg::group_tail_accesses() = 0; return n; }
#endif
```

Before: 193.0 billion.

## Overlap contig RLE kernel with next walk batch via double-buffered path pools

Runs the contig run-length expansion kernel on a separate low-priority stream and double-buffers the path pool and block table, so the next walk batch can start while the previous batch's contigs are still being produced. Deferred buffers are retired per generation and freed once that generation's completion event fires. Every result consumer now calls results_wait to keep ordering correct. The cost is a second path pool and block table per engine, plus extra synchronisation points that could serialise work again if they are hit often.

```diff
diff --git a/corticall_amd/csrc/capi.cpp b/corticall_amd/csrc/capi.cpp
--- a/corticall_amd/csrc/capi.cpp
+++ b/corticall_amd/csrc/capi.cpp
@@ -19,6 +19,7 @@
 int64_t join_ctx_files(const std::vector<std::string>& paths, const std::string& out_path, int device);
 std::vector<uint8_t> join_ctx_image(const std::vector<std::string>& paths, int device, bool find_view);
 void profile_reset_all();
+void profile_flush_pending();
 bool profile_get(const char* family, double* ms, int64_t* n);
 }
 
@@ -617,6 +618,7 @@
 ldbg_status ldbg_engine_dfs_batch(ldbg_engine* e, const char* sources, int64_t n, const char* sinks, const int64_t* sink_offsets, ldbg_dfs_result** out) {
     return guard([&] {
         *out = nullptr;
+        e->e.results_wait();
         for (int attempt = 0;; attempt++) {
             try {
                 std::unique_ptr<DfsBatch> b(e->e.dfs_batch(sources, n, sinks, sink_offsets));
@@ -710,6 +712,7 @@
 ldbg_status ldbg_engine_dfs_kmers_traversed(const ldbg_engine* e, int64_t* n) { return guard([&] { *n = e->e.dfs_traversed(); }); }
 
 static CursorHost& cursor_of(ldbg_engine* e) {
+    e->e.results_wait();
     if (!e->cursor) e->cursor.reset(new CursorHost(e->e));
     return *e->cursor;
 }
@@ -727,6 +730,7 @@
     return guard([&] {
         if (!e || !out) throw StatusError(LDBG_ERR_ARG, "cursor batch: null engine or result pointer");
         *out = nullptr;
+        e->e.results_wait();
         if (!e->cursor_batch) e->cursor_batch.reset(new CursorBatchHost(e->e));
         std::unique_ptr<CursorBatchResult> r(e->cursor_batch->run(seeds, n, on_device, direction, max_steps, stop));
         *out = new ldbg_cursor_result{std::move(r)};
@@ -775,10 +779,9 @@
 #ifdef LDBG_HOSTSIM
 extern "C" void ldbg_hostsim_set_lanes(int n) { int v = 1; while (v * 2 <= n && v < 64) v *= 2; ::ldbg::sim::lanes_setting() = v; }
 #endif
-ldbg_status ldbg_profile_reset(void) { profile_reset_all(); return LDBG_OK; }
+ldbg_status ldbg_profile_reset(void) { return guard([&] { profile_flush_pending(); profile_reset_all(); }); }
 ldbg_status ldbg_profile_get(const char* family, double* total_ms, int64_t* launches) {
-    profile_get(family, total_ms, launches);
-    return LDBG_OK;
-}
-
-}
+    return guard([&] { profile_flush_pending(); profile_get(family, total_ms, launches); });
+}
+
+}
diff --git a/corticall_amd/csrc/engine_host.h b/corticall_amd/csrc/engine_host.h
--- a/corticall_amd/csrc/engine_host.h
+++ b/corticall_amd/csrc/engine_host.h
@@ -28,6 +28,8 @@
     int max_blocks = 0;
     RunIndexView runs{};
     bool dense_pending = false;
+    int pool_set = 0;
+    bool deferred = false;
 };
 
 struct DfsVertex { int64_t rec; int64_t slot; int32_t copy, index; uint8_t flip; };
@@ -97,6 +99,8 @@
     void enter();
     rt::stream_t estream() const { return stream_; }
     void quiesce() noexcept;
+    void results_wait();
+    void flush_contig_times(bool block);
     void walk_roi_hits(int64_t* offsets, uint32_t* hits, int64_t capacity, uint8_t* has_null);
     void sharded_walk_begin(ShardImage& img, const char* seeds, int64_t n, const int32_t* d_seed_slot, rt::stream_t round_stream);
     void sharded_walk_round(int64_t* d_stats);
@@ -118,6 +122,21 @@
     rt::stream_t stream_ = nullptr, own_stream_ = nullptr;
     void* d_vpool_ = nullptr; void* d_ls_ = nullptr; void* d_snap_ = nullptr;
     void* d_pool_ = nullptr; void* d_block_table_ = nullptr;
+    void* d_pool_set_[2] = {nullptr, nullptr}; void* d_bt_set_[2] = {nullptr, nullptr};
+    int cur_set_ = 0;
+    rt::stream_t result_stream_ = nullptr;
+    struct Spare { void* p; size_t bytes; };
+    struct ContigGen {
+        rt::Event c0, c1;
+        bool pending = false;
+        bool timed = false;
+        void* d_strand_n = nullptr;
+        std::vector<void*> retired;
+        std::vector<Spare> retired_arenas;
+    };
+    std::unique_ptr<ContigGen> gens_[2];
+    void gen_complete(ContigGen& g);
+    void sync_own_stream() noexcept;
     int64_t n_slots_ = 0, bt_strands_ = 0;
     uint64_t n_blocks_ = 0, vpool_entries_ = 0, vpool_dirty_ = 0;
     uint32_t ecap_ = 0;
@@ -150,14 +169,13 @@
     void launch_expand_paths(const uint32_t* d_strand_c, const int64_t* d_strand_off, int64_t n_strands, uint64_t* d_dense, int max_blocks, const RunIndexView& runs,
                              unsigned* d_overflow);
     void ensure_run_index();
-    void ensure_scratch(int64_t n_strands, uint32_t ecap, int max_blocks, uint64_t table_floor = 0, bool small = false);
+    void ensure_scratch(int64_t n_strands, uint32_t ecap, int max_blocks, uint64_t table_floor = 0, bool small = false, bool two_sets = false);
     uint64_t scratch_scale_ = 1, scratch_scale_built_ = 1; bool scratch_full_ = true; int64_t pool_growths_ = 0;
     uint64_t table_floor_ = 0;
     void* h_stage_[2] = {nullptr, nullptr};
     void download(char* dst, const void* d_src, size_t bytes);
     uint64_t* h_log_ = nullptr; size_t h_log_cap_ = 0;
     void release_scratch();
-    struct Spare { void* p; size_t bytes; };
     std::vector<Spare> spares_;
     void* result_alloc(size_t bytes, size_t* cap);
     void result_free(void* p, size_t cap);
diff --git a/corticall_amd/csrc/rt.h b/corticall_amd/csrc/rt.h
--- a/corticall_amd/csrc/rt.h
+++ b/corticall_amd/csrc/rt.h
@@ -4,6 +4,9 @@
 #include <string.h>
 
 #include <algorithm>
+#include <atomic>
+#include <deque>
+#include <functional>
 #include <map>
 #include <mutex>
 #include <string>
@@ -124,8 +127,16 @@
 }
 typedef hipStream_t stream_t;
 inline stream_t stream_create() { hipStream_t s; check(hipStreamCreateWithFlags(&s, hipStreamNonBlocking), "hipStreamCreate"); return s; }
+inline stream_t stream_create_low() {
+    int least = 0, greatest = 0;
+    check(hipDeviceGetStreamPriorityRange(&least, &greatest), "hipDeviceGetStreamPriorityRange");
+    hipStream_t s;
+    check(hipStreamCreateWithPriority(&s, hipStreamNonBlocking, least), "hipStreamCreateWithPriority");
+    return s;
+}
 inline void stream_destroy(stream_t s) { if (s) (void)hipStreamDestroy(s); }
 inline void stream_sync(stream_t s) { check(hipStreamSynchronize(s), "hipStreamSynchronize"); }
+template <class F> inline void launch_deferred(stream_t, F&& f) { f(); }
 inline void h2d(void* d, const void* h, size_t n, stream_t s) { if (n) check(hipMemcpyAsync(d, h, n, hipMemcpyHostToDevice, s), "hipMemcpyAsync H2D"); }
 inline void d2h(void* h, const void* d, size_t n, stream_t s) { if (n) check(hipMemcpyAsync(h, d, n, hipMemcpyDeviceToHost, s), "hipMemcpyAsync D2H"); }
 inline void d2d(void* d, const void* s_, size_t n, stream_t s) { if (n) check(hipMemcpyAsync(d, s_, n, hipMemcpyDeviceToDevice, s), "hipMemcpyAsync D2D"); }
@@ -159,6 +170,13 @@
     Event& operator=(const Event&) = delete;
     void record(stream_t s) { check(hipEventRecord(e, s), "hipEventRecord"); }
     void wait() { check(hipEventSynchronize(e), "hipEventSynchronize"); }
+    bool done() {
+        const hipError_t r = hipEventQuery(e);
+        if (r == hipErrorNotReady) { (void)hipGetLastError(); return false; }
+        check(r, "hipEventQuery");
+        return true;
+    }
+    void stream_wait(stream_t s) { check(hipStreamWaitEvent(s, e, 0), "hipStreamWaitEvent"); }
     static float elapsed_ms(Event& a, Event& b) {
         check(hipEventSynchronize(b.e), "hipEventSynchronize");
         float ms = 0;
@@ -244,9 +262,49 @@
 inline void hfree_pinned(void* p) { free(p); }
 inline bool host_is_pinned(const void*) { return getenv("LDBG_HOSTSIM_PAGEABLE") == nullptr; }
 typedef void* stream_t;
+struct HeldStream {
+    std::mutex m;
+    std::deque<std::function<void()>> held;
+    uint64_t queued = 0, ran = 0;
+    void run_upto(uint64_t upto) {
+        std::lock_guard<std::mutex> g(m);
+        while (ran < upto && !held.empty()) { std::function<void()> f = std::move(held.front()); held.pop_front(); ran++; f(); deferred_late()++; }
+    }
+    static std::atomic<uint64_t>& deferred_held() { static std::atomic<uint64_t> n{0}; return n; }
+    static std::atomic<uint64_t>& deferred_late() { static std::atomic<uint64_t> n{0}; return n; }
+};
+struct HeldStreams { std::mutex m; std::vector<HeldStream*> live; };
+inline HeldStreams& held_streams() { static HeldStreams h; return h; }
+inline HeldStream* held_of(stream_t s) {
+    if (!s) return nullptr;
+    HeldStreams& hs = held_streams();
+    std::lock_guard<std::mutex> g(hs.m);
+    return std::find(hs.live.begin(), hs.live.end(), (HeldStream*)s) != hs.live.end() ? (HeldStream*)s : nullptr;
+}
 inline stream_t stream_create() { return nullptr; }
-inline void stream_destroy(stream_t) {}
-inline void stream_sync(stream_t) {}
+inline stream_t stream_create_low() {
+    HeldStream* h = new HeldStream;
+    HeldStreams& hs = held_streams();
+    std::lock_guard<std::mutex> g(hs.m);
+    hs.live.push_back(h);
+    return h;
+}
+inline void stream_sync(stream_t s) { if (HeldStream* h = held_of(s)) h->run_upto(~0ull); }
+inline void stream_destroy(stream_t s) {
+    HeldStream* h = held_of(s);
+    if (!h) return;
+    h->run_upto(~0ull);
+    { HeldStreams& hs = held_streams(); std::lock_guard<std::mutex> g(hs.m); hs.live.erase(std::find(hs.live.begin(), hs.live.end(), h)); }
+    delete h;
+}
+template <class F> inline void launch_deferred(stream_t s, F&& f) {
+    HeldStream* h = held_of(s);
+    if (!h) { f(); return; }
+    std::lock_guard<std::mutex> g(h->m);
+    h->held.emplace_back(std::forward<F>(f));
+    h->queued++;
+    HeldStream::deferred_held()++;
+}
 inline void h2d(void* d, const void* h, size_t n, stream_t) { if (n) memcpy(d, h, n); }
 inline void d2h(void* h, const void* d, size_t n, stream_t) { if (n) memcpy(h, d, n); }
 inline void d2d(void* d, const void* s, size_t n, stream_t) { if (n) memmove(d, s, n); }
@@ -258,9 +316,16 @@
     *free_b = mb << 20; *total_b = mb << 20;
 }
 struct Event {
-    void record(stream_t) {}
-    void wait() {}
-    static float elapsed_ms(Event&, Event&) { return 0.0f; }
+    HeldStream* st = nullptr;
+    uint64_t upto = 0;
+    void record(stream_t s) {
+        st = held_of(s);
+        if (st) { std::lock_guard<std::mutex> g(st->m); upto = st->queued; }
+    }
+    void wait() { if (st) st->run_upto(upto); }
+    bool done() { if (!st) return true; std::lock_guard<std::mutex> g(st->m); return st->ran >= upto; }
+    void stream_wait(stream_t) { wait(); }
+    static float elapsed_ms(Event&, Event& b) { b.wait(); return 0.0f; }
 };
 }
 }
diff --git a/corticall_amd/csrc/walk.cpp b/corticall_amd/csrc/walk.cpp
--- a/corticall_amd/csrc/walk.cpp
+++ b/corticall_amd/csrc/walk.cpp
@@ -736,6 +736,37 @@
     }
 }
 
+namespace {
+std::mutex g_engines_mu;
+std::vector<Engine*> g_engines;
+}
+void profile_flush_pending() {
+    std::lock_guard<std::mutex> l(g_engines_mu);
+    for (Engine* e : g_engines) e->flush_contig_times(true);
+}
+void Engine::flush_contig_times(bool block) {
+    for (auto& g : gens_) {
+        if (!g || !g->timed || (!block && !g->c1.done())) continue;
+        g->timed = false;
+        profile_add("contig", rt::Event::elapsed_ms(g->c0, g->c1));
+    }
+}
+void Engine::gen_complete(ContigGen& g) {
+    if (g.pending) { g.c1.wait(); g.pending = false; }
+    {
+        std::lock_guard<std::mutex> l(g_engines_mu);
+        if (g.timed) { g.timed = false; profile_add("contig", rt::Event::elapsed_ms(g.c0, g.c1)); }
+    }
+    rt::tfree(g.d_strand_n); g.d_strand_n = nullptr;
+    for (void* p : g.retired) rt::tfree(p);
+    g.retired.clear();
+    for (auto& sp : g.retired_arenas) result_free(sp.p, sp.bytes);
+    g.retired_arenas.clear();
+}
+void Engine::results_wait() {
+    for (auto& g : gens_) if (g) gen_complete(*g);
+}
+
 Engine::Engine(const ldbg_engine_config& c) : cfg(c) {
     if (c.n_traversal <= 0) throw StatusError(LDBG_ERR_CORTEXJDK, "Traversal color(s) must be specified.");
     if (!c.graph) throw StatusError(LDBG_ERR_CORTEXJDK, "Must provide graph to traverse.");
@@ -786,20 +817,28 @@
         rt::stream_sync(graph->stream);
         own_stream_ = rt::stream_create();
         if (own_stream_) stream_ = own_stream_;
+        result_stream_ = rt::stream_create_low();
+        for (auto& g : gens_) g.reset(new ContigGen);
+        std::lock_guard<std::mutex> l(g_engines_mu);
+        g_engines.push_back(this);
     }
 }
 void Engine::enter() {
     rt::set_device(graph->device);
     if (stream_ != graph->stream) rt::stream_sync(graph->stream);
-}
-
-Engine::~Engine() { if (own_stream_) { try { rt::set_device(graph->device); } catch (...) {} }
+    if (result_stream_) { std::lock_guard<std::mutex> l(g_engines_mu); flush_contig_times(false); }
+}
+
+Engine::~Engine() { if (own_stream_ || result_stream_) { try { rt::set_device(graph->device); } catch (...) {} }
+                    try { results_wait(); } catch (...) {}
+                    if (result_stream_) { std::lock_guard<std::mutex> l(g_engines_mu); g_engines.erase(std::find(g_engines.begin(), g_engines.end(), this)); }
                     sharded_abort(); clear_batch(); drop_batch_seeds(); drop_spares(); rt::hfree_pinned(h_small_); rt::hfree_pinned(h_log_); rt::hfree_pinned(h_stage_[0]); rt::hfree_pinned(h_stage_[1]); release_scratch(); rt::dfree(d_frames_); rt::dfree(d_roi_bits_); rt::dfree(d_roi_of_);
-                    if (own_stream_) { quiesce(); rt::stream_destroy(own_stream_); } }
+                    if (own_stream_ || result_stream_) { quiesce(); rt::stream_destroy(own_stream_); rt::stream_destroy(result_stream_); } }
 
 void Engine::walk_roi_hits(int64_t* offsets, uint32_t* hits, int64_t capacity, uint8_t* has_null) {
     if (!rois) throw StatusError(LDBG_ERR_ARG, "walk_roi_hits: the engine has no ROI graph");
     enter();
+    results_wait();
     rt::stream_t s = stream_;
     const int W = graph->hdr.W;
     if (!d_roi_of_) {
@@ -864,13 +903,14 @@
 void Engine::ensure_dense(WalkChunk& c) {
     if (!c.dense_pending) return;
     enter();
+    results_wait();
     rt::stream_t s = stream_;
     const int64_t ns = 2 * c.n;
     c.d_path = result_alloc((size_t)std::max<int64_t>(1, c.total_entries) * 8, &c.path_cap);
     unsigned* d_ovf = (unsigned*)rt::dmalloc(4);
     rt::dmemset(d_ovf, 0, 4, s);
     ExpandArgs xa;
-    xa.pool = (const uint64_t*)d_pool_; xa.block_table = (const uint32_t*)d_block_table_; xa.max_blocks = c.max_blocks;
+    xa.pool = (const uint64_t*)d_pool_set_[c.pool_set]; xa.block_table = (const uint32_t*)d_bt_set_[c.pool_set]; xa.max_blocks = c.max_blocks;
     xa.strand_c = (const uint32_t*)c.d_strand_c; xa.strand_off = (const int64_t*)c.d_strand_off; xa.n_strands = ns;
     xa.runs = c.runs; xa.dense = (uint64_t*)c.d_path; xa.overflow = d_ovf;
     LDBG_LAUNCH(k_expand_paths, grid_for(ns * 64, LDBG_STREAM_BLOCK, LDBG_STREAM_GRID), LDBG_STREAM_BLOCK, s, xa);
@@ -881,7 +921,7 @@
     c.dense_pending = false;
     if (ovf) throw StatusError(LDBG_ERR_UNSUPPORTED, "a vertex was visited more than 32767 times in one walk");
 }
-void Engine::materialize_pending() { for (auto& c : chunks) ensure_dense(c); }
+void Engine::materialize_pending() { results_wait(); for (auto& c : chunks) ensure_dense(c); }
 
 LDBG_KERNEL void k_path_lengths(const uint64_t* pool, const uint32_t* block_table, int max_blocks, const uint32_t* strand_c, int64_t n_strands, uint32_t* len) {
     const int64_t wave = global_tid() / wave_size(), nwaves = (global_nthreads() + wave_size() - 1) / wave_size();
@@ -921,9 +961,12 @@
 }
 
 void Engine::release_scratch() {
+    try { results_wait(); } catch (...) {}
     drop_spares();
-    rt::dfree(d_vpool_); rt::dfree(d_ls_); rt::dfree(d_snap_); rt::dfree(d_pool_); rt::dfree(d_block_table_);
+    rt::dfree(d_vpool_); rt::dfree(d_ls_); rt::dfree(d_snap_);
+    for (int i = 0; i < 2; i++) { rt::dfree(d_pool_set_[i]); rt::dfree(d_bt_set_[i]); d_pool_set_[i] = d_bt_set_[i] = nullptr; }
     d_vpool_ = d_ls_ = d_snap_ = d_pool_ = d_block_table_ = nullptr;
+    cur_set_ = 0;
     n_slots_ = 0; n_blocks_ = 0; bt_strands_ = 0; vpool_entries_ = 0; vpool_dirty_ = 0;
 }
 
@@ -971,15 +1014,26 @@
     spares_.clear();
 }
 
+void Engine::sync_own_stream() noexcept { try { rt::stream_sync(stream_); } catch (...) {} }
 void Engine::quiesce() noexcept {
     try {
         rt::stream_sync(stream_);
+        if (result_stream_) rt::stream_sync(result_stream_);
         if (sharded_run_ && sharded_stream_ && sharded_stream_ != stream_) rt::stream_sync(sharded_stream_);
     } catch (...) {}
 }
 void Engine::clear_batch() {
-    if (!chunks.empty()) quiesce();
+    bool pending = false;
+    for (auto& c : chunks) if (c.deferred && gens_[c.pool_set] && gens_[c.pool_set]->pending) pending = true;
+    if (!chunks.empty() && !pending) quiesce();
     for (auto& c : chunks) {
+        if (c.deferred && gens_[c.pool_set] && gens_[c.pool_set]->pending) {
+            ContigGen& g = *gens_[c.pool_set];
+            if (c.d_path) g.retired_arenas.push_back({c.d_path, c.path_cap});
+            if (c.d_contigs) g.retired_arenas.push_back({c.d_contigs, c.contigs_cap});
+            for (void* p : {c.d_seed_words, c.d_term, c.d_strand_c, c.d_strand_off, c.d_contig_off, c.d_walk_len}) if (p) g.retired.push_back(p);
+            continue;
+        }
         result_free(c.d_path, c.path_cap); result_free(c.d_contigs, c.contigs_cap); rt::tfree(c.d_seed_words); rt::tfree(c.d_term);
         rt::tfree(c.d_strand_c); rt::tfree(c.d_strand_off); rt::tfree(c.d_contig_off); rt::tfree(c.d_walk_len);
     }
@@ -998,15 +1052,16 @@
     return v;
 }
 
-void Engine::ensure_scratch(int64_t ns, uint32_t ecap, int max_blocks, uint64_t table_floor, bool small) {
+void Engine::ensure_scratch(int64_t ns, uint32_t ecap, int max_blocks, uint64_t table_floor, bool small, bool two_sets) {
     rt::stream_t s = stream_;
     const uint64_t small_v = (uint64_t)ns * 1024ull * scratch_scale_, small_b = (uint64_t)ns * 2ull * scratch_scale_;
     const bool reusable = d_vpool_ && ecap_ == ecap && max_blocks_ == max_blocks && bt_strands_ >= ns && table_floor_ >= table_floor;
-    if (reusable && (scratch_full_ || (small && scratch_scale_ == scratch_scale_built_))) return;
+    if (reusable && (scratch_full_ || (small && scratch_scale_ == scratch_scale_built_)) && (!two_sets || d_pool_set_[1] || scratch_full_)) return;
     release_scratch();
     size_t free_b = 0, total_b = 0;
     rt::mem_info(&free_b, &total_b);
     const int64_t slots = ((ns + 63) / 64) * 64;
+    const int sets = two_sets ? 2 : 1;
     const uint64_t vcap_max = next_pow2(2ull * (uint64_t)(cfg.max_branch_length + 12));
     uint64_t want_v = std::max<uint64_t>((uint64_t)ns * vt_series(vt_initial_entries(), vcap_max), table_floor) + LDBG_VT_INITIAL;
     uint64_t want_blocks = (uint64_t)ns * (uint64_t)max_blocks;
@@ -1015,12 +1070,22 @@
     scratch_scale_built_ = scratch_scale_;
     vpool_entries_ = std::max<uint64_t>(LDBG_VT_INITIAL * 2, std::min<uint64_t>(want_v, (uint64_t)(free_b * 0.40) / 8));
     table_floor_ = table_floor;
-    n_blocks_ = std::max<uint64_t>(2, std::min<uint64_t>(want_blocks, (uint64_t)(free_b * 0.35) / (LDBG_PATH_BLOCK * 8)));
+    n_blocks_ = std::max<uint64_t>(2, std::min<uint64_t>(want_blocks, (uint64_t)(free_b * 0.35) / (LDBG_PATH_BLOCK * 8) / sets));
     d_vpool_ = rt::dmalloc((size_t)vpool_entries_ * 8);
     d_ls_ = rt::dmalloc((size_t)slots * ecap * sizeof(LsElem));
     d_snap_ = rt::dmalloc((size_t)slots * LDBG_SNAP_CAP * sizeof(LsSnap));
-    d_pool_ = rt::dmalloc((size_t)n_blocks_ * LDBG_PATH_BLOCK * 8);
-    d_block_table_ = rt::dmalloc((size_t)ns * max_blocks * 4);
+    for (int i = 0; i < sets; i++) {
+        d_pool_set_[i] = rt::dmalloc((size_t)n_blocks_ * LDBG_PATH_BLOCK * 8);
+        d_bt_set_[i] = rt::dmalloc((size_t)ns * max_blocks * 4);
+    }
+    cur_set_ = 0;
+    d_pool_ = d_pool_set_[0]; d_block_table_ = d_bt_set_[0];
+    if (sets == 2 && getenv("LDBG_HOST_TIMES")) {
+        static std::atomic<bool> said{false};
+        if (!said.exchange(true))
+            fprintf(stderr, "[ldbg] second path pool + block table: %.1f MB more device memory per engine (%lld strands)\n",
+                    ((double)n_blocks_ * LDBG_PATH_BLOCK * 8 + (double)ns * max_blocks * 4) / 1048576.0, (long long)ns);
+    }
     rt::dmemset(d_vpool_, 0, (size_t)vpool_entries_ * 8, s);
     vpool_dirty_ = 0;
     n_slots_ = slots; ecap_ = ecap; max_blocks_ = max_blocks; bt_strands_ = ns;
@@ -1052,7 +1117,7 @@
                 (uint64_t*)d_batch_words_, (uint8_t*)d_batch_valid_);
 }
 void Engine::drop_batch_seeds() {
-    if (d_batch_words_ || d_batch_valid_ || d_batch_ascii_) quiesce();
+    if (d_batch_words_ || d_batch_valid_ || d_batch_ascii_) sync_own_stream();
     rt::tfree(d_batch_words_); rt::tfree(d_batch_valid_); rt::tfree(d_batch_ascii_);
     d_batch_words_ = d_batch_valid_ = d_batch_ascii_ = nullptr;
 }
@@ -1080,6 +1145,7 @@
         else if (!scratch_full_ && scratch_scale_ < (1ull << 24)) {
             scratch_scale_ *= 4;
             pool_growths_++;
+            profile_add("walk_pool_growths", 1.0);
             todo.push_back({first, cnt});
         } else {
             if (cnt == 1) throw StatusError(LDBG_ERR_HIP, "path pool too small for a single walk: not enough device memory");
@@ -1168,7 +1234,14 @@
     r.max_blocks = (int)(((int64_t)cfg.max_branch_length + 2 + LDBG_PATH_BLOCK - 1) / LDBG_PATH_BLOCK);
     HostLaps laps;
     const bool lean_pools = !img && (view.g.k & 1) && !getenv("LDBG_NO_RUNS") && !getenv("LDBG_VT_INITIAL") && !getenv("LDBG_FULL_POOLS");
-    ensure_scratch(ns, link_store_capacity, r.max_blocks, 0, lean_pools);
+    const bool two_sets = lean_pools && result_stream_ && !getenv("LDBG_SYNC_CONTIGS");
+    ensure_scratch(ns, link_store_capacity, r.max_blocks, 0, lean_pools, two_sets);
+    if (!img && d_pool_set_[1]) {
+        cur_set_ ^= 1;
+        d_pool_ = d_pool_set_[cur_set_]; d_block_table_ = d_bt_set_[cur_set_];
+        if (gens_[cur_set_] && gens_[cur_set_]->pending) gens_[cur_set_]->c1.stream_wait(s);
+    }
+    r.out.pool_set = cur_set_;
     zero_dirty_tables(s);
     laps.lap("scratch + zero (issued)");
 
@@ -1371,6 +1444,7 @@
         LDBG_LAUNCH(k_retry_list, grid_for(ns, 256, 1024), 256, s, (const uint32_t*)r.d_status, ns, r.d_retry, r.d_ctr + 28);
         rt::d2h(ctr, r.d_ctr, 256, s);
         rt::stream_sync(s);
+        results_wait();
         if (r.timed) { r.walk_ms += rt::Event::elapsed_ms(r.ev0, r.ev1); r.timed = false; }
         const int64_t n_again = (int64_t)ctr[28];
         if (n_again > 0) {
@@ -1407,6 +1481,7 @@
     rt::d2h(ctr, r.d_ctr, 256, s);
     rt::d2h(ctr + 32, d_totals, 16, s);
     rt::stream_sync(s);
+    results_wait();
     if (r.timed) { r.walk_ms += rt::Event::elapsed_ms(r.ev0, r.ev1); r.timed = false; }
     {
         static const char* const kind_names[8] = {"walk_steps_run", "walk_run_vertices", "walk_steps_lean", "walk_steps_general", "walk_link_adds", "walk_choices",
@@ -1460,32 +1535,54 @@
     out.runs = a.e.runs;
     out.dense_pending = true;
     laps.lap("result buffers");
-    rt::Event c0, c1;
-    c0.record(s);
+    ContigRleArgs ra{};
+    int rle_block = LDBG_STREAM_BLOCK, rle_grid = 1;
     if (lazy) {
-        ContigRleArgs ra;
         ra.g = graph->view; ra.runs = a.e.runs; ra.n = n; ra.seeds = a.seeds;
         ra.pool = (const uint64_t*)d_pool_; ra.block_table = (const uint32_t*)d_block_table_; ra.max_blocks = r.max_blocks;
         ra.strand_c = (const uint32_t*)out.d_strand_c; ra.strand_n = r.d_strand_n; ra.walk_len = d_walk_len; ra.contig_off = d_contig_off;
         ra.out = (char*)out.d_contigs;
-        int rb = LDBG_STREAM_BLOCK, rcap = LDBG_STREAM_GRID;
+        int rcap = LDBG_STREAM_GRID;
 #ifndef LDBG_HOSTSIM
-        if (const char* ev = getenv("LDBG_RLE_BLOCK")) rb = atoi(ev) >= 256 ? 256 : (atoi(ev) >= 128 ? 128 : 64);
+        if (const char* ev = getenv("LDBG_RLE_BLOCK")) rle_block = atoi(ev) >= 256 ? 256 : (atoi(ev) >= 128 ? 128 : 64);
         if (const char* ev = getenv("LDBG_RLE_GRID")) rcap = std::max(1, atoi(ev));
 #endif
-        LDBG_LAUNCH_W(r.W, k_contigs_rle, grid_for(n * 64, rb, rcap), rb, s, ra);
+        rle_grid = grid_for(n * 64, rle_block, rcap);
+    }
+    if (lazy && !a.img_on && result_stream_ && d_pool_set_[1] && !getenv("LDBG_SYNC_CONTIGS")) {
+        ContigGen& g = *gens_[out.pool_set];
+        gen_complete(g);
+        const int W = r.W;
+        rt::stream_t rs = result_stream_;
+        {
+            std::lock_guard<std::mutex> l(g_engines_mu);
+            g.c0.record(rs);
+            rt::launch_deferred(rs, [=] { LDBG_LAUNCH_W(W, k_contigs_rle, rle_grid, rle_block, rs, ra); });
+            g.c1.record(rs);
+            g.timed = true;
+        }
+        g.pending = true;
+        g.d_strand_n = r.d_strand_n; r.d_strand_n = nullptr;
+        out.deferred = true;
+        laps.lap("contigs (queued)");
     } else {
-        ensure_dense(out);
-        ContigArgs ca;
-        ca.g = graph->view; ca.n = n; ca.seeds = a.seeds; ca.dense = (const uint64_t*)out.d_path; ca.strand_off = (const int64_t*)out.d_strand_off;
-        ca.walk_len = d_walk_len; ca.contig_off = d_contig_off; ca.quirk = r.d_quirk; ca.term = (const uint64_t*)out.d_term;
-        ca.out = (char*)out.d_contigs;
-        LDBG_LAUNCH_W(r.W, k_contigs, grid_for(n * 64), 256, s, ca);
-    }
-    c1.record(s);
-    rt::stream_sync(s);
-    profile_add("contig", rt::Event::elapsed_ms(c0, c1));
-    laps.lap("paths + contigs");
+        rt::Event c0, c1;
+        c0.record(s);
+        if (lazy) {
+            LDBG_LAUNCH_W(r.W, k_contigs_rle, rle_grid, rle_block, s, ra);
+        } else {
+            ensure_dense(out);
+            ContigArgs ca;
+            ca.g = graph->view; ca.n = n; ca.seeds = a.seeds; ca.dense = (const uint64_t*)out.d_path; ca.strand_off = (const int64_t*)out.d_strand_off;
+            ca.walk_len = d_walk_len; ca.contig_off = d_contig_off; ca.quirk = r.d_quirk; ca.term = (const uint64_t*)out.d_term;
+            ca.out = (char*)out.d_contigs;
+            LDBG_LAUNCH_W(r.W, k_contigs, grid_for(n * 64), 256, s, ca);
+        }
+        c1.record(s);
+        rt::stream_sync(s);
+        profile_add("contig", rt::Event::elapsed_ms(c0, c1));
+        laps.lap("paths + contigs");
+    }
     r.free_tmp();
     d_walk_len = nullptr; d_contig_off = nullptr;
     free_results();
@@ -1499,6 +1596,7 @@
         throw StatusError(LDBG_ERR_UNSUPPORTED, "walks over a sharded table run ContigStopper without connectAllNeighbors / secondary colours");
     if (&img.graph() != graph) throw StatusError(LDBG_ERR_ARG, "the engine was not created on this image's graph");
     enter();
+    results_wait();
     sharded_abort();
     clear_batch();
     seeds_to_device(seeds, n, false);
@@ -1606,6 +1704,7 @@
 
 void Engine::walk_batch_fetch(char* arena, int64_t cap, int64_t* offsets, int64_t* walk_len) {
     enter();
+    results_wait();
     if (offsets || walk_len) for (auto& c : chunks) ensure_host(c);
     if (offsets) {
         int64_t o = 0;
@@ -1626,6 +1725,7 @@
 
 void Engine::walk_vertices(int64_t walk, int64_t capacity, int64_t* len, uint64_t* words, int64_t* rec, int32_t* copy, int32_t* index) {
     enter();
+    results_wait();
     if (walk < 0 || walk >= batch_n) throw StatusError(LDBG_ERR_ARG, "walk index out of range");
     const int W = graph->hdr.W;
     for (auto& c : chunks) {
@@ -1660,6 +1760,8 @@
 
 #ifdef LDBG_HOSTSIM
 extern "C" unsigned ldbg_hostsim_ls_peak(void) { const unsigned p = ::ldbg::ls_peak_elements(); ::ldbg::ls_peak_elements() = 0; return p; }
+extern "C" unsigned long long ldbg_hostsim_deferred_held(void) { return (unsigned long long)::ldbg::rt::HeldStream::deferred_held().load(); }
+extern "C" unsigned long long ldbg_hostsim_deferred_late(void) { return (unsigned long long)::ldbg::rt::HeldStream::deferred_late().load(); }
 extern "C" unsigned ldbg_hostsim_ls_fast(void) { return (unsigned)LDBG_LS_FAST; }
 extern "C" unsigned long long ldbg_hostsim_group_tail(void) { const unsigned long long n = ::ldbg::group_tail_accesses(); ::ldbg::group_tail_accesses() = 0; return n; }
 #endif
```

After: 192.6 billion. Within noise of the previous version (-0.2%).
